# falcon-computing/bwa-flow

Hardware: AMD Instinct MI355X
Metric: million reads/sec (2×150 bp PE) end-to-end align; SW-extend GCUPS at 1/2/4/8 MI355X (higher is better)
Workload: dtype int32

## Files before the change

### bwa-flow_amd/csrc/capi.hip

```cpp
#include <hip/hip_runtime.h>
#include <string.h>

#include <algorithm>
#include <chrono>
#include <condition_variable>
#include <deque>
#include <functional>
#include <cstdio>
#include <mutex>
#include <new>
#include <string>
#include <thread>
#include <vector>

#include "regpost.h"
#include "seed.h"
#include "chain.h"
#include "ctx.h"
#include "engine.h"

using namespace bwagpu;

namespace {

// ... 65 lines not shown

struct InLayout {
  size_t seq_off, seq, rco, cso, rid, frac, seeds, total;
  void make(const bwagpu_batch_t& b) {
    size_t o = 0;
    auto take = [&](size_t n) {
      size_t at = o;
      o += (n + 255) & ~(size_t)255;
      return at;
    };
    seq_off = take(sizeof(int64_t) * (size_t)(b.n_reads + 1));
    rco = take(sizeof(int32_t) * (size_t)(b.n_reads + 1));
    cso = take(sizeof(int32_t) * (size_t)(b.n_chains + 1));
    rid = take(sizeof(int32_t) * (size_t)b.n_chains);
    frac = take(sizeof(float) * (size_t)b.n_chains);
    seeds = take(sizeof(bwagpu_seed_t) * (size_t)b.n_seeds);
    seq = take((size_t)b.seq_bytes);
    total = o;
  }
};

__global__ void side_probe_spin(uint64_t ticks) {
  const uint64_t t0 = __builtin_amdgcn_s_memrealtime();
  while (__builtin_amdgcn_s_memrealtime() - t0 < ticks) __builtin_amdgcn_s_sleep(8);
}
__global__ void side_probe_nop() {}

bool streams_concurrent(hipStream_t a, hipStream_t b) {
  hipEvent_t ea = nullptr, eb = nullptr;
  if (hipEventCreateWithFlags(&ea, hipEventDisableTiming) != hipSuccess) return false;
  if (hipEventCreateWithFlags(&eb, hipEventDisableTiming) != hipSuccess) {
    (void)hipEventDestroy(ea);
    return false;
  }
  hipLaunchKernelGGL(side_probe_spin, dim3(1), dim3(64), 0, a, (uint64_t)15000);
  bool conc = false;
  if (hipGetLastError() == hipSuccess && hipEventRecord(ea, a) == hipSuccess) {
    hipLaunchKernelGGL(side_probe_nop, dim3(1), dim3(64), 0, b);
    if (hipGetLastError() == hipSuccess && hipEventRecord(eb, b) == hipSuccess &&
        hipEventSynchronize(eb) == hipSuccess)
      conc = hipEventQuery(ea) == hipErrorNotReady;
  }
  (void)hipEventSynchronize(ea);
  (void)hipEventDestroy(ea);
  (void)hipEventDestroy(eb);
  return conc;
}

constexpr int kDenseScanBlock = 1024;
__global__ void __launch_bounds__(kDenseScanBlock) dense_scan_kernel(const int32_t* __restrict__ n, int nr,
                                                                     int32_t* __restrict__ off,
                                                                     int32_t* __restrict__ h_off) {
  __shared__ int32_t part[kDenseScanBlock];
  const int t = (int)threadIdx.x;
  const int per = (nr + kDenseScanBlock - 1) / kDenseScanBlock;
  const int r0 = min(t * per, nr), r1 = min(r0 + per, nr);
  int sum = 0;
  for (int r = r0; r < r1; ++r) sum += n[r];
  part[t] = sum;
  __syncthreads();
  for (int d = 1; d < kDenseScanBlock; d <<= 1) {
    const int v = t >= d ? part[t - d] : 0;
    __syncthreads();
    part[t] += v;
    __syncthreads();
  }
  int run = part[t] - sum;
  for (int r = r0; r < r1; ++r) {
    off[r] = run;
    h_off[r] = run;
    run += n[r];
  }
  if (t == kDenseScanBlock - 1) {
    off[nr] = part[t];
    h_off[nr] = part[t];
  }
}

__global__ void __launch_bounds__(256) dense_copy_kernel(const bwagpu_alnreg_t* __restrict__ out,
                                                         const int32_t* __restrict__ n,
                                                         const int32_t* __restrict__ off,
                                                         const int32_t* __restrict__ rco,
                                                         const int32_t* __restrict__ cso, int nr,
                                                         bwagpu_alnreg_t* __restrict__ dense) {
  constexpr int kW = (int)(sizeof(bwagpu_alnreg_t) / 8);
  const int r = (int)((blockIdx.x * 256u + threadIdx.x) >> 4), l = (int)(threadIdx.x & 15);
  if (r >= nr) return;
  const int words = n[r] * kW;
  const uint2* src = reinterpret_cast<const uint2*>(out + cso[rco[r]]);
  uint2* dst = reinterpret_cast<uint2*>(dense + off[r]);
  for (int w = l; w < words; w += 16) dst[w] = src[w];
}

}

namespace {

bool make_opt(const bwagpu_opt_t* o, DevOpt* d, std::string* why) {
  if (!o) { *why = "opt is NULL"; return false; }
  if (o->e_del <= 0 || o->e_ins <= 0) { *why = "gap extension penalties must be > 0"; return false; }
  if (o->w < 0 || o->a < 0) { *why = "negative band width or match score"; return false; }
  if (o->a > 127 || o->e_del > 65535 || o->e_ins > 65535 || o->o_del < 0 || o->o_del > 65535 || o->o_ins < 0 ||
      o->o_ins > 65535 || o->pen_clip5 < 0 || o->pen_clip5 >= (1 << 20) || o->pen_clip3 < 0 ||
      o->pen_clip3 >= (1 << 20) || o->w > (1 << 20)) {
    *why = "scoring option out of range";
    return false;
  }
  memset(d, 0, sizeof(*d));
  d->a = o->a;
  d->o_del = o->o_del;
  d->e_del = o->e_del;
  d->o_ins = o->o_ins;
  d->e_ins = o->e_ins;
  d->oe_del = o->o_del + o->e_del;
  d->oe_ins = o->o_ins + o->e_ins;
  d->pen_clip5 = o->pen_clip5;
  d->pen_clip3 = o->pen_clip3;
  d->w = o->w;
  d->zdrop = o->zdrop;
  int mx = 0;
  for (int i = 0; i < 25; ++i) mx = std::max<int>(mx, o->mat[i]);
  d->max_mat = mx;
  d->row_bound = 1;
  memcpy(d->mat, o->mat, 25);
  for (int q = 0; q < 5; ++q) {
    uint32_t w = 0;
    for (int t = 0; t < 4; ++t) w |= (uint32_t)(uint8_t)o->mat[t * 5 + q] << (8 * t);
    d->qprof[q] = w;
    d->qprof4[q] = o->mat[20 + q];
  }
  return true;
}

int create_common(int device, const bwagpu_opt_t* opt, const bwagpu_bns_t* bns, bwagpu_ctx_t** out,
                  bwagpu_ctx_t** made) {
  if (!out || !bns || bns->l_pac <= 0 || bns->n_seqs <= 0 || !bns->ann_offset || !bns->ann_len)
    return BWAGPU_E_INVAL;
  int n = 0;
  if (hipGetDeviceCount(&n) != hipSuccess || n <= 0) return BWAGPU_E_NODEVICE;
  if (device < 0 || device >= n) return BWAGPU_E_NODEVICE;
  bwagpu_ctx_t* ctx = new (std::nothrow) bwagpu_ctx_t();
  if (!ctx) return BWAGPU_E_NOMEM;
  std::string why;
  if (!make_opt(opt, &ctx->opt, &why)) {
    delete ctx;
    return BWAGPU_E_INVAL;
  }
  ctx->device = device;
  ctx->opt_b = opt->b;
  ctx->ext_form = set_ext_form(-1);
  ctx->ext_short = ext_short_default();
  ctx->ext_short_fill = ext_short_fill_default();
  ctx->light_pack = light_pack_default();
  *made = ctx;
  HIPC(hipSetDevice(device), "hipSetDevice");
  HIPC(hipMalloc(&ctx->d_ann_off, sizeof(int64_t) * bns->n_seqs), "hipMalloc(ann_offset)");
  HIPC(hipMalloc(&ctx->d_ann_len, sizeof(int32_t) * bns->n_seqs), "hipMalloc(ann_len)");
  HIPC(hipMemcpy(ctx->d_ann_off, bns->ann_offset, sizeof(int64_t) * bns->n_seqs, hipMemcpyHostToDevice),
       "upload ann_offset");
  HIPC(hipMemcpy(ctx->d_ann_len, bns->ann_len, sizeof(int32_t) * bns->n_seqs, hipMemcpyHostToDevice),
       "upload ann_len");
  for (auto& s : ctx->slot) {
    HIPC(hipEventCreate(&s.ev0), "hipEventCreate");
    HIPC(hipEventCreate(&s.ev1), "hipEventCreate");
    HIPC(hipEventCreate(&s.ev2), "hipEventCreate");
    HIPC(hipEventCreate(&s.ev3), "hipEventCreate");
  }
  ctx->ref.l_pac = bns->l_pac;
  ctx->ref.n_seqs = bns->n_seqs;
  ctx->ref.ann_offset = ctx->d_ann_off;
  ctx->ref.ann_len = ctx->d_ann_len;
  return BWAGPU_OK;
}

std::vector<Slot*> all_slots(bwagpu_ctx_t* ctx) {
  std::vector<Slot*> v;
  for (auto& x : ctx->slot) v.push_back(&x);
  for (auto& x : ctx->dev_scratch) v.push_back(&x);
  v.push_back(&ctx->ch_slot);
  return v;
}

void destroy_ctx(bwagpu_ctx_t* ctx) {
  if (!ctx) return;
  (void)hipSetDevice(ctx->device);
  for (auto& s : ctx->slot) {
    if (s.stream) (void)hipStreamSynchronize(s.stream);
    s.d_in.release(); s.release_scratch();
    s.d_out.release(); s.d_n.release(); s.d_stats.release();
    s.h_in.release(); s.h_out.release(); s.h_n.release(); s.h_stats.release();
    s.h_dense.release(); s.h_off.release(); s.d_off.release();
    if (s.ev0) (void)hipEventDestroy(s.ev0);
    if (s.ev1) (void)hipEventDestroy(s.ev1);
    if (s.ev2) (void)hipEventDestroy(s.ev2);
    if (s.ev3) (void)hipEventDestroy(s.ev3);
    if (s.stream) (void)hipStreamDestroy(s.stream);
  }
  for (int k = 0; k < BWAGPU_NUM_SLOTS; ++k) {
    if (ctx->dev_stream[k]) (void)hipStreamSynchronize(ctx->dev_stream[k]);
    Slot& s = ctx->dev_scratch[k];
    s.release_scratch();
    s.d_stats.release();
  }
  if (ctx->sdh_done) {
    (void)hipEventSynchronize(ctx->sdh_done);
    (void)hipEventDestroy(ctx->sdh_done);
  }
  for (hipStream_t x : ctx->side_graveyard) {
    (void)hipStreamSynchronize(x);
    (void)hipStreamDestroy(x);
  }
  ctx->side_graveyard.clear();
  for (hipEvent_t e : ctx->prof_ev) (void)hipEventDestroy(e);
  ctx->prof_ev.clear();
  for (int i = 0; i < bwagpu_ctx::kA2Streams; ++i) {
    if (ctx->a2_st[i]) (void)hipStreamSynchronize(ctx->a2_st[i]);
    if (ctx->a2_st[i]) (void)hipStreamDestroy(ctx->a2_st[i]);
    if (ctx->a2_join[i]) (void)hipEventDestroy(ctx->a2_join[i]);
  }
  if (ctx->a2_fork) (void)hipEventDestroy(ctx->a2_fork);
  ctx->ch_slot.release_scratch();
  for (int k = 0; k < 2; ++k) {
    if (ctx->ch_cs.side[k]) (void)hipStreamSynchronize(ctx->ch_cs.side[k]);
    if (ctx->ch_cs.side[k]) (void)hipStreamDestroy(ctx->ch_cs.side[k]);
    if (ctx->ch_cs.join[k]) (void)hipEventDestroy(ctx->ch_cs.join[k]);
  }
  if (ctx->ch_cs.fork) (void)hipEventDestroy(ctx->ch_cs.fork);
  ctx->ch_slot.d_out.release(); ctx->ch_slot.d_n.release(); ctx->ch_slot.d_stats.release();
  if (ctx->r2d_done && ctx->r2d_pending) (void)hipEventSynchronize(ctx->r2d_done);
  for (DevBuf* b : {&ctx->ex_tasks, &ctx->ex_list, &ctx->ex_q, &ctx->ex_t, &ctx->ex_res, &ctx->ex_stats, &ctx->a2_tasks,
                    &ctx->a2_q, &ctx->a2_t, &ctx->a2_out, &ctx->a2_scratch, &ctx->a2_lists, &ctx->a2_counts, &ctx->a2_boff,
                    &ctx->r2_tasks, &ctx->r2_q, &ctx->r2_out, &ctx->r2_cig, &ctx->r2_md, &ctx->r2_lists, &ctx->r2_z,
                    &ctx->r2_stats, &ctx->bwt_words, &ctx->sa_d, &ctx->sa_in, &ctx->sa_out, &ctx->occ_d, &ctx->sup_d, &ctx->sa_full, &ctx->sd_off,
                    &ctx->sd_seq, &ctx->sd_out, &ctx->sd_n, &ctx->sd_scratch, &ctx->sd_poff, &ctx->sd_pack,
                    &ctx->sd_heavy, &ctx->sd_dbg, &ctx->st_buf, &ctx->st_start, &ctx->st_q, &ctx->st_tasks, &ctx->st_lists,
                    &ctx->st_seen, &ctx->st_ctr, &ctx->st_out, &ctx->ch_npos, &ctx->ch_posoff, &ctx->ch_frac,
                    &ctx->ch_nout, &ctx->ch_noseed, &ctx->ch_nsw, &ctx->ch_need, &ctx->ch_swtab, &ctx->ch_alt,
                    &ctx->ch_kpos, &ctx->ch_rbeg, &ctx->ch_qinfo, &ctx->ch_label, &ctx->ch_score, &ctx->ch_slist,
                    &ctx->ch_ord, &ctx->ch_chains, &ctx->ch_nodes, &ctx->ch_ochains, &ctx->ch_oslist, &ctx->ch_bins, &ctx->ch_dbg, &ctx->ch_swoff, &ctx->ch_swtasks, &ctx->ch_swt,
                    &ctx->ch_swskip, &ctx->ch_swres, &ctx->ch_swscr, &ctx->ch_ocoff, &ctx->ch_osoff, &ctx->ch_rco,
                    &ctx->ch_cso, &ctx->ch_rid, &ctx->ch_cfrac, &ctx->ch_out, &ctx->ch_seeds, &ctx->ch_regoff,
                    &ctx->ch_regc, &ctx->rp_stats, &ctx->pe_isize, &ctx->pe_cnt, &ctx->rs_pair, &ctx->rs_soff,
                    &ctx->rs_tab, &ctx->rs_toff, &ctx->rs_boff, &ctx->rs_qpool, &ctx->rs_ctr, &ctx->rs_scr,
                    &ctx->ps_scratch, &ctx->ps_log, &ctx->ps_erfc, &ctx->r2d_keys, &ctx->r2d_lists, &ctx->r2d_tab,
                    &ctx->r2d_z, &ctx->r2d_sums})
    b->release();
  ctx->r2d_htab.release();
  for (hipEvent_t e : {ctx->r2d_done, ctx->r2d_ev[0], ctx->r2d_ev[1]})
    if (e) (void)hipEventDestroy(e);
  ctx->stg.release();
  for (hipEvent_t e : ctx->rs_ev)
    if (e) (void)hipEventDestroy(e);
  for (int k = 0; k < kRescueMaxRounds; ++k)
    for (DevBuf* b : {&ctx->rs_tasks[k], &ctx->rs_tpool[k], &ctx->rs_res[k]}) b->release();
  for (HostBuf* b : {&ctx->sdh_in, &ctx->chh_tot, &ctx->chh_rco, &ctx->chh_cso, &ctx->chh_chains, &ctx->chh_seeds, &ctx->chh_regs,
                     &ctx->chh_n})
    b->release();
  if (ctx->own_pac && ctx->d_pac) (void)hipFree(ctx->d_pac);
  if (ctx->d_ann_off) (void)hipFree(ctx->d_ann_off);
  if (ctx->d_ann_len) (void)hipFree(ctx->d_ann_len);
  delete ctx;
}

int check_batch_header(bwagpu_ctx_t* ctx, const bwagpu_batch_t* b) {
  if (!b) return fail(ctx, BWAGPU_E_INVAL, "batch is NULL");
  if (b->n_reads < 0 || b->n_chains < 0 || b->n_seeds < 0 || b->seq_bytes < 0)
    return fail(ctx, BWAGPU_E_INVAL, "negative batch dimension");
  if (b->n_reads == 0) return BWAGPU_OK;
  if (!b->seq_off || !b->read_chain_off || !b->chain_seed_off)
    return fail(ctx, BWAGPU_E_INVAL, "NULL offset array");
  if (b->seq_off[0] != 0 || b->seq_off[b->n_reads] != b->seq_bytes)
    return fail(ctx, BWAGPU_E_INVAL, "seq_off does not span seq_bytes");
  if (b->read_chain_off[0] != 0 || b->read_chain_off[b->n_reads] != b->n_chains)
    return fail(ctx, BWAGPU_E_INVAL, "read_chain_off does not span n_chains");
  if (b->chain_seed_off[0] != 0 || b->chain_seed_off[b->n_chains] != b->n_seeds)
    return fail(ctx, BWAGPU_E_INVAL, "chain_seed_off does not span n_seeds");
  if (b->n_chains && (!b->chain_rid || !b->chain_frac_rep)) return fail(ctx, BWAGPU_E_INVAL, "NULL chain array");
  if (b->n_seeds && !b->seeds) return fail(ctx, BWAGPU_E_INVAL, "NULL seeds");
  if (b->seq_bytes && !b->seq) return fail(ctx, BWAGPU_E_INVAL, "NULL seq");
  return BWAGPU_OK;
}

int check_reads(const bwagpu_batch_t* b, int64_t l_pac, int r0, int r1, int64_t* lmax, int* bad_read) {
  const int64_t two = l_pac << 1;
  const int64_t* so = b->seq_off;
  const int32_t* rco = b->read_chain_off;
  const int32_t* cso = b->chain_seed_off;
  const bwagpu_seed_t* sd = b->seeds;
  int64_t lm = 0;
  for (int r = r0; r < r1; ++r) {
    const int64_t l = so[r + 1] - so[r];
    if (l < 0) return 1;
    if (l > BWAGPU_MAX_READ_LEN) {
      *bad_read = r;
      return 2;
    }
    lm = std::max(lm, l);
    const int c0 = rco[r], c1 = rco[r + 1];
    if (c0 < 0 || c1 < c0 || c1 > b->n_chains) return 3;
    bool bad_seed = false;
    for (int c = c0; c < c1; ++c) {
      const int k0 = cso[c], k1 = cso[c + 1];
      if (k0 < 0 || k1 < k0 || k1 > b->n_seeds) return 4;
      for (int k = k0; k < k1; ++k) {
        const bwagpu_seed_t& s = sd[k];
        bad_seed |= (s.qbeg < 0) | (s.len <= 0) | ((int64_t)s.qbeg + s.len > l) | (s.rbeg < 0) | (s.rbeg + s.len > two);
// ... 31 lines not shown
  int code[4] = {0, 0, 0, 0}, bad_read[4] = {0, 0, 0, 0};
  int64_t lmaxs[4] = {0, 0, 0, 0};
  host_parallel(nt, [&](int t) {
    code[t] = check_reads(b, ctx->ref.l_pac, (int)((int64_t)b->n_reads * t / nt),
                          (int)((int64_t)b->n_reads * (t + 1) / nt), &lmaxs[t], &bad_read[t]);
  });
  if (int rc = check_report(ctx, b, code, bad_read, nt)) return rc;
  *lq_max_out = (int)std::max(std::max(lmaxs[0], lmaxs[1]), std::max(lmaxs[2], lmaxs[3]));
  return BWAGPU_OK;
}

int stage_and_check(bwagpu_ctx_t* ctx, const bwagpu_batch_t* b, char* h, const InLayout& L, int* lq_max_out) {
  *lq_max_out = 0;
  const int nr = b->n_reads;
  if (nr == 0) return BWAGPU_OK;
  constexpr int kBlk = 1024, kMaxT = 8;
  const int nt = b->n_seeds >= (1 << 16) ? kMaxT : 1;
  const int nblk = (nr + kBlk - 1) / kBlk;
  int code[kMaxT] = {}, bad_read[kMaxT] = {};
  int64_t lmaxs[kMaxT] = {};
  auto work = [&](int t) {
    for (int k = (int)((int64_t)nblk * t / nt), ke = (int)((int64_t)nblk * (t + 1) / nt); k < ke; ++k) {
      const int r0 = k * kBlk, r1 = std::min(nr, r0 + kBlk);
      const int64_t b0 = b->seq_off[r0], b1 = b->seq_off[r1];
      const int c0 = b->read_chain_off[r0], c1 = b->read_chain_off[r1];
      if (b0 < 0 || b1 < b0 || b1 > b->seq_bytes) {
        code[t] = 1;
        return;
      }
      if (c0 < 0 || c1 < c0 || c1 > b->n_chains) {
        code[t] = 3;
        return;
      }
      const int k0 = b->chain_seed_off[c0], k1 = b->chain_seed_off[c1];
      if (k0 < 0 || k1 < k0 || k1 > b->n_seeds) {
        code[t] = 4;
        return;
      }
      const int re = r1 == nr ? r1 + 1 : r1, ce = c1 == b->n_chains ? c1 + 1 : c1;
      memcpy(h + L.seq_off + sizeof(int64_t) * r0, b->seq_off + r0, sizeof(int64_t) * (size_t)(re - r0));
      memcpy(h + L.rco + sizeof(int32_t) * r0, b->read_chain_off + r0, sizeof(int32_t) * (size_t)(re - r0));
      memcpy(h + L.cso + sizeof(int32_t) * c0, b->chain_seed_off + c0, sizeof(int32_t) * (size_t)(ce - c0));
      if (c1 > c0) {
        memcpy(h + L.rid + sizeof(int32_t) * c0, b->chain_rid + c0, sizeof(int32_t) * (size_t)(c1 - c0));
        memcpy(h + L.frac + sizeof(float) * c0, b->chain_frac_rep + c0, sizeof(float) * (size_t)(c1 - c0));
      }
      if (k1 > k0) memcpy(h + L.seeds + sizeof(bwagpu_seed_t) * k0, b->seeds + k0, sizeof(bwagpu_seed_t) * (size_t)(k1 - k0));
      if (b1 > b0) memcpy(h + L.seq + b0, b->seq + b0, (size_t)(b1 - b0));
      int64_t lm = 0;
      if ((code[t] = check_reads(b, ctx->ref.l_pac, r0, r1, &lm, &bad_read[t]))) return;
      lmaxs[t] = std::max(lmaxs[t], lm);
    }
  };
  host_parallel(nt, work);
  if (int rc = check_report(ctx, b, code, bad_read, nt)) return rc;
  int64_t lm = 0;
  for (int t = 0; t < nt; ++t) lm = std::max(lm, lmaxs[t]);
  *lq_max_out = (int)lm;
  return BWAGPU_OK;
}

bool use_read_kernels() {
  const char* e = getenv("BWAGPU_C2A_PATH");
  return e && (strcmp(e, "fast") == 0 || strcmp(e, "read") == 0);
}

size_t variant_lds(const DevOpt& o, int v, int lq_max) {
  const Variant& vk = kVariants[v];
  const int lqv = std::min(lq_max, vk.max_len());
  const int tb = tb_bytes_for(o, std::max(lqv, 1));
  return vk.kind == VK_FAST ? (size_t)(kBlock / 64) * fast_wave_lds(tb) : (size_t)tb * (kBlock / vk.G);
}

int check_lds(bwagpu_ctx_t* ctx, int lq_max) {
  if (!use_read_kernels()) {
    if (spec_redo_cap(tb_bytes_for(ctx->opt, std::max(lq_max, 1))) < 64)
      return fail(ctx, BWAGPU_E_UNSUPPORTED, "LDS row buffer too large for these options (w, pen_clip, read length)");
    return BWAGPU_OK;
  }
  for (int v = 0; v < kNumVariants; ++v) {
    if (variant_lds(ctx->opt, v, lq_max) > 64 * 1024)
      return fail(ctx, BWAGPU_E_UNSUPPORTED, "LDS row buffer too large for these options (w, pen_clip, read length)");
  }
  return BWAGPU_OK;
}

void register_caller_locked(bwagpu_ctx_t* ctx, hipStream_t st) {
  for (hipStream_t c : ctx->callers)
    if (c == st) return;
  for (Slot* x : all_slots(ctx))
    if (x->side_chosen && x->spec.side && hipStreamSynchronize(x->spec.side) == hipSuccess &&
        !streams_concurrent(x->spec.side, st)) {
      ctx->side_graveyard.push_back(x->spec.side);
      x->spec.side = nullptr;
      x->side_chosen = false;
    }
  ctx->callers.push_back(st);
}

hipError_t choose_side(bwagpu_ctx_t* ctx, Slot& s, hipStream_t st, SpecStreams* snap) {
  std::lock_guard<std::mutex> g(ctx->side_mu);
  register_caller_locked(ctx, st);
  if (s.side_chosen) {
    *snap = s.spec;
    return hipSuccess;
  }
  if (!s.spec.fork) {
    hipError_t e = hipEventCreateWithFlags(&s.spec.fork, hipEventDisableTiming);
    if (e == hipSuccess) e = hipEventCreateWithFlags(&s.spec.join, hipEventDisableTiming);
    if (e != hipSuccess) return e;
  }
  std::vector<hipStream_t> avoid = ctx->callers;
  for (Slot* x : all_slots(ctx))
    if (x != &s && x->side_chosen && x->spec.side) avoid.push_back(x->spec.side);
  std::vector<hipStream_t> tried;
  hipStream_t pick = nullptr;
  hipError_t e = hipSuccess;
  for (int t = 0; t < 6 && !pick; ++t) {
    hipStream_t c = nullptr;
    if ((e = hipStreamCreateWithFlags(&c, hipStreamNonBlocking)) != hipSuccess) break;
    bool ok = true;
    for (hipStream_t a : avoid)
      if (!streams_concurrent(c, a)) {
        ok = false;
        break;
      }
    if (ok) pick = c;
    else tried.push_back(c);
  }
  for (hipStream_t c : tried) (void)hipStreamDestroy(c);
  if (e != hipSuccess) return e;
  s.spec.side = pick;
  s.side_chosen = true;
  *snap = s.spec;
  return hipSuccess;
}

int enqueue_spec(bwagpu_ctx_t* ctx, Slot& s, const DevBatch& db, int lq_max, bwagpu_alnreg_t* d_out, int32_t* d_n,
                 int64_t* d_stats, hipStream_t st) {
  const size_t nc = (size_t)std::max(db.n_chains, 1), ns = (size_t)std::max(db.n_seeds, 1),
               nr = (size_t)std::max(db.n_reads, 1);
  HIPC(s.d_win.ensure(sizeof(ChainWin) * nc), "hipMalloc(win)");
  HIPC(s.d_cread.ensure(sizeof(int32_t) * nc), "hipMalloc(chain_read)");
  HIPC(s.d_prog.ensure(sizeof(bwagpu_seed_t) * ns), "hipMalloc(prog)");
  HIPC(s.d_ext.ensure(sizeof(SeedExt) * ns), "hipMalloc(ext)");
  HIPC(s.d_tasks.ensure(sizeof(int2) * kSpecBins * (nc + (kSpecRounds - 1) * ns)), "hipMalloc(tasks)");
  HIPC(s.d_ctr.ensure(sizeof(int32_t) * SPC_WORDS), "hipMalloc(ctr)");
  HIPC(s.d_regpos.ensure(sizeof(int32_t) * ns), "hipMalloc(regpos)");
  HIPC(s.d_skipf.ensure(sizeof(int32_t) * ns), "hipMalloc(skipf)");
  HIPC(s.d_heavy.ensure(sizeof(int32_t) * nr), "hipMalloc(heavy)");
  HIPC(s.d_redo.ensure(sizeof(int32_t) * nr), "hipMalloc(redo)");
  HIPC(s.d_rbits.ensure(sizeof(uint32_t) * (nr / 32 + 1)), "hipMalloc(rbits)");
  HIPC(s.d_desc.ensure(sizeof(ReadDesc) * nr), "hipMalloc(desc)");
  HIPC(s.d_schain.ensure(sizeof(int32_t) * ns), "hipMalloc(seedchain)");
  HIPC(s.d_hinfo.ensure(sizeof(int4) * nr), "hipMalloc(hinfo)");
  HIPC(s.d_cov.ensure(sizeof(int32_t) * ns), "hipMalloc(cov)");
  HIPC(s.d_hflag.ensure(sizeof(int32_t) * ns), "hipMalloc(hflag)");
  HIPC(s.d_colent.ensure(sizeof(int32_t) * ns), "hipMalloc(colent)");
  HIPC(s.d_longc.ensure(sizeof(int32_t) * nc), "hipMalloc(longc)");
  HIPC(s.d_qh.ensure(sizeof(int32_t) * kQHWords), "hipMalloc(qh)");
  HIPC(s.d_sorth.ensure(sizeof(int32_t) * kSortWords), "hipMalloc(sorth)");
  HIPC(s.d_stasks.ensure(sizeof(int2) * kSpecBins * (nc + (kSpecRounds - 1) * ns)), "hipMalloc(stasks)");
  HIPC(s.d_ftask.ensure(sizeof(FatTask) * kSpecBins * (nc + (kSpecRounds - 1) * ns)), "hipMalloc(ftask)");
  HIPC(s.d_ftaskR.ensure(sizeof(FatTask) * kSpecBins * (nc + (kSpecRounds - 1) * ns)), "hipMalloc(ftaskR)");
  const int64_t mat_words = std::max<int64_t>(1 << 20, 16 * (int64_t)ns);
  HIPC(s.d_mat.ensure(sizeof(uint64_t) * (size_t)mat_words), "hipMalloc(mat)");
  SpecArgs a;
  a.win = s.d_win.as<ChainWin>();
  a.chain_read = s.d_cread.as<int32_t>();
  a.prog = s.d_prog.as<bwagpu_seed_t>();
  a.ext = s.d_ext.as<SeedExt>();
  a.tasks = s.d_tasks.as<int2>();
  a.ctr = s.d_ctr.as<int32_t>();
  a.regpos = s.d_regpos.as<int32_t>();
  a.skipf = s.d_skipf.as<int32_t>();
  a.heavy = s.d_heavy.as<int32_t>();
  a.redo = s.d_redo.as<int32_t>();
  a.rbits = s.d_rbits.as<uint32_t>();
  a.rdesc = s.d_desc.as<ReadDesc>();
  a.seedchain = s.d_schain.as<int32_t>();
  a.hinfo = s.d_hinfo.as<int4>();
  a.mat = s.d_mat.as<uint64_t>();
  a.mat_words = (int64_t)(s.d_mat.cap / sizeof(uint64_t));
  a.cov = s.d_cov.as<int32_t>();
  a.hflag = s.d_hflag.as<int32_t>();
  a.colent = s.d_colent.as<int32_t>();
  a.longc = s.d_longc.as<int32_t>();
  a.qh = s.d_qh.as<int32_t>();
  a.sorth = s.d_sorth.as<int32_t>();
  a.stasks = s.d_stasks.as<int2>();
  a.ftask = s.d_ftask.as<FatTask>();
  a.ftaskR = s.d_ftaskR.as<FatTask>();
  static const int ext_prefetch = [] {
    const char* e = getenv("BWAGPU_EXT_PREFETCH");
    return e ? std::max(0, atoi(e)) : 0;
  }();
  a.ext_prefetch = ext_prefetch;
  static const int risky_first = [] {
    const char* e = getenv("BWAGPU_LIGHT_RISKY_FIRST");
    return e && e[0] == '1';
  }();
  a.risky_first = risky_first;
  static const int emu_strict = [] {
    const char* e = getenv("BWAGPU_EMU_STRICT");
    return !(e && e[0] == '0');
  }();
  a.emu_strict = emu_strict;
  a.light_pack = ctx->light_pack;
  a.out = d_out;
  a.out_n = d_n;
  a.stats = d_stats;
  SpecStreams ss;
  HIPC(choose_side(ctx, s, st, &ss), "side stream");
  a.lq_bound = lq_max;
  const int tb = tb_bytes_for(ctx->opt, std::max(lq_max, 1));
  ss.form = ctx->ext_form;
  ss.short_q = ctx->ext_short;
  ss.short_fill = ctx->ext_short_fill;
  ss.pool = ctx->prof_ev.empty() ? nullptr : ctx->prof_ev.data();
  ss.pool_n = (int)ctx->prof_ev.size();
  ss.pool_used = &ctx->prof_used;
  HIPC(launch_spec_clear(a, db.n_reads, db.n_seeds, st), "spec clear");
  HIPC(launch_spec_chain2aln(ctx->opt, ctx->ref, db, a, tb, lq_max, st, ss), "spec chain2aln launch");
  return BWAGPU_OK;
}

int enqueue_chain2aln(bwagpu_ctx_t* ctx, Slot& s, const DevBatch& db, int lq_max, bwagpu_alnreg_t* d_out,
                      int32_t* d_n, int64_t* d_stats, hipStream_t st) {
  if (!use_read_kernels()) return enqueue_spec(ctx, s, db, lq_max, d_out, d_n, d_stats, st);
  HIPC(s.d_win.ensure(sizeof(ChainWin) * (size_t)std::max(db.n_chains, 1)), "hipMalloc(win)");
  HIPC(s.d_srt.ensure(sizeof(uint64_t) * (size_t)std::max(db.n_seeds, 1)), "hipMalloc(srt)");
  HIPC(s.d_prog.ensure(sizeof(bwagpu_seed_t) * (size_t)std::max(db.n_seeds, 1)), "hipMalloc(prog)");
  const size_t nr = (size_t)std::max(db.n_reads, 1);
  HIPC(s.d_desc.ensure(sizeof(ReadDesc) * nr), "hipMalloc(desc)");
  HIPC(s.d_lists.ensure(2 * sizeof(int32_t) * nr), "hipMalloc(lists)");
  int32_t* bins = s.d_lists.as<int32_t>();
  int32_t* read_list = bins + nr;
  HIPC(s.d_counts.ensure(sizeof(int32_t) * kCountWords), "hipMalloc(counts)");
  HIPC(hipMemsetAsync(s.d_counts.p, 0, sizeof(int32_t) * kCountWords, st), "memset counts");
  if (db.n_reads) HIPC(hipMemsetAsync(d_n, 0, sizeof(int32_t) * db.n_reads, st), "memset out_n");
  HIPC(launch_chain_prep(ctx->opt, ctx->ref, db, s.d_win.as<ChainWin>(), s.d_srt.as<uint64_t>(),
                         s.d_prog.as<bwagpu_seed_t>(), d_stats, st),
       "chain_prep launch");
  HIPC(launch_read_order(db, bins, s.d_counts.as<int32_t>() + kHistOff, s.d_counts.as<int32_t>(),
                         s.d_desc.as<ReadDesc>(), read_list, d_stats, st),
       "read order launch");
  C2AArgs a;
  a.read_list = read_list;
  a.desc = s.d_desc.as<ReadDesc>();
  a.counts = s.d_counts.as<int32_t>();
  a.win = s.d_win.as<ChainWin>();
  a.srt = s.d_srt.as<uint64_t>();
  a.prog = s.d_prog.as<bwagpu_seed_t>();
  a.out = d_out;
  a.out_n = d_n;
  a.stats = d_stats;
  for (int v = 0; v < kNumVariants; ++v) {
    const int lqv = std::min(lq_max, kVariants[v].max_len());
    const int tb = tb_bytes_for(ctx->opt, std::max(lqv, 1));
    HIPC(launch_chain2aln(v, ctx->opt, ctx->ref, db, db.n_reads, tb, a, st), "chain2aln launch");
  }
  return BWAGPU_OK;
}

}

extern "C" {

int bwagpu_abi_version(void) { return BWAGPU_ABI_VERSION; }

int bwagpu_device_count(int* n) {
  if (!n) return BWAGPU_E_INVAL;
  int k = 0;
  if (hipGetDeviceCount(&k) != hipSuccess) k = 0;
  *n = k;
  return k > 0 ? BWAGPU_OK : BWAGPU_E_NODEVICE;
}

int bwagpu_create(int device, const bwagpu_opt_t* opt, const bwagpu_bns_t* bns, const uint8_t* pac_host,
                  bwagpu_ctx_t** out) {
  if (!pac_host) return BWAGPU_E_INVAL;
  bwagpu_ctx_t* ctx = nullptr;
  int rc = create_common(device, opt, bns, out, &ctx);
  if (rc == BWAGPU_OK) {
    const size_t pac_bytes = (size_t)(bns->l_pac / 4 + 1);
    hipError_t e = hipMalloc(&ctx->d_pac, pac_bytes);
    if (e == hipSuccess) {
      ctx->own_pac = true;
      e = hipMemcpy(ctx->d_pac, pac_host, pac_bytes, hipMemcpyHostToDevice);
    }
    if (e != hipSuccess) rc = hip_fail(ctx, e, "pac upload");
    ctx->ref.pac = (const uint8_t*)ctx->d_pac;
  }
  if (rc != BWAGPU_OK) {
    destroy_ctx(ctx);
    return rc;
  }
  *out = ctx;
  return BWAGPU_OK;
}

int bwagpu_create_resident(int device, const bwagpu_opt_t* opt, const bwagpu_bns_t* bns, const void* pac_device,
                           bwagpu_ctx_t** out) {
  if (!pac_device) return BWAGPU_E_INVAL;
  bwagpu_ctx_t* ctx = nullptr;
  int rc = create_common(device, opt, bns, out, &ctx);
  if (rc != BWAGPU_OK) {
    destroy_ctx(ctx);
    return rc;
  }
  ctx->d_pac = (void*)pac_device;
  ctx->own_pac = false;
  ctx->ref.pac = (const uint8_t*)pac_device;
  *out = ctx;
  return BWAGPU_OK;
}

int bwagpu_destroy(bwagpu_ctx_t* ctx) {
  if (!ctx) return BWAGPU_E_INVAL;
  destroy_ctx(ctx);
  return BWAGPU_OK;
}

const char* bwagpu_last_error(const bwagpu_ctx_t* ctx) { return ctx ? ctx->err.c_str() : "NULL context"; }

int bwagpu_set_watchdog_ms(bwagpu_ctx_t* ctx, int ms) {
  if (!ctx || ms < 0) return BWAGPU_E_INVAL;
  ctx->watchdog_ms = ms;
  return BWAGPU_OK;
}

namespace {
void expand_slots(const Slot& s, bwagpu_alnreg_t* dst) {
  const char* h = s.h_in.as<const char>();
  const int32_t* rco = s.kept ? s.keep_rco.data() : (const int32_t*)(h + s.in_rco);
  const int32_t* cso = s.kept ? s.keep_cso.data() : (const int32_t*)(h + s.in_cso);
  const int32_t* n = s.h_n.as<const int32_t>();
  const int32_t* off = s.h_off.as<const int32_t>();
  const bwagpu_alnreg_t* src = s.h_dense.as<const bwagpu_alnreg_t>();
  for (int32_t r = 0; r < s.n_reads; ++r)
    if (n[r]) memcpy(dst + cso[rco[r]], src + off[r], sizeof(bwagpu_alnreg_t) * (size_t)n[r]);
}
}

int bwagpu_chain2aln_submit(bwagpu_ctx_t* ctx, int slot, const bwagpu_batch_t* b) {
  if (!ctx || slot < 0 || slot >= BWAGPU_NUM_SLOTS) return BWAGPU_E_INVAL;
  Slot& s = ctx->slot[slot];
  if (s.busy) return fail(ctx, BWAGPU_E_INVAL, "slot already has a batch in flight");
  s.has_results = false;
  s.kept = false;
  s.slot_view = false;
  int lq_max = 0;
  int rc = check_batch_header(ctx, b);
  if (rc) return rc;
  HIPC(hipSetDevice(ctx->device), "hipSetDevice");
  s.t_submit = std::chrono::steady_clock::now();
  InLayout L;
  L.make(*b);
  HIPC(s.h_in.ensure(L.total), "hipHostMalloc(in)");
  HIPC(s.d_in.ensure(L.total), "hipMalloc(in)");
  HIPC(s.d_out.ensure(sizeof(bwagpu_alnreg_t) * (size_t)std::max(b->n_seeds, 1)), "hipMalloc(out)");
// ... 187 lines not shown
  if (!ctx || slot < 0 || slot >= BWAGPU_NUM_SLOTS || !regs || !n || !off) return BWAGPU_E_INVAL;
  Slot& s = ctx->slot[slot];
  if (s.busy) return fail(ctx, BWAGPU_E_INVAL, "slot's batch still in flight (wait first)");
  if (!s.has_results || !s.h_dense.p || !s.h_off.p) return fail(ctx, BWAGPU_E_INVAL, "slot has no results");
  *regs = s.h_dense.as<const bwagpu_alnreg_t>();
  *n = s.h_n.as<const int32_t>();
  *off = s.h_off.as<const int32_t>();
  return BWAGPU_OK;
}

int bwagpu_chain2aln(bwagpu_ctx_t* ctx, const bwagpu_batch_t* b, bwagpu_alnreg_t* out_regs, int32_t* out_n) {
  int rc = bwagpu_chain2aln_submit(ctx, 0, b);
  if (rc) return rc;
  return bwagpu_chain2aln_wait(ctx, 0, out_regs, out_n);
}

int bwagpu_chain2aln_device(bwagpu_ctx_t* ctx, const bwagpu_batch_t* db_in, bwagpu_alnreg_t* dev_out,
                            int32_t* dev_n, int64_t* dev_stats, void* stream) {
  if (!ctx || !db_in || !dev_out || !dev_n) return BWAGPU_E_INVAL;
  HIPC(hipSetDevice(ctx->device), "hipSetDevice");
  const int lq_bound = use_read_kernels() ? BWAGPU_MAX_READ_LEN : ctx->dev_read_len;
  int rc = check_lds(ctx, lq_bound);
  if (rc) return rc;
  hipStream_t st = (hipStream_t)stream;
  if (!st) HIPC(lazy_stream(ctx->slot[0], &st), "hipStreamCreate");
  int k = 0;
  while (k < BWAGPU_NUM_SLOTS && ctx->dev_stream[k] && ctx->dev_stream[k] != st) ++k;
  if (k == BWAGPU_NUM_SLOTS) return fail(ctx, BWAGPU_E_INVAL, "more than BWAGPU_NUM_SLOTS streams on one context");
  ctx->dev_stream[k] = st;
  Slot& s = ctx->dev_scratch[k];
  DevBatch db;
  db.n_reads = db_in->n_reads;
  db.n_chains = db_in->n_chains;
  db.n_seeds = db_in->n_seeds;
  db.seq_off = db_in->seq_off;
  db.seq = db_in->seq;
  db.read_chain_off = db_in->read_chain_off;
  db.chain_seed_off = db_in->chain_seed_off;
  db.chain_rid = db_in->chain_rid;
  db.chain_frac_rep = db_in->chain_frac_rep;
  db.seeds = db_in->seeds;
  int64_t* stats = dev_stats;
  if (!stats) {
    HIPC(s.d_stats.ensure(sizeof(int64_t) * ST_N), "hipMalloc(stats)");
    stats = s.d_stats.as<int64_t>();
    HIPC(hipMemsetAsync(stats, 0, sizeof(int64_t) * ST_N, st), "memset stats");
  }
  return enqueue_chain2aln(ctx, s, db, lq_bound, dev_out, dev_n, stats, st);
}

int bwagpu_debug_set_trace(bwagpu_ctx_t* ctx, void* dev_ptr) {
  if (!ctx) return BWAGPU_E_INVAL;
  HIPC(hipSetDevice(ctx->device), "hipSetDevice");
  HIPC(set_trace(dev_ptr), "set trace");
  HIPC(set_trace_spec(dev_ptr), "set trace");
  return BWAGPU_OK;
}

int bwagpu_debug_fail_wait(bwagpu_ctx_t* ctx, int after_n_waits, int code) {
  if (!ctx || code <= 0) return BWAGPU_E_INVAL;
  ctx->fail_after = after_n_waits;
  ctx->fail_code = code;
  return BWAGPU_OK;
}

int bwagpu_debug_occupancy(bwagpu_ctx_t* ctx, void* stream, int64_t* out) {
  if (!ctx || !out) return BWAGPU_E_INVAL;
  hipStream_t st = nullptr;
  if (int rc = entry_stream(ctx, stream, &st)) return rc;
  int k = 0;
  while (k < BWAGPU_NUM_SLOTS && ctx->dev_stream[k] != st) ++k;
  if (k == BWAGPU_NUM_SLOTS || !ctx->dev_scratch[k].d_ctr.p) return fail(ctx, BWAGPU_E_INVAL, "no device-entry batch on this stream");
  HIPC(hipStreamSynchronize(st), "hipStreamSynchronize");
  int32_t c[SPC_WORDS];
  HIPC(hipMemcpy(c, ctx->dev_scratch[k].d_ctr.p, sizeof c, hipMemcpyDeviceToHost), "hipMemcpy(ctr)");
  memcpy(out, c + 32, 14 * sizeof(int64_t));
#ifdef BWAGPU_OCC_DIAG
  return BWAGPU_OK;
#else
  return fail(ctx, BWAGPU_E_UNSUPPORTED, "built without BWAGPU_OCC_DIAG");
#endif
}

int bwagpu_debug_spec_counters(bwagpu_ctx_t* ctx, void* stream, int64_t* out) {
  if (!ctx || !out) return BWAGPU_E_INVAL;
  hipStream_t st = nullptr;
  if (int rc = entry_stream(ctx, stream, &st)) return rc;
  int k = 0;
  while (k < BWAGPU_NUM_SLOTS && ctx->dev_stream[k] != st) ++k;
  if (k == BWAGPU_NUM_SLOTS || !ctx->dev_scratch[k].d_ctr.p) return fail(ctx, BWAGPU_E_INVAL, "no device-entry batch on this stream");
  HIPC(hipStreamSynchronize(st), "hipStreamSynchronize");
  int32_t c[SPC_WORDS];
  HIPC(hipMemcpy(c, ctx->dev_scratch[k].d_ctr.p, sizeof c, hipMemcpyDeviceToHost), "hipMemcpy(ctr)");
  for (int r = 0; r < kSpecRounds; ++r) {
    out[r] = 0;
    for (int b = 0; b < kSpecBins; ++b) out[r] += c[SPC_CNT + r * kSpecBins + b];
  }
  int64_t spec = 0;
  memcpy(&spec, c + SPC_SPEC64, 8);
  out[3] = spec;
  out[4] = c[SPC_MISS];
  out[5] = c[SPC_HEAVY_N];
  out[6] = c[SPC_REDO_N];
  out[7] = c[SPC_HCOLS];
  return BWAGPU_OK;
}

int bwagpu_debug_spec_ext(bwagpu_ctx_t* ctx, void* stream, void* host_out, int32_t n) {
  if (!ctx || !host_out || n < 0) return BWAGPU_E_INVAL;
  hipStream_t st = nullptr;
  if (int rc = entry_stream(ctx, stream, &st)) return rc;
  int k = 0;
  while (k < BWAGPU_NUM_SLOTS && ctx->dev_stream[k] != st) ++k;
  if (k == BWAGPU_NUM_SLOTS || !ctx->dev_scratch[k].d_ext.p || ctx->dev_scratch[k].d_ext.cap < sizeof(SeedExt) * (size_t)n)
    return fail(ctx, BWAGPU_E_INVAL, "no device-entry batch of that size on this stream");
  HIPC(hipStreamSynchronize(st), "hipStreamSynchronize");
  HIPC(hipMemcpy(host_out, ctx->dev_scratch[k].d_ext.p, sizeof(SeedExt) * (size_t)n, hipMemcpyDeviceToHost),
       "hipMemcpy(ext)");
  return BWAGPU_OK;
}

int bwagpu_debug_ext_form(int form) { return set_ext_form(form); }

int bwagpu_streams_concurrent(void* a, void* b) {
  if (!a || !b || a == b) return BWAGPU_E_INVAL;
  return streams_concurrent((hipStream_t)a, (hipStream_t)b) ? 1 : 0;
}

int bwagpu_ctx_ext_form(bwagpu_ctx_t* ctx, int form) {
  if (!ctx) return BWAGPU_E_INVAL;
  const int prev = ctx->ext_form;
  if (form >= 0) ctx->ext_form = form > 2 ? 1 : form;
  return prev;
}

int bwagpu_ctx_ext_short(bwagpu_ctx_t* ctx, int q) {
  if (!ctx) return BWAGPU_E_INVAL;
  const int prev = ctx->ext_short;
  if (q >= 0) ctx->ext_short = q > 63 ? 63 : q;
  return prev;
}

int bwagpu_ctx_ext_short_fill(bwagpu_ctx_t* ctx, int percent) {
  if (!ctx) return BWAGPU_E_INVAL;
  const int prev = ctx->ext_short_fill;
  if (percent >= 0) ctx->ext_short_fill = percent > 100000 ? 100000 : percent;
  return prev;
}

int bwagpu_ctx_light_pack(bwagpu_ctx_t* ctx, int on) {
  if (!ctx) return BWAGPU_E_INVAL;
  const int prev = ctx->light_pack;
  if (on >= 0) ctx->light_pack = on != 0;
  return prev;
}

int bwagpu_debug_spec_short(bwagpu_ctx_t* ctx, void* stream, int64_t* out) {
  if (!ctx || !out) return BWAGPU_E_INVAL;
  hipStream_t st = nullptr;
  if (int rc = entry_stream(ctx, stream, &st)) return rc;
  int k = 0;
  while (k < BWAGPU_NUM_SLOTS && ctx->dev_stream[k] != st) ++k;
  if (k == BWAGPU_NUM_SLOTS || !ctx->dev_scratch[k].d_ctr.p) return fail(ctx, BWAGPU_E_INVAL, "no device-entry batch on this stream");
  HIPC(hipStreamSynchronize(st), "hipStreamSynchronize");
  int32_t c[SPC_WORDS];
  HIPC(hipMemcpy(c, ctx->dev_scratch[k].d_ctr.p, sizeof c, hipMemcpyDeviceToHost), "hipMemcpy(ctr)");
  out[0] = c[SPC_SHORT_N];
  for (int r = 0; r < 2; ++r) {
    const int l = r * kSpecBins;
    out[1 + 4 * r] = c[SPC_LCNT + l];
    out[2 + 4 * r] = c[SPC_LLONG + l];
    out[3 + 4 * r] = c[SPC_RCNT + l];
    out[4 + 4 * r] = c[SPC_RLONG + l];
  }
  return BWAGPU_OK;
}

int bwagpu_ctx_row_bound(bwagpu_ctx_t* ctx, int on) {
  if (!ctx) return BWAGPU_E_INVAL;
  const int prev = ctx->opt.row_bound;
  if (on >= 0) ctx->opt.row_bound = on ? 1 : 0;
  return prev;
}

int bwagpu_debug_ext_kernel(bwagpu_ctx_t* ctx, int32_t lq_max) {
  if (!ctx || lq_max < 1 || lq_max > BWAGPU_MAX_READ_LEN) return BWAGPU_E_INVAL;
  return ext_kernel_for(ctx->opt, ctx->ext_form, tb_bytes_for(ctx->opt, lq_max));
}

int bwagpu_prof_start(bwagpu_ctx_t* ctx, int max_launches) {
  if (!ctx || max_launches < 0) return BWAGPU_E_INVAL;
  HIPC(hipSetDevice(ctx->device), "hipSetDevice");
  for (hipEvent_t e : ctx->prof_ev) HIPC(hipEventSynchronize(e), "hipEventSynchronize");
  for (hipEvent_t e : ctx->prof_ev) (void)hipEventDestroy(e);
  ctx->prof_ev.clear();
  ctx->prof_used = 0;
  for (int i = 0; i < 2 * max_launches; ++i) {
    hipEvent_t e = nullptr;
    HIPC(hipEventCreate(&e), "hipEventCreate");
    ctx->prof_ev.push_back(e);
  }
  return BWAGPU_OK;
}

int bwagpu_prof_read(bwagpu_ctx_t* ctx, double* total_ms, int32_t* launches) {
  if (!ctx || !total_ms || !launches) return BWAGPU_E_INVAL;
  HIPC(hipSetDevice(ctx->device), "hipSetDevice");
  double t = 0;
  for (int i = 0; i + 1 < ctx->prof_used; i += 2) {
    HIPC(hipEventSynchronize(ctx->prof_ev[i + 1]), "hipEventSynchronize");
    float ms = 0;
    HIPC(hipEventElapsedTime(&ms, ctx->prof_ev[i], ctx->prof_ev[i + 1]), "hipEventElapsedTime");
    t += ms;
  }
  *total_ms = t;
  *launches = ctx->prof_used / 2;
  return BWAGPU_OK;
}

int bwagpu_prof_intervals(bwagpu_ctx_t* ctx, double* start_ms, double* end_ms, int32_t max, int32_t* n) {
  if (!ctx || !n || max < 0 || (max && (!start_ms || !end_ms))) return BWAGPU_E_INVAL;
  HIPC(hipSetDevice(ctx->device), "hipSetDevice");
  int k = 0;
  for (int i = 0; i + 1 < ctx->prof_used && k < max; i += 2, ++k) {
    HIPC(hipEventSynchronize(ctx->prof_ev[i + 1]), "hipEventSynchronize");
    float a = 0, b = 0;
    HIPC(hipEventElapsedTime(&a, ctx->prof_ev[0], ctx->prof_ev[i]), "hipEventElapsedTime");
    HIPC(hipEventElapsedTime(&b, ctx->prof_ev[0], ctx->prof_ev[i + 1]), "hipEventElapsedTime");
    start_ms[k] = a;
    end_ms[k] = b;
  }
  *n = k;
  return BWAGPU_OK;
}

int bwagpu_last_stats(const bwagpu_ctx_t* ctx, int slot, bwagpu_stats_t* out) {
  if (!ctx || !out || slot < 0 || slot >= BWAGPU_NUM_SLOTS) return BWAGPU_E_INVAL;
  *out = ctx->slot[slot].last;
  return BWAGPU_OK;
}

}

extern "C" int bwagpu_set_bwt(bwagpu_ctx_t* ctx, const bwagpu_bwt_t* bwt) {
  if (!ctx || !bwt || !bwt->bwt || bwt->bwt_size == 0) return BWAGPU_E_INVAL;
  if (bwt->bwt_size < ((bwt->seq_len + 127) >> 7) * 16 || bwt->L2[4] != bwt->seq_len || bwt->primary > bwt->seq_len)
    return fail(ctx, BWAGPU_E_INVAL, "bwt header inconsistent with its occurrence array");
  HIPC(hipSetDevice(ctx->device), "hipSetDevice");
  HIPC(ctx->bwt_words.ensure(sizeof(uint32_t) * bwt->bwt_size + 64), "hipMalloc");
  HIPC(hipMemcpy(ctx->bwt_words.p, bwt->bwt, sizeof(uint32_t) * bwt->bwt_size, hipMemcpyHostToDevice), "H2D");
  ctx->bwt.primary = bwt->primary;
  for (int i = 0; i < 5; ++i) ctx->bwt.L2[i] = bwt->L2[i];
  ctx->bwt.seq_len = bwt->seq_len;
  ctx->bwt.bwt = ctx->bwt_words.as<uint32_t>();
  {
    HIPC(ctx->occ_d.ensure(2 * sizeof(uint4) * (size_t)occ64_blocks(bwt->seq_len)), "hipMalloc");
    ctx->bwt.sup_shift = ctx->sup_shift;
    HIPC(ctx->sup_d.ensure(4 * sizeof(uint64_t) * (size_t)occ64_supers(bwt->seq_len, ctx->sup_shift)), "hipMalloc");
    HIPC(hipMemset(ctx->occ_d.p, 0, 2 * sizeof(uint4) * (size_t)occ64_blocks(bwt->seq_len)), "memset");
    hipStream_t st = nullptr;
  HIPC(lazy_stream(ctx->slot[0], &st), "hipStreamCreate");
    HIPC(launch_build_occ64(ctx->bwt, ctx->occ_d.as<uint4>(), ctx->sup_d.as<uint64_t>(), st), "build_occ64 launch");
    HIPC(hipStreamSynchronize(st), "sync");
    ctx->bwt.occ = ctx->occ_d.as<uint4>();
    ctx->bwt.sup = ctx->sup_d.as<uint64_t>();
  }
  ctx->bwt.sa = nullptr;
  ctx->bwt.sa_mask = 0;
  ctx->bwt.sa_shift = 0;
  ctx->bwt.sa_full32 = nullptr;
  ctx->bwt.sa_full64 = nullptr;
  if (bwt->sa) {
    const int iv = bwt->sa_intv;
    if (iv < 1 || (iv & (iv - 1)) || bwt->n_sa < bwt->seq_len / (uint64_t)iv + 1)
      return fail(ctx, BWAGPU_E_INVAL, "suffix array sample interval / size inconsistent");
    HIPC(ctx->sa_d.ensure(sizeof(uint64_t) * bwt->n_sa), "hipMalloc");
    HIPC(hipMemcpy(ctx->sa_d.p, bwt->sa, sizeof(uint64_t) * bwt->n_sa, hipMemcpyHostToDevice), "H2D");
    ctx->bwt.sa = ctx->sa_d.as<uint64_t>();
    ctx->bwt.sa_mask = (uint64_t)iv - 1;
    while ((1 << ctx->bwt.sa_shift) < iv) ++ctx->bwt.sa_shift;
    const char* fe = getenv("BWAGPU_SA_FULL");
    const bool narrow = bwt->seq_len < 0xffffffffull && !(fe && strcmp(fe, "64") == 0);
    const uint64_t bytes = (bwt->seq_len + 1) * (narrow ? 4 : 8);
    size_t free_b = 0, total_b = 0;
    if (!(fe && strcmp(fe, "0") == 0) && iv > 1 && hipMemGetInfo(&free_b, &total_b) == hipSuccess &&
        bytes <= ((uint64_t)64 << 30) && bytes <= free_b / 4) {
      HIPC(ctx->sa_full.ensure((size_t)bytes), "hipMalloc");
      hipStream_t st = nullptr;
      HIPC(lazy_stream(ctx->slot[0], &st), "hipStreamCreate");
      HIPC(launch_sa_expand(ctx->bwt, narrow ? ctx->sa_full.as<uint32_t>() : nullptr,
                            narrow ? nullptr : ctx->sa_full.as<uint64_t>(), st),
           "sa_expand launch");
      HIPC(hipStreamSynchronize(st), "sync");
      if (narrow) ctx->bwt.sa_full32 = ctx->sa_full.as<uint32_t>();
      else ctx->bwt.sa_full64 = ctx->sa_full.as<uint64_t>();
    }
  }
  ctx->has_bwt = true;
  return BWAGPU_OK;
}

extern "C" int bwagpu_bwt_sa(bwagpu_ctx_t* ctx, int64_t n, const uint64_t* k, uint64_t* out) {
  if (!ctx || n < 0 || (n && (!k || !out))) return BWAGPU_E_INVAL;
  if (!ctx->has_bwt || !ctx->bwt.sa) return fail(ctx, BWAGPU_E_INVAL, "no suffix array: pass it to bwagpu_set_bwt");
  for (int64_t i = 0; i < n; ++i)
    if (k[i] > ctx->bwt.seq_len) return fail(ctx, BWAGPU_E_INVAL, "BWT position past seq_len");
// ... 533 lines not shown
```

### bwa-flow_amd/csrc/ctx.h

```cpp
#pragma once
#include <hip/hip_runtime.h>
#include <stdint.h>

#include <algorithm>
#include <chrono>
#include <mutex>
#include <string>
#include <vector>

#include "bwagpu.h"
#include "chain.h"
#include "engine.h"
#include "rescue.h"
#include "seed.h"
#include "stage_host.h"
#include "task_host.h"

namespace bwagpu {

template <bool kPinned>
struct GrowBuf {
  void* p = nullptr;
  size_t cap = 0;
  hipError_t ensure(size_t n) {
    if (n <= cap) return hipSuccess;
    release();
    const size_t want = std::max<size_t>(n + n / 4, 4096);
    const hipError_t e = kPinned ? hipHostMalloc(&p, want, hipHostMallocDefault) : hipMalloc(&p, want);
    if (e == hipSuccess) cap = want;
    else p = nullptr;
    return e;
  }
  void release() {
    if (p) (void)(kPinned ? hipHostFree(p) : hipFree(p));
    p = nullptr;
    cap = 0;
  }
  template <class T>
  T* as() const { return (T*)p; }
};
using DevBuf = GrowBuf<false>;
using HostBuf = GrowBuf<true>;

struct Slot {
  hipStream_t stream = nullptr;
  std::once_flag stream_once;
  hipError_t stream_err = hipSuccess;
  hipEvent_t ev0 = nullptr, ev1 = nullptr, ev2 = nullptr, ev3 = nullptr;
  DevBuf d_in, d_win, d_srt, d_prog, d_desc, d_out, d_n, d_stats, d_lists, d_counts;
  DevBuf d_cread, d_ext, d_tasks, d_ctr, d_regpos, d_skipf, d_heavy, d_redo, d_rbits;
  DevBuf d_schain, d_hinfo, d_mat, d_cov, d_hflag, d_colent, d_qh, d_longc, d_sorth, d_stasks, d_ftask, d_ftaskR;
  SpecStreams spec;
  bool side_chosen = false;
  void release_scratch() {
    d_win.release(); d_srt.release(); d_prog.release(); d_desc.release(); d_lists.release(); d_counts.release();
    d_cread.release(); d_ext.release(); d_tasks.release(); d_ctr.release(); d_regpos.release(); d_skipf.release();
    d_heavy.release(); d_redo.release(); d_rbits.release(); d_schain.release(); d_hinfo.release(); d_mat.release(); d_cov.release(); d_hflag.release(); d_colent.release(); d_longc.release();
    d_qh.release();
    d_sorth.release();
    d_stasks.release();
    d_ftask.release();
    d_ftaskR.release();
    if (spec.side) (void)hipStreamSynchronize(spec.side);
    if (spec.side) (void)hipStreamDestroy(spec.side);
    if (spec.fork) (void)hipEventDestroy(spec.fork);
    if (spec.join) (void)hipEventDestroy(spec.join);
    spec = SpecStreams{};
    side_chosen = false;
  }
  HostBuf h_in, h_out, h_n, h_stats;
  HostBuf h_dense, h_off;
  DevBuf d_off;
  size_t in_rco = 0, in_cso = 0;
  bool slot_view = false;
  bool busy = false;
  bool has_results = false;
  bool kept = false;
  std::vector<int32_t> keep_rco, keep_cso;
  int32_t n_reads = 0, n_chains = 0, n_seeds = 0;
  std::chrono::steady_clock::time_point t_submit;
  bwagpu_stats_t last{};
  int64_t h2d = 0, d2h = 0;
};

inline hipError_t lazy_stream(Slot& s, hipStream_t* st) {
  std::call_once(s.stream_once, [&s] { s.stream_err = hipStreamCreateWithFlags(&s.stream, hipStreamNonBlocking); });
  *st = s.stream;
  return s.stream_err;
}

struct Staging {
  DevBuf regs, out_regs;
  DevBuf seq;
  DevBuf seq_off, reg_off, out_off;
  DevBuf n, out_n, n_pri, status, n_sw, mapq, sel;
  DevBuf pes;
  void release() {
    for (DevBuf* b : {&regs, &out_regs, &seq, &seq_off, &reg_off, &out_off, &n, &out_n, &n_pri, &status, &n_sw, &mapq,
                      &sel, &pes})
      b->release();
  }
};

}

struct bwagpu_ctx {
  using DevBuf = bwagpu::DevBuf;
  using HostBuf = bwagpu::HostBuf;
  using Slot = bwagpu::Slot;
  int device = 0;
  std::mutex side_mu;
  std::vector<hipStream_t> callers, side_graveyard;
  bwagpu::DevOpt opt{};
  bwagpu::DevRef ref{};
  bool own_pac = false;
  void* d_pac = nullptr;
  int64_t* d_ann_off = nullptr;
  int32_t* d_ann_len = nullptr;
  int watchdog_ms = 10000;
  int ext_form = 0;
  int ext_short = 0;
  int light_pack = 0;
  int ext_short_fill = 0;
  Slot slot[BWAGPU_NUM_SLOTS];
  hipStream_t dev_stream[BWAGPU_NUM_SLOTS] = {};
  Slot dev_scratch[BWAGPU_NUM_SLOTS];
  DevBuf ex_tasks, ex_list, ex_q, ex_t, ex_res, ex_stats;
  DevBuf a2_tasks, a2_q, a2_t, a2_out, a2_scratch, a2_lists, a2_counts, a2_boff;
  DevBuf r2_tasks, r2_q, r2_out, r2_cig, r2_md, r2_lists, r2_z, r2_stats;
  DevBuf r2d_keys, r2d_lists, r2d_tab, r2d_z, r2d_sums;
  HostBuf r2d_htab;
  hipEvent_t r2d_done = nullptr, r2d_ev[2] = {};
  bool r2d_pending = false, r2d_timing = false, r2d_timed = false;
  double r2d_wait_ms = 0, r2d_call_ms = 0;
  int32_t r2d_jobs = 0;
  static constexpr int kA2Streams = 4;
  hipStream_t a2_st[kA2Streams] = {};
  hipEvent_t a2_fork = nullptr, a2_join[kA2Streams] = {};
  DevBuf bwt_words, sa_d, sa_in, sa_out, occ_d, sup_d, sa_full;
  bwagpu::DevBwt bwt{};
  bool has_bwt = false;
  DevBuf sd_off, sd_seq, sd_out, sd_n, sd_scratch, sd_poff, sd_pack, sd_heavy, sd_dbg;
  DevBuf ch_npos, ch_posoff, ch_frac, ch_nout, ch_noseed, ch_nsw, ch_need, ch_swtab, ch_alt;
  DevBuf ch_kpos, ch_rbeg, ch_qinfo, ch_label, ch_score, ch_slist, ch_ord, ch_chains, ch_nodes;
  DevBuf ch_ochains, ch_oslist, ch_bins, ch_dbg;
  DevBuf ch_swoff, ch_swtasks, ch_swt, ch_swskip, ch_swres, ch_swscr;
  DevBuf ch_ocoff, ch_osoff, ch_rco, ch_cso, ch_rid, ch_cfrac, ch_out, ch_seeds;
  DevBuf ch_regoff, ch_regc;
  HostBuf chh_tot, chh_rco, chh_cso, chh_chains, chh_seeds, chh_regs, chh_n;
  HostBuf sdh_in;
  hipEvent_t sdh_done = nullptr;
  Slot ch_slot;
  bwagpu::ChainStreams ch_cs{};
  bool has_alt = false;
  bwagpu::Staging stg;
  int opt_b = 0;
  bwagpu_postopt_t post_opt{};
  int32_t post_flags = 0;
  int64_t post_id0 = 0;
  DevBuf rp_stats;
  DevBuf pe_isize, pe_cnt;
  DevBuf rs_pair, rs_soff, rs_tab, rs_toff, rs_boff, rs_qpool, rs_ctr, rs_scr;
  DevBuf rs_tasks[bwagpu::kRescueMaxRounds], rs_tpool[bwagpu::kRescueMaxRounds], rs_res[bwagpu::kRescueMaxRounds];
  int32_t rescue_drop = 0;
  hipEvent_t rs_ev[4 * bwagpu::kRescueMaxRounds] = {};
  int rs_ev_rounds = 0;
  hipStream_t rs_ev_stream = nullptr;
  DevBuf ps_scratch, ps_log, ps_erfc;
  bool ps_log_ready = false;
  DevBuf st_buf, st_start, st_q, st_tasks, st_lists, st_seen, st_ctr, st_out;
  int seed_budget = 1024;
  int sup_shift = 32;
  int dev_read_len = BWAGPU_MAX_READ_LEN;
  int fail_after = -1, fail_code = 0;
  std::vector<hipEvent_t> prof_ev;
  int prof_used = 0;
  std::string err;
};

namespace bwagpu {

inline int fail(bwagpu_ctx_t* c, int code, const std::string& msg) {
  if (c) c->err = msg;
  return code;
}

inline int hip_fail(bwagpu_ctx_t* c, hipError_t e, const char* what) {
  std::string m = std::string(what) + ": " + hipGetErrorString(e);
  if (e == hipErrorOutOfMemory || e == hipErrorMemoryAllocation) return fail(c, BWAGPU_E_NOMEM, m);
  return fail(c, BWAGPU_E_DEVICE, m);
}

#define HIPC(call, what)                             \
  do {                                               \
    hipError_t e_ = (call);                          \
    if (e_ != hipSuccess) return hip_fail(ctx, e_, what); \
  } while (0)
#define TRY(call)                     \
  do {                                \
    if (int rc_ = (call)) return rc_; \
  } while (0)

inline int refuse(bwagpu_ctx_t* c, int code, const char* why) { return why && *why ? fail(c, code, why) : code; }

inline int entry_stream(bwagpu_ctx_t* ctx, void* stream, hipStream_t* st) {
  HIPC(hipSetDevice(ctx->device), "hipSetDevice");
  *st = (hipStream_t)stream;
  if (!*st) HIPC(lazy_stream(ctx->slot[0], st), "hipStreamCreate");
  return BWAGPU_OK;
}

inline int side_fork(bwagpu_ctx_t* ctx, hipStream_t st, size_t n_launches, int* used) {
  for (int i = 0; i < bwagpu_ctx::kA2Streams; ++i) {
    if (!ctx->a2_st[i]) HIPC(hipStreamCreateWithFlags(&ctx->a2_st[i], hipStreamNonBlocking), "stream");
    if (!ctx->a2_join[i]) HIPC(hipEventCreateWithFlags(&ctx->a2_join[i], hipEventDisableTiming), "event");
  }
  if (!ctx->a2_fork) HIPC(hipEventCreateWithFlags(&ctx->a2_fork, hipEventDisableTiming), "event");
  *used = (int)std::min<size_t>(bwagpu_ctx::kA2Streams, n_launches);
  HIPC(hipEventRecord(ctx->a2_fork, st), "event");
  for (int i = 0; i < *used; ++i) HIPC(hipStreamWaitEvent(ctx->a2_st[i], ctx->a2_fork, 0), "stream wait");
  return BWAGPU_OK;
}
inline int side_join(bwagpu_ctx_t* ctx, hipStream_t st, int used) {
  for (int i = 0; i < used; ++i) {
    HIPC(hipEventRecord(ctx->a2_join[i], ctx->a2_st[i]), "event");
    HIPC(hipStreamWaitEvent(st, ctx->a2_join[i], 0), "stream wait");
  }
  return BWAGPU_OK;
}

struct EventPair {
  hipEvent_t e0 = nullptr, e1 = nullptr;
  EventPair() = default;
  EventPair(const EventPair&) = delete;
  EventPair& operator=(const EventPair&) = delete;
  ~EventPair() {
    if (e0) (void)hipEventDestroy(e0);
    if (e1) (void)hipEventDestroy(e1);
  }
  hipError_t start(hipStream_t st) {
    hipError_t e = hipEventCreate(&e0);
    if (e == hipSuccess) e = hipEventCreate(&e1);
    return e == hipSuccess ? hipEventRecord(e0, st) : e;
  }
  hipError_t stop(hipStream_t st) { return hipEventRecord(e1, st); }
  float ms() const {
    float t = 0;
    (void)hipEventElapsedTime(&t, e0, e1);
    return t;
  }
};

int enqueue_regpost(bwagpu_ctx_t* ctx, const bwagpu_postopt_t& po, int32_t flags, int64_t id0, int32_t n_reads,
                    const int64_t* seq_off, const uint8_t* seq, const int64_t* reg_off, const int32_t* rco,
                    const int32_t* cso, bwagpu_alnreg_t* regs, int32_t* n, int64_t* stats, hipStream_t st);

struct HostCall {
  bwagpu_ctx_t* ctx;
  Staging& g;
  hipStream_t st = nullptr;
  EventPair ev;
  int64_t h2d = 0, d2h = 0, hs[ST_N] = {};
  std::vector<int64_t> roff, soff, ooff;
  bool open = false;

  explicit HostCall(bwagpu_ctx_t* c) : ctx(c), g(c->stg) {}
  HostCall(const HostCall&) = delete;
  HostCall& operator=(const HostCall&) = delete;
  ~HostCall() {
    if (open) (void)hipStreamSynchronize(st);
  }
  int begin() {
    if (int rc = entry_stream(ctx, nullptr, &st)) return rc;
    open = true;
    return BWAGPU_OK;
// ... 55 lines not shown
```

### bwa-flow_amd/csrc/engine.h

```cpp
#pragma once
#include <hip/hip_runtime.h>
#include <stdint.h>

#include "bwagpu.h"
#include "bwagpu_debug.h"
#include "pure.h"
#include "spec_plan.h"

namespace bwagpu {

struct ReadDesc {
  int64_t qoff;
  int32_t rd;
  int32_t lq;
  int32_t c0;
  int32_t nch;
  int32_t s0;
  int32_t ns;
};

struct ChainWin {
  int64_t lo, hi;
};

struct DevBatch {
  int32_t n_reads, n_chains, n_seeds;
  const int64_t* seq_off;
  const uint8_t* seq;
  const int32_t* read_chain_off;
  const int32_t* chain_seed_off;
  const int32_t* chain_rid;
  const float* chain_frac_rep;
  const bwagpu_seed_t* seeds;
};

struct DevRef {
  int64_t l_pac;
  int32_t n_seqs;
  const uint8_t* pac;
  const int64_t* ann_offset;
  const int32_t* ann_len;
};

enum { ST_CELLS = 0, ST_ROWS = 1, ST_CALLS = 2, ST_ERR = 3, ST_N = 4 };
enum { ERR_RID = 1, ERR_LEN = 2 };

constexpr int kFastMaxSeeds = 32;
constexpr int kFastMaxChains = 32;
constexpr int kSeqLds = 256;
constexpr int kNumVariants = 3;
extern const Variant kVariants[kNumVariants];
constexpr int kHistOff = 128;
constexpr int kCountWords = kHistOff + kNumVariants * 256;

hipError_t launch_chain_prep(const DevOpt& o, const DevRef& ref, const DevBatch& b, ChainWin* win, uint64_t* srt,
                             bwagpu_seed_t* prog, int64_t* stats, hipStream_t st);
hipError_t launch_read_order(const DevBatch& b, int32_t* bins, int32_t* hist, int32_t* counts, ReadDesc* desc,
                             int32_t* list, int64_t* stats, hipStream_t st);
struct C2AArgs {
  const int32_t* read_list;
  const ReadDesc* desc;
  int32_t* counts;
  const ChainWin* win;
  uint64_t* srt;
  const bwagpu_seed_t* prog;
  bwagpu_alnreg_t* out;
  int32_t* out_n;
  int64_t* stats;
};
hipError_t launch_chain2aln(int variant, const DevOpt& o, const DevRef& ref, const DevBatch& b, int32_t max_list,
                            int tb_bytes, const C2AArgs& a, hipStream_t st);
size_t fast_wave_lds(int tb);

hipError_t launch_extend(int variant, bool t5, const DevOpt& o, int32_t n_tasks,
                         const bwagpu_ext_task_t* tasks, const int32_t* task_list, int32_t n_list,
                         const uint8_t* qpool, const uint8_t* tpool, int tb_bytes,
                         bwagpu_ext_result_t* res, int64_t* stats, hipStream_t st);
hipError_t launch_extend4(const DevOpt& o, const bwagpu_ext_task_t* tasks, const int32_t* task_list, int32_t n_list,
                          const uint8_t* qpool, const uint8_t* tpool, int tb_bytes, bwagpu_ext_result_t* res,
                          int64_t* stats, hipStream_t st);

struct SeedExt {
  int64_t rb, re;
  int32_t qb, qe, score, truesc, w;
  int32_t cells, rows, calls;
};

constexpr int kSpecRounds = 3;
constexpr int kOrderLane = 8;
constexpr int kSelLight = 64;
constexpr int kSelRegLds = 256;
constexpr int kSelMatMaxSeeds = 4096;
enum {
  SPC_CNT = 0,
  SPC_HEAVY_N = 16,
  SPC_SEL_CUR = 17,
  SPC_REDO_N = 20,
  SPC_SPEC64 = 24,
  SPC_MISS = 26,
  SPC_MATW64 = 28,
  SPC_HCOLS = 30,
  SPC_LONG_N = 31,
  SPC_LCNT = 64,
  SPC_RCNT = 73,
  SPC_LIGHT_CUR = 82,
  SPC_LLONG = 84,
  SPC_RLONG = 93,
  SPC_SHORT_N = 102,
  SPC_WORDS = 128
};
constexpr int kQHStride = 32;
constexpr int kQHShort = 2 * kSpecRounds * kSpecBins * 8 * kQHStride;
constexpr int kQHWords = 2 * kQHShort;
constexpr int kSortKeys = 1024;
constexpr int kSortWordsR = kSpecRounds * 2 * kSortKeys;
constexpr int kSortWords = 2 * kSortWordsR;
__host__ __device__ inline size_t spec_list_off(int list, int n_chains, int n_seeds) {
  const int round = list / kSpecBins, bin = list % kSpecBins;
  return round == 0 ? (size_t)bin * n_chains
                    : (size_t)kSpecBins * n_chains + ((size_t)(round - 1) * kSpecBins + bin) * n_seeds;
}
struct FatTask {
  int64_t rbeg, qoff;
  int32_t pos;
  int32_t dlo, dhi;
  uint32_t qls;
};
static_assert(sizeof(FatTask) == 32, "FatTask layout");
static_assert(BWAGPU_MAX_READ_LEN < 1024, "FatTask packs qbeg / len / lq in 10 bits each");
struct SpecArgs {
  int lq_bound;
  ChainWin* win;
  int32_t* chain_read;
  bwagpu_seed_t* prog;
  SeedExt* ext;
  int2* tasks;
  int32_t* ctr;
  int32_t* regpos;
  int32_t* skipf;
  int32_t* heavy;
  int32_t* redo;
  uint32_t* rbits;
  ReadDesc* rdesc;
  int32_t* seedchain;
  int4* hinfo;
  int32_t* colent;
  int32_t* longc;
  uint64_t* mat;
  int64_t mat_words;
  int32_t* cov;
  int32_t* hflag;
  int32_t* qh;
  int32_t* sorth;
  int2* stasks;
  FatTask* ftask;
  FatTask* ftaskR;
  int risky_first;
  int emu_strict;
  int light_pack;
  int ext_prefetch;
  bwagpu_alnreg_t* out;
  int32_t* out_n;
  int64_t* stats;
};
struct SpecStreams {
  hipStream_t side = nullptr;
  hipEvent_t fork = nullptr, join = nullptr;
  hipEvent_t* pool = nullptr;
  int pool_n = 0;
  int* pool_used = nullptr;
  int form = 0;
  int short_q = 0;
  int short_fill = 0;
};
int set_ext_form(int form);
int ext_short_default();
int ext_short_fill_default();
int light_pack_default();
int ext_kernel_for(const DevOpt& o, int form, int tb_bytes);
hipError_t launch_spec_clear(const SpecArgs& a, int n_reads, int n_seeds, hipStream_t st);
hipError_t launch_spec_chain2aln(const DevOpt& o, const DevRef& ref, const DevBatch& b, const SpecArgs& a,
                                 int tb_bytes, int lq_max, hipStream_t st, const SpecStreams& ss);
size_t spec_select_lds(int tb_bytes);
int spec_redo_cap(int tb_bytes);

struct StreamTask {
  bwagpu_seed_t s;
  int64_t lo, hi;
  int64_t qoff;
  int32_t lq, pad_;
};
enum { STR_ERR_RECORD = 1, STR_ERR_TASK = 2, STR_ERR_DUP = 4, STR_ERR_SEED = 8, STR_ERR_BASE = 16 };
enum { kStrDecoded = 4, kStrMax = 5, kStrErr = 6, kStrHeads = 64 };
constexpr int kStrCtrWords = kStrHeads + kSpecBins * 8 * kQHStride;
struct StreamArgs {
  const int32_t* buf;
  const int64_t* rstart;
  int32_t n_reads, cap;
  int64_t l_pac;
  uint8_t* qpool;
  StreamTask* tasks;
  int32_t* lists;
  int32_t* seen;
  int32_t* ctr;
  int32_t* out;
};
hipError_t launch_sw_stream(const DevOpt& o, const DevRef& ref, const StreamArgs& a, int tb_bytes, hipStream_t st);

hipError_t set_trace(void* dev_ptr);
hipError_t set_trace_spec(void* dev_ptr);

}
```

### bwa-flow_amd/csrc/spec.hip

```cpp
#include "spec_dev.h"

namespace bwagpu {

__device__ uint32_t* g_trace = nullptr;
hipError_t set_trace_spec(void* p) { return hipMemcpyToSymbol(HIP_SYMBOL(g_trace), &p, sizeof(p)); }


__global__ void __launch_bounds__(256) spec_chain_kernel(DevOpt o, DevRef ref, DevBatch b, SpecArgs a) {
  sel_prio();
  const int c = blockIdx.x * blockDim.x + threadIdx.x;
  bool task = false, longc = false;
  int bin = 0, s0 = 0;
  if (c < b.n_chains) {
    const int rd = a.chain_read[c];
    s0 = b.chain_seed_off[c];
    const int ns = b.chain_seed_off[c + 1] - s0;
    const int lq = (int)(b.seq_off[rd + 1] - b.seq_off[rd]);
    if (ns <= 0) {
      a.win[c] = ChainWin{0, 0};
    } else {
      int64_t wlo = ref.l_pac << 1, whi = 0;
      longc = ns > kOrderLane;
      if (!longc) {
        uint64_t key[kOrderLane];
#pragma unroll
        for (int t = 0; t < kOrderLane; ++t) {
          key[t] = ~0ull;
          if (t < ns) {
            const bwagpu_seed_t v = b.seeds[s0 + t];
            key[t] = (uint64_t)(uint32_t)v.score << 32 | (uint32_t)t;
            seed_reach(o, v, lq, wlo, whi);
          }
        }
#pragma unroll
        for (int t = 0; t < kOrderLane; ++t) {
          if (t < ns) {
            int rank = 0;
#pragma unroll
            for (int u = 0; u < kOrderLane; ++u) rank += key[u] < key[t];
            bwagpu_seed_t v = b.seeds[s0 + t];
            v.pad_ = key[t] == 0 ? 1 : 0;
            a.prog[s0 + ns - 1 - rank] = v;
            a.seedchain[s0 + ns - 1 - rank] = c;
          }
        }
      }
      const bool ok = finish_window(ref, b.chain_rid[c], b.seeds[s0].rbeg, wlo, whi);
      if (!ok) {
        atomicOr((unsigned long long*)&a.stats[ST_ERR], (unsigned long long)ERR_RID);
        a.win[c] = ChainWin{0, -1};
      } else {
        if (!longc) a.win[c] = ChainWin{wlo, whi};
        task = lq <= a.lq_bound;
        bin = spec_bin(lq);
      }
    }
  }
#pragma unroll
  for (int k = 0; k < kSpecBins; ++k) {
    const int p = wave_append(&a.ctr[SPC_CNT + k], task && bin == k);
    if (p >= 0) a.tasks[(size_t)k * b.n_chains + p] = make_int2(s0, c);
  }
  const int p = wave_append(&a.ctr[SPC_LONG_N], longc);
  if (p >= 0) a.longc[p] = c;
}

__global__ void __launch_bounds__(256) spec_reads_kernel(DevBatch b, SpecArgs a) {
  sel_prio();
  const int rd = blockIdx.x * blockDim.x + threadIdx.x;
  bool heavy = false;
  int ns = 0;
  if (rd < b.n_reads) {
    const int lq = (int)(b.seq_off[rd + 1] - b.seq_off[rd]);
    if (lq > a.lq_bound) atomicOr((unsigned long long*)&a.stats[ST_ERR], (unsigned long long)ERR_LEN);
    ReadDesc d;
    d.qoff = b.seq_off[rd];
    d.rd = rd;
    d.lq = lq;
    d.c0 = b.read_chain_off[rd];
    d.nch = b.read_chain_off[rd + 1] - d.c0;
    d.s0 = b.chain_seed_off[d.c0];
    d.ns = b.chain_seed_off[d.c0 + d.nch] - d.s0;
    a.rdesc[rd] = d;
    for (int c = d.c0; c < d.c0 + d.nch; ++c) a.chain_read[c] = rd;
    heavy = d.ns > kSelLight || d.nch > kSelLight;
    ns = d.ns;
  }
  const int p = wave_append(&a.ctr[SPC_HEAVY_N], heavy);
  if (p >= 0) {
    a.heavy[p] = rd;
    const long long words = 2 * tri_off(ns);
    int woff = -1, col = 0;
    if (ns <= kSelMatMaxSeeds) {
      const long long o = (long long)atomicAdd(reinterpret_cast<unsigned long long*>(&a.ctr[SPC_MATW64]),
                                               (unsigned long long)words);
      if (o + words <= a.mat_words) {
        woff = (int)o;
        col = atomicAdd(&a.ctr[SPC_HCOLS], ns);
        for (int i = 0; i < ns; ++i) a.colent[col + i] = p;
      }
    }
    a.hinfo[p] = make_int4(rd, woff, col, ns);
  }
}

constexpr int kOrderBlocks = 1024;
constexpr int kOrderLds = 4096;
__device__ __forceinline__ uint64_t order_key(const bwagpu_seed_t* sd, int i) {
  return (uint64_t)(uint32_t)sd[i].score << 32 | (uint32_t)i;
}
__global__ void __launch_bounds__(256) spec_order_kernel(DevOpt o, DevRef ref, DevBatch b, SpecArgs a) {
  sel_prio();
  __shared__ uint64_t keys[kOrderLds];
  __shared__ int64_t wred[2][4];
  const int tid = (int)threadIdx.x;
  const int n_long = __hip_atomic_load(&a.ctr[SPC_LONG_N], __ATOMIC_RELAXED, __HIP_MEMORY_SCOPE_AGENT);
  for (int gi = (int)blockIdx.x; gi < n_long; gi += (int)gridDim.x) {
    const int g = a.longc[gi];
    const int s0 = b.chain_seed_off[g], ns = b.chain_seed_off[g + 1] - s0;
    const bwagpu_seed_t* sd = b.seeds + s0;
    const bool in_lds = ns <= kOrderLds;
    const int rd = a.chain_read[g];
    const int lq = (int)(b.seq_off[rd + 1] - b.seq_off[rd]);
    int64_t wlo = ref.l_pac << 1, whi = 0;
    for (int i = tid; i < ns; i += 256) {
      const bwagpu_seed_t v = sd[i];
      if (in_lds) keys[i] = (uint64_t)(uint32_t)v.score << 32 | (uint32_t)i;
      seed_reach(o, v, lq, wlo, whi);
    }
#pragma unroll
    for (int m = 32; m >= 1; m >>= 1) {
      wlo = min(wlo, (int64_t)__shfl_xor((long long)wlo, m, 64));
      whi = max(whi, (int64_t)__shfl_xor((long long)whi, m, 64));
    }
    if ((tid & 63) == 0) {
      wred[0][tid >> 6] = wlo;
      wred[1][tid >> 6] = whi;
    }
    __syncthreads();
    if (tid == 0) {
      wlo = min(min(wred[0][0], wred[0][1]), min(wred[0][2], wred[0][3]));
      whi = max(max(wred[1][0], wred[1][1]), max(wred[1][2], wred[1][3]));
      if (finish_window(ref, b.chain_rid[g], sd[0].rbeg, wlo, whi)) a.win[g] = ChainWin{wlo, whi};
    }
    for (int i = tid; i < ns; i += 256) {
      bwagpu_seed_t v = sd[i];
      const uint64_t ki = (uint64_t)(uint32_t)v.score << 32 | (uint32_t)i;
      int rank = 0;
      if (in_lds)
        for (int j = 0; j < ns; ++j) rank += keys[j] < ki;
      else
        for (int j = 0; j < ns; ++j) rank += order_key(sd, j) < ki;
      v.pad_ = ki == 0 ? 1 : 0;
      a.prog[s0 + ns - 1 - rank] = v;
      a.seedchain[s0 + ns - 1 - rank] = g;
    }
    __syncthreads();
  }
}


template <int C>
__global__ void __launch_bounds__(kBlock) spec_ext_kernel(DevOpt o, DevRef ref, DevBatch b, SpecArgs a, int list,
                                                          int tb_bytes) {
  extern __shared__ __attribute__((aligned(16))) uint8_t lds[];
  const int wib = uni((int)(threadIdx.x >> 6));
  uint8_t* const tbl = lds + wib * 2 * tb_bytes;
  uint8_t* const tbr = tbl + tb_bytes;
  const int n = uni(__hip_atomic_load(&a.ctr[SPC_CNT + list], __ATOMIC_RELAXED, __HIP_MEMORY_SCOPE_AGENT));
  const int2* tl = a.tasks + spec_list_off(list, b.n_chains, b.n_seeds);
  ShardQ qq;
  qq.init(a.qh + 8 * kQHStride * list, n);
  long long spec_cells = 0;
  int m0, cap;
  while (qq.claim(1, m0, cap)) {
    for (int m = m0; m < m0 + 1 && m < cap; ++m) {
      const int2 tk = tl[qq.shard + 8 * m];
      const int pos = uni(tk.x), c = uni(tk.y);
      const int rd = uni(a.chain_read[c]);
      const int64_t qoff = uni64(b.seq_off[rd]);
      const int lq = uni((int)(b.seq_off[rd + 1] - qoff));
      const bwagpu_seed_t s = uni_seed(a.prog[pos]);
      ChainWin cw = a.win[c];
      cw.lo = uni64(cw.lo);
      cw.hi = uni64(cw.hi);
      const SeedExt e = extend_seed<C>(o, ref, s, lq, b.seq + qoff, cw, tbl, tbr);
      store_ext(a.ext + pos, e);
      spec_cells += e.cells;
    }
  }
  if ((threadIdx.x & 63) == 0 && spec_cells)
    atomicAdd(reinterpret_cast<unsigned long long*>(a.ctr + SPC_SPEC64), (unsigned long long)spec_cells);
}


struct PairCtx {
  int64_t rbeg, lo, hi, qoff;
  int32_t qbeg, len, lq, phase;
  int64_t rb, re;
  int32_t score, truesc, qb, qe, sc0, aw0, aw1, cells, rows, calls, pad_[2];
};
static_assert(sizeof(PairCtx) == 112, "PairCtx layout");
typedef volatile __attribute__((address_space(3))) PairCtx LdsCtx;

template <int PMAX>
__device__ __forceinline__ SeedExt extend_seed2(const DevOpt& o, const DevRef& ref, LdsCtx* cx, const uint8_t* seq,
                                                uint8_t* tbl, uint8_t* tbr) {
  {
    const int64_t rbeg = cx->rbeg, lo = cx->lo, hi = cx->hi;
    const int qbeg = cx->qbeg, len = cx->len, lq = cx->lq;
    const int qlenL = qbeg, qlenR = lq - (qbeg + len);
    const int64_t x0R = rbeg + len;
    fill_two_half(tbl, rbeg - 1, qlenL ? rows_needed(o, qlenL, (int)(rbeg - lo), o.w << 1, o.pen_clip5) : 0, tbr, x0R,
                  qlenR ? rows_needed(o, qlenR, (int)(hi - x0R), o.w << 1, o.pen_clip3) : 0, ref);
    cx->phase = qbeg != 0 ? 0 : (qlenR != 0 ? 2 : 4);
    const int sc = qbeg != 0 ? -1 : len * o.a;
    cx->score = sc;
    cx->truesc = sc;
    cx->qb = 0;
    cx->qe = lq;
    cx->sc0 = 0;
    cx->aw0 = o.w;
    cx->aw1 = o.w;
    cx->rb = rbeg;
    cx->re = rbeg + len;
    cx->cells = 0;
    cx->rows = 0;
    cx->calls = 0;
  }
  for (;;) {
    const int phase = cx->phase;
    if (phase >= 4) break;
    const int64_t rbeg = cx->rbeg;
    const int qbeg = cx->qbeg, len = cx->len, lq = cx->lq;
    const bool left = phase < 2;
    const int t = phase & 1;
    const int qlenR = lq - (qbeg + len);
    const int qlen = left ? qbeg : qlenR;
    const int64_t x0 = left ? rbeg - 1 : rbeg + len;
    const int tlen = left ? (int)(rbeg - cx->lo) : (int)(cx->hi - x0);
    const int qa = left ? qbeg - 1 : qbeg + len;
    const int eb = left ? o.pen_clip5 : o.pen_clip3;
    if (t == 0) cx->sc0 = cx->score;
    const int h0 = left ? len * o.a : cx->sc0;
    const int aw = o.w << t;
    if (left) cx->aw0 = aw;
    else cx->aw1 = aw;
    Tally32 tl{0, 0, 0};
    const ExtOut x = extend_pair_dispatch<PMAX>(o, qlen, seq + cx->qoff, qa, left ? -1 : 1, tlen, left ? tbl : tbr, aw,
                                             eb, o.zdrop, h0, tl);
    cx->cells = cx->cells + tl.cells;
    cx->rows = cx->rows + tl.rows;
    cx->calls = cx->calls + tl.calls;
    const int prev = cx->score;
    const int score = x.score;
    cx->score = score;
// ... 885 lines not shown
    }
    const bool present = r < d.ns && vchain;
    const bool computed = present && x.calls != 0;
    const uint64_t present_m = __builtin_amdgcn_ballot_w64(present);
    const uint64_t computed_m = __builtin_amdgcn_ballot_w64(computed);
    const uint64_t pad_m = __builtin_amdgcn_ballot_w64(r < d.ns && sd.pad_ != 0);
    const int rep_lim = (int)floor(.1 * d.lq) + 1;
    const int S = d.ns <= 8 ? 8 : d.ns <= 16 ? 16 : d.ns <= 32 ? 32 : 64;
    const int lgS = S == 8 ? 3 : S == 16 ? 4 : S == 32 ? 5 : 6;
    const int npass = (S * S) >> 6;
    uint32_t c_lo = 0, c_hi = 0, o_lo = 0, o_hi = 0;
    int cov = 0;
    const int j = r & (S - 1);
    const int jl = min(j, d.ns - 1) << 2;
    const int64_t j_rbeg = (int64_t)((uint64_t)(uint32_t)__builtin_amdgcn_ds_bpermute(jl, (int)(sd.rbeg >> 32)) << 32 |
                                     (uint32_t)__builtin_amdgcn_ds_bpermute(jl, (int)sd.rbeg));
    const int j_qbeg = __builtin_amdgcn_ds_bpermute(jl, sd.qbeg), j_len = __builtin_amdgcn_ds_bpermute(jl, sd.len);
    const int j_cid = __builtin_amdgcn_ds_bpermute(jl, cid);
    const bool j_pad = __builtin_amdgcn_ds_bpermute(jl, sd.pad_) != 0;
    const bool j_done = __builtin_amdgcn_ds_bpermute(jl, computed ? 1 : 0) != 0;
    RegRec pj;
    pj.rb = (int64_t)((uint64_t)(uint32_t)__builtin_amdgcn_ds_bpermute(jl, (int)(x.rb >> 32)) << 32 |
                      (uint32_t)__builtin_amdgcn_ds_bpermute(jl, (int)x.rb));
    pj.re = (int64_t)((uint64_t)(uint32_t)__builtin_amdgcn_ds_bpermute(jl, (int)(x.re >> 32)) << 32 |
                      (uint32_t)__builtin_amdgcn_ds_bpermute(jl, (int)x.re));
    pj.qb = __builtin_amdgcn_ds_bpermute(jl, x.qb);
    pj.qe = __builtin_amdgcn_ds_bpermute(jl, x.qe);
    pj.w = __builtin_amdgcn_ds_bpermute(jl, x.w);
    pj.seedlen0 = j_len;
    for (int it = 0; it < npass; ++it) {
      const int k = (it << (6 - lgS)) + (r >> lgS);
      const int kl = min(k, d.ns - 1) << 2;
      bwagpu_seed_t sk;
      sk.rbeg = (int64_t)((uint64_t)(uint32_t)__builtin_amdgcn_ds_bpermute(kl, (int)(sd.rbeg >> 32)) << 32 |
                          (uint32_t)__builtin_amdgcn_ds_bpermute(kl, (int)sd.rbeg));
      sk.qbeg = __builtin_amdgcn_ds_bpermute(kl, sd.qbeg);
      sk.len = __builtin_amdgcn_ds_bpermute(kl, sd.len);
      const int k_cid = __builtin_amdgcn_ds_bpermute(kl, cid);
      const bool valid = k < d.ns && j < d.ns;
      const bool inside = valid && j < k && j_done &&
                          !(sk.rbeg < pj.rb || sk.rbeg + sk.len > pj.re || sk.qbeg < pj.qb || sk.qbeg + sk.len > pj.qe) &&
                          !(sk.len - j_len >= rep_lim);
      uint64_t cm = __builtin_amdgcn_ballot_w64(inside);
      if (cm) cm = __builtin_amdgcn_ballot_w64(inside && seed_near(MG, sk, pj));
      const int len95 = (int)ceil(sk.len * .95);
      const bool a1 = sk.qbeg <= j_qbeg && sk.qbeg + sk.len - j_qbeg >= sk.len >> 2 &&
                      (int64_t)(j_qbeg - sk.qbeg) != j_rbeg - sk.rbeg;
      const bool b1 = j_qbeg <= sk.qbeg && j_qbeg + j_len - sk.qbeg >= sk.len >> 2 &&
                      (int64_t)(sk.qbeg - j_qbeg) != sk.rbeg - j_rbeg;
      const uint64_t om = __builtin_amdgcn_ballot_w64(valid && j < k && j_cid == k_cid && !j_pad && j_len >= len95 && (a1 || b1));
      c_lo = r == it ? (uint32_t)cm : c_lo;
      c_hi = r == it ? (uint32_t)(cm >> 32) : c_hi;
      o_lo = r == it ? (uint32_t)om : o_lo;
      o_hi = r == it ? (uint32_t)(om >> 32) : o_hi;
      if (WRITE) {
        const int64_t krb = (int64_t)((uint64_t)(uint32_t)__builtin_amdgcn_ds_bpermute(kl, (int)(x.rb >> 32)) << 32 |
                                      (uint32_t)__builtin_amdgcn_ds_bpermute(kl, (int)x.rb));
        const int64_t kre = (int64_t)((uint64_t)(uint32_t)__builtin_amdgcn_ds_bpermute(kl, (int)(x.re >> 32)) << 32 |
                                      (uint32_t)__builtin_amdgcn_ds_bpermute(kl, (int)x.re));
        const int kqb = __builtin_amdgcn_ds_bpermute(kl, x.qb), kqe = __builtin_amdgcn_ds_bpermute(kl, x.qe);
        int v = valid && j_cid == k_cid && j_qbeg >= kqb && j_qbeg + j_len <= kqe && j_rbeg >= krb &&
                        j_rbeg + j_len <= kre ? j_len : 0;
        for (int m = 1; m < S; m <<= 1) v += __shfl_xor(v, m, 64);
        const int src = (r - (it << (6 - lgS))) << lgS;
        const int got = __builtin_amdgcn_ds_bpermute(min(max(src, 0), 63) << 2, v);
        cov = (r >= (it << (6 - lgS)) && r < ((it + 1) << (6 - lgS))) ? got : cov;
      }
    }
    uint64_t ext = 0, skip = pad_m, pend = 0, spend = 0, unc = 0;
    int miss = -1;
    for (int k = 0; k < d.ns; ++k) {
      const uint64_t bit = 1ull << k;
      if (!(present_m & bit)) continue;
      const int it = (k << lgS) >> 6, sh = (k << lgS) & 63;
      const uint64_t fld = S == 64 ? ~0ull : ((1ull << S) - 1);
      const uint64_t cm = ((uint64_t)__builtin_amdgcn_readlane(c_hi, it) << 32 | (uint32_t)__builtin_amdgcn_readlane(c_lo, it)) >> sh & fld;
      if (cm & ext) {
        const uint64_t om = ((uint64_t)__builtin_amdgcn_readlane(o_hi, it) << 32 | (uint32_t)__builtin_amdgcn_readlane(o_lo, it)) >> sh & fld;
        if (!(om & ~skip)) {
          skip |= bit;
          if (MODE == SEL_EMULATE && a.emu_strict && (!(cm & ext & ~unc) || (om & unc))) {
            unc |= bit;
            if (!(computed_m & bit)) spend |= bit;
          }
          continue;
        }
      }
      if (!(computed_m & bit)) {
        if (MODE == SEL_EMULATE) {
          pend |= bit;
          unc |= bit;
          continue;
        }
        miss = k;
        break;
      }
      ext |= bit;
      if (MODE == SEL_EMULATE && pend) unc |= bit;
    }
    if constexpr (MODE == SEL_EMULATE) {
      const int list = kSpecBins + spec_bin(d.lq);
      const bool pnd = ((pend | spend) >> r) & 1;
      const int p = wave_append(&a.ctr[SPC_CNT + list], pnd);
      if (p >= 0) a.tasks[spec_list_off(list, b.n_chains, b.n_seeds) + p] = make_int2(d.s0 + r, d.c0 + cid);
      if (pend && r == 0) atomicOr(&a.rbits[rd >> 5], 1u << (rd & 31));
    } else {
      if (BWAGPU_LIGHT_INLINE && miss >= 0 && d.lq <= kSpecBinLen[0]) {
        const bwagpu_seed_t sm = uni_seed(a.prog[d.s0 + miss]);
        const int cm_id = uni(__shfl(cid, miss, 64));
        ChainWin cw = a.win[d.c0 + cm_id];
        cw.lo = uni64(cw.lo);
        cw.hi = uni64(cw.hi);
        const SeedExt e = extend_seed<3>(o, ref, sm, d.lq, b.seq + d.qoff, cw, tbl, tbr);
        store_ext(a.ext + d.s0 + miss, e);
        if (r == 0) atomicAdd(&a.ctr[SPC_MISS], 1);
        mem_fence_group();
        __builtin_amdgcn_wave_barrier();
        continue;
      }
      if (miss >= 0) {
        const int list = 2 * kSpecBins + spec_bin(d.lq);
        const int p = wave_append(&a.ctr[SPC_CNT + list], r >= miss && present && !computed);
        if (p >= 0) a.tasks[spec_list_off(list, b.n_chains, b.n_seeds) + p] = make_int2(d.s0 + r, d.c0 + cid);
        if (r == miss) a.redo[atomicAdd(&a.ctr[SPC_REDO_N], 1)] = rd;
        break;
      }
      const bool mine = (ext >> r) & 1;
      if (mine) {
        const int slot = (int)__popcll(ext & lt_mask);
        uint2* dst = reinterpret_cast<uint2*>(a.out + d.s0 + slot);
        dst[0] = make_uint2((uint32_t)x.rb, (uint32_t)((uint64_t)x.rb >> 32));
        dst[1] = make_uint2((uint32_t)x.re, (uint32_t)((uint64_t)x.re >> 32));
        dst[2] = make_uint2((uint32_t)x.qb, (uint32_t)x.qe);
        dst[3] = make_uint2((uint32_t)rid, (uint32_t)x.score);
        dst[4] = make_uint2((uint32_t)x.truesc, 0u);
        dst[5] = make_uint2(0u, 0u);
        dst[6] = make_uint2(0u, (uint32_t)x.w);
        dst[7] = make_uint2((uint32_t)cov, 0u);
        dst[8] = make_uint2(0u, (uint32_t)sd.len);
        dst[9] = make_uint2(0u, __float_as_uint(frac));
        dst[10] = make_uint2(0u, 0u);
        tl.cells += x.cells;
        tl.rows += x.rows;
        tl.calls += x.calls - 1;
      }
      if (r == 0) a.out_n[rd] = (int)__popcll(ext);
    }
    trace_read(MODE, b.n_reads, rd, t_start, d.ns, (int)__popcll(ext), 1);
    break;
    }
}

constexpr int kPackW = 8;
template <int MODE>
__device__ __forceinline__ uint64_t light_packed(const DevBatch& b, const SpecArgs& a, const int32_t* MG, int rd,
                                                 const ReadDesc& d, bool nar, Tally& tl) {
  constexpr bool WRITE = MODE != SEL_EMULATE;
  const uint64_t t_start = g_trace ? __builtin_amdgcn_s_memrealtime() : 0;
  int r = (int)(threadIdx.x & 63);
  asm volatile("" : "+v"(r));
  const int i = r & 7, g0 = r & ~7;
  const auto grp = [&](int v, int l) { return __builtin_amdgcn_ds_bpermute((g0 + l) << 2, v); };
  const auto grp64 = [&](int64_t v, int l) {
    return (int64_t)((uint64_t)(uint32_t)grp((int)(v >> 32), l) << 32 | (uint32_t)grp((int)v, l));
  };
  const auto byte_of = [&](uint64_t m) { return (uint32_t)(m >> g0) & 0xFFu; };
  const bool has_c = nar && i < d.nch, has_s = nar && i < d.ns;
  int ce_l = 15, rid_l = 0;
  float fr_l = 0.f;
  bool ok_l = false;
  if (has_c) {
    ce_l = b.chain_seed_off[d.c0 + i + 1] - d.s0;
    const ChainWin cw = a.win[d.c0 + i];
    ok_l = cw.hi >= cw.lo;
    rid_l = b.chain_rid[d.c0 + i];
    fr_l = b.chain_frac_rep[d.c0 + i];
  }
  bwagpu_seed_t sd{};
  SeedExt x{};
  if (has_s) {
    sd = a.prog[d.s0 + i];
    x = a.ext[d.s0 + i];
  }
  uint32_t ends = (uint32_t)ce_l << (4 * i);
  ends |= (uint32_t)dpp<0xB1>(0, (int)ends);
  ends |= (uint32_t)dpp<0x4E>(0, (int)ends);
  ends |= (uint32_t)dpp<0x141>(0, (int)ends);
  int cid = 0;
#pragma unroll
  for (int c = 0; c < kPackW - 1; ++c) cid += (int)((ends >> (4 * c)) & 15u) <= i;
  const bool vchain = grp(ok_l ? 1 : 0, cid) != 0;
  const int rid = grp(rid_l, cid);
  const float frac = __int_as_float(grp(__float_as_int(fr_l), cid));
  const bool present = has_s && vchain;
  const bool computed = present && x.calls != 0;
  const bool j_pad = has_s && sd.pad_ != 0;
  const uint32_t present_m = byte_of(__builtin_amdgcn_ballot_w64(present));
  const uint32_t computed_m = byte_of(__builtin_amdgcn_ballot_w64(computed));
  const uint32_t pad_m = byte_of(__builtin_amdgcn_ballot_w64(j_pad));
  const int rep_lim = (int)floor(.1 * d.lq) + 1;
  RegRec pj;
  pj.rb = x.rb;
  pj.re = x.re;
  pj.qb = x.qb;
  pj.qe = x.qe;
  pj.w = x.w;
  pj.seedlen0 = sd.len;
  uint64_t C = 0, O = 0;
  int cov = 0;
#pragma unroll 1
  for (int k = 0; k < kPackW && __builtin_amdgcn_ballot_w64(nar && k < d.ns) != 0; ++k) {
    bwagpu_seed_t sk;
    sk.rbeg = grp64(sd.rbeg, k);
    sk.qbeg = grp(sd.qbeg, k);
    sk.len = grp(sd.len, k);
    const int k_cid = grp(cid, k);
    const bool valid = has_s && k < d.ns;
    const bool inside = valid && i < k && computed &&
                        !(sk.rbeg < pj.rb || sk.rbeg + sk.len > pj.re || sk.qbeg < pj.qb || sk.qbeg + sk.len > pj.qe) &&
                        !(sk.len - sd.len >= rep_lim);
    uint64_t cm = __builtin_amdgcn_ballot_w64(inside);
    if (cm) cm = __builtin_amdgcn_ballot_w64(inside && seed_near(MG, sk, pj));
    const int len95 = (int)ceil(sk.len * .95);
    const bool a1 = sk.qbeg <= sd.qbeg && sk.qbeg + sk.len - sd.qbeg >= sk.len >> 2 &&
                    (int64_t)(sd.qbeg - sk.qbeg) != sd.rbeg - sk.rbeg;
    const bool b1 = sd.qbeg <= sk.qbeg && sd.qbeg + sd.len - sk.qbeg >= sk.len >> 2 &&
                    (int64_t)(sk.qbeg - sd.qbeg) != sk.rbeg - sd.rbeg;
    const uint64_t om = __builtin_amdgcn_ballot_w64(valid && i < k && cid == k_cid && !j_pad && sd.len >= len95 && (a1 || b1));
    C |= (uint64_t)byte_of(cm) << (8 * k);
    O |= (uint64_t)byte_of(om) << (8 * k);
    if (WRITE) {
      const int64_t krb = grp64(x.rb, k), kre = grp64(x.re, k);
      const int kqb = grp(x.qb, k), kqe = grp(x.qe, k);
      int v = valid && cid == k_cid && sd.qbeg >= kqb && sd.qbeg + sd.len <= kqe && sd.rbeg >= krb &&
                      sd.rbeg + sd.len <= kre ? sd.len : 0;
      v += dpp<0xB1>(0, v);
      v += dpp<0x4E>(0, v);
      v += dpp<0x141>(0, v);
      cov = i == k ? v : cov;
    }
  }
  uint32_t ext = 0, skip = pad_m, pend = 0, spend = 0, unc = 0;
  bool missed = false;
#pragma unroll
  for (int k = 0; k < kPackW; ++k) {
    const uint32_t bit = 1u << k;
    const uint32_t cm = (uint32_t)(C >> (8 * k)) & 0xFFu, om = (uint32_t)(O >> (8 * k)) & 0xFFu;
    const bool act = (present_m & bit) != 0 && !missed;
    const bool done = (computed_m & bit) != 0;
    const bool skp = act && (cm & ext) != 0 && !(om & ~skip);
    const bool sunc = skp && MODE == SEL_EMULATE && a.emu_strict && (!(cm & ext & ~unc) || (om & unc));
    const bool nores = act && !skp && !done;
    const bool go = act && !skp && done;
    skip |= skp ? bit : 0u;
    spend |= sunc && !done ? bit : 0u;
    if (MODE == SEL_EMULATE) {
      unc |= sunc || nores || (go && pend) ? bit : 0u;
      pend |= nores ? bit : 0u;
    } else {
      missed = missed || nores;
    }
    ext |= go ? bit : 0u;
  }
  if constexpr (MODE == SEL_EMULATE) {
    const bool pnd = nar && (((pend | spend) >> i) & 1u) != 0;
    const int bin = spec_bin(d.lq);
    for (int k = 0; k < kSpecBins; ++k) {
      const int list = kSpecBins + k;
      const int p = wave_append(&a.ctr[SPC_CNT + list], pnd && bin == k);
      if (p >= 0) a.tasks[spec_list_off(list, b.n_chains, b.n_seeds) + p] = make_int2(d.s0 + i, d.c0 + cid);
    }
    if (nar && pend && i == 0) atomicOr(&a.rbits[rd >> 5], 1u << (rd & 31));
  } else {
    const bool wr = nar && !missed;
    if (wr && ((ext >> i) & 1u)) {
      const int slot = (int)__popc(ext & ((1u << i) - 1u));
      uint2* dst = reinterpret_cast<uint2*>(a.out + d.s0 + slot);
      dst[0] = make_uint2((uint32_t)x.rb, (uint32_t)((uint64_t)x.rb >> 32));
      dst[1] = make_uint2((uint32_t)x.re, (uint32_t)((uint64_t)x.re >> 32));
      dst[2] = make_uint2((uint32_t)x.qb, (uint32_t)x.qe);
      dst[3] = make_uint2((uint32_t)rid, (uint32_t)x.score);
      dst[4] = make_uint2((uint32_t)x.truesc, 0u);
      dst[5] = make_uint2(0u, 0u);
      dst[6] = make_uint2(0u, (uint32_t)x.w);
      dst[7] = make_uint2((uint32_t)cov, 0u);
      dst[8] = make_uint2(0u, (uint32_t)sd.len);
      dst[9] = make_uint2(0u, __float_as_uint(frac));
      dst[10] = make_uint2(0u, 0u);
      tl.cells += x.cells;
      tl.rows += x.rows;
      tl.calls += x.calls - 1;
    }
    if (wr && i == 0) a.out_n[rd] = (int)__popc(ext);
  }
  if (uint32_t* const tr = g_trace) {
    const uint64_t t_end = __builtin_amdgcn_s_memrealtime();
    uint32_t v = 1u;
    v = i == 0 ? (uint32_t)t_start : v;
    v = i == 1 ? (uint32_t)(t_start >> 32) : v;
    v = i == 2 ? (uint32_t)t_end : v;
    v = i == 3 ? (uint32_t)(t_end >> 32) : v;
    v = i == 4 ? (uint32_t)d.ns : v;
    v = i == 5 ? (uint32_t)__popc(ext) : v;
    v = i == 6 ? __builtin_amdgcn_s_getreg((31 << 11) | 20) : v;
    if (nar && !missed) tr[((size_t)MODE * b.n_reads + rd) * 8 + i] = v;
  }
  return __builtin_amdgcn_ballot_w64(nar && missed);
}

template <int MODE>
__global__ void __launch_bounds__(kBlock) spec_select_light(DevOpt o, DevRef ref, DevBatch b, SpecArgs a,
                                                            int tb_bytes) {
  sel_prio();
  constexpr bool WRITE = MODE != SEL_EMULATE;
  __shared__ int32_t MG[kMglN];
  extern __shared__ __attribute__((aligned(16))) uint8_t lrows[];
  uint8_t* const tbl = lrows + (threadIdx.x >> 6) * 2 * tb_bytes;
  uint8_t* const tbr = tbl + tb_bytes;
  constexpr int kLightList = 64;
  __shared__ int32_t WL[kBlock / 64][kLightList];
  int32_t* const wl = WL[threadIdx.x >> 6];
  for (int x = threadIdx.x; x < kMglN; x += kBlock) MG[x] = max_gap_len(o, x);
  __syncthreads();
  const int r = (int)(threadIdx.x & 63);
  Tally tl{0, 0, 0};
  const int NW = (int)gridDim.x * (kBlock / 64);
  const int w0 = (int)blockIdx.x * (kBlock / 64) + uni((int)(threadIdx.x >> 6));
  constexpr int kLightChunk = 16;
  int ph = 0, cb = 0, ce = 0, pbase = w0 - 64 * NW;
  uint64_t pm = 0;
  const auto risky = [&](int x) { return ((a.rbits[x >> 5] >> (x & 31)) & 1u) != 0; };
  const auto next_read = [&]() -> int {
    if (ph == 0) {
      for (;;) {
        if (pm) {
          const int i = __builtin_ctzll(pm);
          pm &= pm - 1;
          return pbase + i * NW;
        }
        pbase += 64 * NW;
        if (pbase >= b.n_reads) break;
        const int x = pbase + r * NW;
        pm = __builtin_amdgcn_ballot_w64(x < b.n_reads && risky(x));
      }
      ph = 1;
    }
    for (;;) {
      if (cb >= ce) {
        int c = 0;
        if (r == 0) c = atomicAdd(&a.ctr[SPC_LIGHT_CUR], kLightChunk);
        c = __builtin_amdgcn_readfirstlane(__shfl(c, 0, 64));
        if (c >= b.n_reads) return b.n_reads;
        cb = c;
        ce = min(c + kLightChunk, b.n_reads);
      }
      const int y = cb++;
      if (!risky(y)) return y;
    }
  };
  const bool dyn = MODE == SEL_FINAL && a.risky_first;
  const bool pack = a.light_pack && !dyn;
  const int n_units = pack ? (b.n_reads + kPackW - 1) / kPackW : b.n_reads;
  const int unit_reads = pack ? kPackW : dyn ? 1 : 64;
  const uint64_t first_lanes = pack ? 0x0101010101010101ull : dyn ? 1ull : ~0ull;
  const auto lane_read = [&](int u) { return pack ? kPackW * u + (r >> 3) : dyn ? u : u + r * NW; };
  const uint64_t lt_mask = r ? (~0ull >> (64 - r)) : 0ull;
  int un = dyn ? next_read() : w0;
  while (un < n_units) {
    int nw = 0;
    ReadDesc dn{};
    if (lane_read(un) < b.n_reads) dn = a.rdesc[lane_read(un)];
    while (un < n_units && nw + unit_reads <= kLightList) {
      const ReadDesc d = dn;
      const int rd = lane_read(un);
      un = dyn ? next_read() : pack ? un + NW : un + 64 * NW;
      if (un < n_units && lane_read(un) < b.n_reads) dn = a.rdesc[lane_read(un)];
      const bool mine = rd < b.n_reads && !(d.ns > kSelLight || d.nch > kSelLight) && !(d.lq > a.lq_bound);
      const bool nar = pack && mine && d.ns <= kPackW && d.nch <= kPackW;
      if (WRITE && mine && !nar && d.ns == 0) a.out_n[rd] = 0;
      uint64_t wide = __builtin_amdgcn_ballot_w64(mine && !nar && d.ns != 0);
      if (pack) wide |= light_packed<MODE>(b, a, MG, rd, d, nar, tl);
      wide &= first_lanes;
      if ((wide >> r) & 1) wl[nw + (int)__popcll(wide & lt_mask)] = rd;
      nw += (int)__popcll(wide);
    }
    __builtin_amdgcn_fence(__ATOMIC_RELEASE, "wavefront");
    __builtin_amdgcn_wave_barrier();
    __builtin_amdgcn_fence(__ATOMIC_ACQUIRE, "wavefront");
    ReadDesc wn{};
    if (nw) wn = a.rdesc[uni(wl[0])];
    for (int k = 0; k < nw; ++k) {
      const ReadDesc u = uniform_desc(wn);
      const int rd = uni(wl[k]);
      if (k + 1 < nw) wn = a.rdesc[uni(wl[k + 1])];
      light_read<MODE>(o, ref, b, a, MG, tbl, tbr, rd, u, tl);
    }
    __builtin_amdgcn_fence(__ATOMIC_RELEASE, "wavefront");
    __builtin_amdgcn_wave_barrier();
    __builtin_amdgcn_fence(__ATOMIC_ACQUIRE, "wavefront");
  }
  if constexpr (WRITE) block_stats<64>(tl, a.stats);
}

template <int MODE>
__global__ void __launch_bounds__(kBlock) spec_pairs_kernel(DevOpt o, DevBatch b, SpecArgs a) {
  sel_prio();
  __shared__ int32_t MG[kMglN];
  for (int x = threadIdx.x; x < kMglN; x += kBlock) MG[x] = max_gap_len(o, x);
  __syncthreads();
  const int r = (int)(threadIdx.x & 63);
  const int ncol = uni(__hip_atomic_load(&a.ctr[SPC_HCOLS], __ATOMIC_RELAXED, __HIP_MEMORY_SCOPE_AGENT));
  const int nwv = (int)gridDim.x * (kBlock / 64);
  int x = (int)blockIdx.x * (kBlock / 64) + uni((int)(threadIdx.x >> 6));
  if (x >= ncol) return;
  int4 hi = a.hinfo[uni(a.colent[x])];
  for (; x < ncol; x += nwv) {
    const int tn = uni(a.colent[min(x + nwv, ncol - 1)]);
    const int rd = uni(hi.x), woff = uni(hi.y), col = uni(hi.z), ns = uni(hi.w);
    const int k = x - col, nw = (ns + 63) >> 6;
    const int nlow = (k + 63) >> 6;
    const ReadDesc d = uniform_desc(a.rdesc[rd]);
    const int rep_lim = (int)floor(.1 * d.lq) + 1;
    const bwagpu_seed_t s = uni_seed(a.prog[d.s0 + k]);
    const int ck = uni(a.seedchain[d.s0 + k]);
    const int len95 = uni((int)ceil(s.len * .95));
    const SeedExt ek = a.ext[d.s0 + k];
    const bool k_cov = uni(ek.calls) != 0 && (MODE == SEL_EMULATE || uni(a.cov[d.s0 + k]) < 0);
    const int64_t krb = uni64(ek.rb), kre = uni64(ek.re);
    const int kqb = uni(ek.qb), kqe = uni(ek.qe);
    const int4 hin = a.hinfo[tn];
    const ChainWin wk = a.win[ck];
    if (r == 0)
      a.hflag[d.s0 + k] = (uni64(wk.hi) >= uni64(wk.lo) ? 1 : 0) | (uni(ek.calls) != 0 ? 2 : 0) | (s.pad_ != 0 ? 4 : 0);
    int cov = 0;
    bwagpu_seed_t sj{};
    int cj = 0;
    SeedExt ej{};
    if (nlow > 0) {
      const int jj = min(r, ns - 1);
      sj = a.prog[d.s0 + jj];
      cj = a.seedchain[d.s0 + jj];
      ej = a.ext[d.s0 + jj];
    }
    for (int w = 0; w < nlow; ++w) {
      const bwagpu_seed_t sc = sj;
      const int cc = cj;
      const SeedExt ec = ej;
      if (w + 1 < nlow) {
        const int jj = min(64 * (w + 1) + r, ns - 1);
        sj = a.prog[d.s0 + jj];
        cj = a.seedchain[d.s0 + jj];
        ej = a.ext[d.s0 + jj];
      }
      const int j = 64 * w + r;
      RegRec p;
      p.rb = ec.rb;
      p.re = ec.re;
      p.qb = ec.qb;
      p.qe = ec.qe;
      p.w = ec.w;
      p.seedlen0 = sc.len;
      const bool inside = j < k && ec.calls != 0 &&
                          !(s.rbeg < p.rb || s.rbeg + s.len > p.re || s.qbeg < p.qb || s.qbeg + s.len > p.qe) &&
                          !(s.len - sc.len >= rep_lim);
      uint64_t cm = __builtin_amdgcn_ballot_w64(inside);
      if (cm) cm = __builtin_amdgcn_ballot_w64(inside && seed_near(MG, s, p));
      if (r == 0) a.mat[woff + tri_off(k) + w] = cm;
      if (MODE == SEL_EMULATE) {
        const bool a1 = s.qbeg <= sc.qbeg && s.qbeg + s.len - sc.qbeg >= s.len >> 2 &&
                        (int64_t)(sc.qbeg - s.qbeg) != sc.rbeg - s.rbeg;
        const bool b1 = sc.qbeg <= s.qbeg && sc.qbeg + sc.len - s.qbeg >= s.len >> 2 &&
                        (int64_t)(s.qbeg - sc.qbeg) != s.rbeg - sc.rbeg;
        const uint64_t om =
            __builtin_amdgcn_ballot_w64(j < k && cc == ck && sc.pad_ == 0 && sc.len >= len95 && (a1 || b1));
        if (r == 0) a.mat[woff + tri_off(ns) + tri_off(k) + w] = om;
      }
      if (k_cov)
        cov += (j < ns && cc == ck && sc.qbeg >= kqb && sc.qbeg + sc.len <= kqe && sc.rbeg >= krb &&
                sc.rbeg + sc.len <= kre) ? sc.len : 0;
    }
    if (k_cov) {
      for (int w = nlow; w < nw; ++w) {
        const int j = 64 * w + r, jj = min(j, ns - 1);
        const bwagpu_seed_t sc = a.prog[d.s0 + jj];
        const int cc = a.seedchain[d.s0 + jj];
        cov += (j < ns && cc == ck && sc.qbeg >= kqb && sc.qbeg + sc.len <= kqe && sc.rbeg >= krb &&
                sc.rbeg + sc.len <= kre) ? sc.len : 0;
      }
      cov = (int)grp_sum64(cov, 64);
      if (r == 0) a.cov[d.s0 + k] = cov;
    } else if (MODE == SEL_EMULATE) {
      if (r == 0) a.cov[d.s0 + k] = -1;
    }
    hi = hin;
  }
}

__device__ __forceinline__ uint64_t lane64(uint64_t v, int l) { return (uint64_t)readlane64((int64_t)v, l); }

constexpr int kScanLds = 64 * 1024;

__device__ __forceinline__ void heavy_fill_missing(const DevOpt& o, const DevRef& ref, const DevBatch& b,
                                                   const SpecArgs& a, const ReadDesc& d, int k, int ns,
                                                   uint64_t* C, uint8_t* tbl, uint8_t* tbr) {
  const int r = (int)(threadIdx.x & 63);
  const bwagpu_seed_t sk = uni_seed(a.prog[d.s0 + k]);
  const int ck = uni(a.seedchain[d.s0 + k]);
  ChainWin cw = a.win[ck];
  cw.lo = uni64(cw.lo);
  cw.hi = uni64(cw.hi);
  const SeedExt e = d.lq <= 192 ? extend_seed<3>(o, ref, sk, d.lq, b.seq + d.qoff, cw, tbl, tbr)
                                 : extend_seed<4>(o, ref, sk, d.lq, b.seq + d.qoff, cw, tbl, tbr);
  store_ext(a.ext + d.s0 + k, e);
  if (r == 0) atomicAdd(&a.ctr[SPC_MISS], 1);
  RegRec p;
  p.rb = e.rb;
  p.re = e.re;
  p.qb = e.qb;
  p.qe = e.qe;
  p.w = e.w;
  p.seedlen0 = sk.len;
  const int rep_lim = (int)floor(.1 * d.lq) + 1;
  int cov = 0;
  for (int base = 0; base < ns; base += 64) {
    const int j = base + r, jj = min(j, ns - 1);
    const bwagpu_seed_t sj = a.prog[d.s0 + jj];
    bool in = j > k && j < ns && !(sj.rbeg < p.rb || sj.rbeg + sj.len > p.re || sj.qbeg < p.qb || sj.qbeg + sj.len > p.qe) &&
              !(sj.len - sk.len >= rep_lim);
    if (in) {
      const int qd1 = sj.qbeg - p.qb;
      const int64_t rd1 = sj.rbeg - p.rb;
      const int g1 = max_gap_len(o, max(qd1 < rd1 ? qd1 : (int)rd1, 0));
      const int bw1 = g1 < p.w ? g1 : p.w;
      const int qd2 = p.qe - (sj.qbeg + sj.len);
      const int64_t rd2 = p.re - (sj.rbeg + sj.len);
// ... 103 lines not shown
              if (MODE == SEL_EMULATE) is_pend = is_unc = true;
              else is_lack = true;
            } else {
              is_ext = true;
              is_unc = strict && (fp < k || (pn & lt_mask));
            }
          }
          const uint64_t e1 = __builtin_amdgcn_ballot_w64(is_ext), sk1 = skp0 | __builtin_amdgcn_ballot_w64(is_skip);
          uint64_t pn1 = 0, sp1 = 0, un1 = 0, lack1 = 0;
          if (MODE == SEL_EMULATE) {
            pn1 = __builtin_amdgcn_ballot_w64(is_pend);
            if (strict) {
              sp1 = __builtin_amdgcn_ballot_w64(is_spend);
              un1 = __builtin_amdgcn_ballot_w64(is_unc);
            }
          } else {
            lack1 = __builtin_amdgcn_ballot_w64(is_lack);
          }
          const bool same = e1 == e && sk1 == sk && pn1 == pn && sp1 == sp && un1 == un && lack1 == lack;
          e = e1, sk = sk1, pn = pn1, sp = sp1, un = un1, lack = lack1;
          if (same) {
            resolved = lack == 0;
            break;
          }
        }
        if (resolved) {
          ext = e, skp = sk, pend = pn, spend = sp;
          uncb = strict ? un : pn;
          if (pn) fp = min(fp, kb + (int)__builtin_ctzll(pn));
        }
      }
      const uint64_t cbm = resolved ? 0 : __builtin_amdgcn_ballot_w64(valid && cb);
      uint64_t obm = resolved ? 0 : __builtin_amdgcn_ballot_w64(valid && ob);
      const uint64_t cbcm = resolved ? 0 : __builtin_amdgcn_ballot_w64(valid && cbc);
      const uint64_t oum = resolved ? 0 : __builtin_amdgcn_ballot_w64(valid && ou);
      for (int i = 0; i < (resolved ? 0 : nb); ++i) {
        const uint64_t bit = 1ull << i;
        if (!(pres & bit)) continue;
        if ((cbm & bit) || (lane64(cin, i) & ext)) {
          if (!(obm & bit) && !(lane64(oin, i) & ~skp)) {
            skp |= bit;
            if (strict && (!((cbcm & bit) || (lane64(cin, i) & ext & ~uncb)) || (oum & bit) || (lane64(oin, i) & uncb))) {
              uncb |= bit;
              if (!(comp & bit)) spend |= bit;
            }
            continue;
          }
        }
        if (!(comp & bit)) {
          if (MODE == SEL_EMULATE) {
            pend |= bit;
            uncb |= bit;
            fp = min(fp, kb + i);
            continue;
          }
          if (d.lq > kSpecBinLen[1]) {
            miss = kb + i;
            break;
          }
          heavy_fill_missing(o, ref, b, a, d, kb + i, ns, C, tbl, tbr);
          comp |= bit;
          cin = valid && r > 0 ? C[row + bw] : 0;
          const bool fresh = valid && !need && cin != 0;
          if (__builtin_amdgcn_ballot_w64(fresh)) {
            if (fresh) {
              for (int w = 0; w < bw; ++w) ob |= (O[row + w] & ~lane64(skip_w, w)) != 0;
              oin = O[row + bw];
            }
            need = need || fresh;
            obm = __builtin_amdgcn_ballot_w64(valid && ob);
          }
        }
        ext |= bit;
        if (strict && fp < kb + i) uncb |= bit;
      }
      ext_w = r == bw ? ext : ext_w;
      skip_w = r == bw ? skp : skip_w;
      pend_w = r == bw ? pend | spend : pend_w;
      unc_w = r == bw ? uncb : unc_w;
      computed_w = r == bw ? comp : computed_w;
    }
    int nreg = 0;
    if constexpr (MODE == SEL_EMULATE) {
      const int list = kSpecBins + spec_bin(d.lq);
      const int tot = (int)grp_sum64(r < nw ? (int)__popcll(pend_w) : 0, 64);
      if (tot) {
        int off = 0;
        if (r == 0) off = atomicAdd(&a.ctr[SPC_CNT + list], tot);
        off = __builtin_amdgcn_readfirstlane(off);
        for (int w = 0; w < nw; ++w) {
          const uint64_t pw = lane64(pend_w, w);
          const int j = 64 * w + r;
          if ((pw >> r) & 1)
            a.tasks[spec_list_off(list, b.n_chains, b.n_seeds) + off + (int)__popcll(pw & lt_mask)] =
                make_int2(d.s0 + j, a.seedchain[d.s0 + j]);
          off += (int)__popcll(pw);
        }
      }
    } else {
      if (miss >= 0) {
        if (r == 0) {
          const int list = 2 * kSpecBins + spec_bin(d.lq);
          const int p = atomicAdd(&a.ctr[SPC_CNT + list], 1);
          a.tasks[spec_list_off(list, b.n_chains, b.n_seeds) + p] = make_int2(d.s0 + miss, a.seedchain[d.s0 + miss]);
          a.redo[atomicAdd(&a.ctr[SPC_REDO_N], 1)] = rd;
        }
        continue;
      }
      for (int w = 0; w < nw; ++w) {
        const uint64_t ew = (uint64_t)__builtin_amdgcn_readlane((uint32_t)(ext_w >> 32), w) << 32 |
                            (uint32_t)__builtin_amdgcn_readlane((uint32_t)ext_w, w);
        const int j = 64 * w + r;
        if ((ew >> r) & 1) {
          const int slot = nreg + (int)__popcll(ew & lt_mask);
          const SeedExt x = a.ext[d.s0 + j];
          const int c = a.seedchain[d.s0 + j];
          uint2* dst = reinterpret_cast<uint2*>(a.out + d.s0 + slot);
          dst[0] = make_uint2((uint32_t)x.rb, (uint32_t)((uint64_t)x.rb >> 32));
          dst[1] = make_uint2((uint32_t)x.re, (uint32_t)((uint64_t)x.re >> 32));
          dst[2] = make_uint2((uint32_t)x.qb, (uint32_t)x.qe);
          dst[3] = make_uint2((uint32_t)b.chain_rid[c], (uint32_t)x.score);
          dst[4] = make_uint2((uint32_t)x.truesc, 0u);
          dst[5] = make_uint2(0u, 0u);
          dst[6] = make_uint2(0u, (uint32_t)x.w);
          dst[7] = make_uint2((uint32_t)a.cov[d.s0 + j], 0u);
          dst[8] = make_uint2(0u, (uint32_t)a.prog[d.s0 + j].len);
          dst[9] = make_uint2(0u, __float_as_uint(b.chain_frac_rep[c]));
          dst[10] = make_uint2(0u, 0u);
          tl.cells += x.cells;
          tl.rows += x.rows;
          tl.calls += x.calls - 1;
        }
        nreg += (int)__popcll(ew);
      }
      if (r == 0) a.out_n[rd] = nreg;
    }
    trace_read(MODE, b.n_reads, rd, t_start, ns, nreg, 3);
  }
  if constexpr (WRITE) block_stats<64>(tl, a.stats);
}

constexpr int kScanGrid = 1024;

#ifndef BWAGPU_LIGHT_PACK_DEFAULT
#define BWAGPU_LIGHT_PACK_DEFAULT 1
#endif
int light_pack_default() {
  static const int v = [] {
    const char* e = getenv("BWAGPU_LIGHT_PACK");
    return e && e[0] ? (atoi(e) != 0 ? 1 : 0) : BWAGPU_LIGHT_PACK_DEFAULT;
  }();
  return v;
}
#ifndef BWAGPU_LIGHT_PACK_WGS_DEFAULT
#define BWAGPU_LIGHT_PACK_WGS_DEFAULT 2
#endif
static int light_pack_wgs() {
  static const int v = [] {
    const char* e = getenv("BWAGPU_LIGHT_PACK_WGS");
    return std::min(std::max(e && e[0] ? atoi(e) : BWAGPU_LIGHT_PACK_WGS_DEFAULT, 1), 64);
  }();
  return v;
}
static int device_cus() {
  int dev = 0, ncu = 0;
  if (hipGetDevice(&dev) != hipSuccess ||
      hipDeviceGetAttribute(&ncu, hipDeviceAttributeMultiprocessorCount, dev) != hipSuccess || ncu < 1)
    return 256;
  return ncu;
}

template <int MODE>
static void launch_select(const DevOpt& o, const DevRef& ref, const DevBatch& b, const SpecArgs& a, int tb_bytes,
                          hipStream_t st, const SpecStreams& ss) {
  hipStream_t hs = st;
  if (MODE != SEL_REDO && ss.side) {
    (void)hipEventRecord(ss.fork, st);
    (void)hipStreamWaitEvent(ss.side, ss.fork, 0);
    hs = ss.side;
  }
  if (MODE != SEL_REDO) {
    const size_t lds = BWAGPU_LIGHT_INLINE && MODE == SEL_FINAL ? (size_t)(kBlock / 64) * 2 * tb_bytes : 0;
    int nb = resident_blocks(spec_select_light<MODE>, lds);
    if (a.light_pack && !(MODE == SEL_FINAL && a.risky_first)) {
      const int octets = (b.n_reads + kPackW - 1) / kPackW, per_wg = kBlock / 64;
      nb = std::min(nb, std::max(1, std::min((octets + per_wg - 1) / per_wg, light_pack_wgs() * device_cus())));
    }
    hipLaunchKernelGGL((spec_select_light<MODE>), dim3(nb), dim3(kBlock), lds, st, o, ref, b, a, tb_bytes);
  }
  if (MODE != SEL_REDO) {
    const int nb = resident_blocks(spec_pairs_kernel<MODE>, 0);
    hipLaunchKernelGGL((spec_pairs_kernel<MODE>), dim3(nb), dim3(kBlock), 0, hs, o, b, a);
    hipLaunchKernelGGL((spec_scan_kernel<MODE>), dim3(kScanGrid), dim3(64), (size_t)kScanLds + 2 * (size_t)tb_bytes, hs, o,
                       ref, b, a, tb_bytes);
  }
  hipLaunchKernelGGL((spec_select_kernel<MODE, true>), dim3(MODE == SEL_REDO ? 256 : 1024), dim3(64),
                     (size_t)kSelHeavyLds, hs, o, ref, b, a, tb_bytes);
  if (hs != st) {
    (void)hipEventRecord(ss.join, hs);
    (void)hipStreamWaitEvent(st, ss.join, 0);
  }
}

static std::atomic<int> g_ext_form{0};
int ext_kernel_for(const DevOpt& o, int form, int tb_bytes) { return ext_plan(o, form, tb_bytes, 0).bin[0].code; }
int set_ext_form(int form) {
  const int prev = g_ext_form.load(std::memory_order_relaxed);
  if (form >= 0) g_ext_form.store(form > 2 ? 1 : form, std::memory_order_relaxed);
  return prev;
}

#ifndef BWAGPU_EXT_SHORT_Q_DEFAULT
#define BWAGPU_EXT_SHORT_Q_DEFAULT 63
#endif
int ext_short_default() {
  static const int q = [] {
    const char* e = getenv("BWAGPU_EXT_SHORT_Q");
    const int v = e && e[0] ? atoi(e) : BWAGPU_EXT_SHORT_Q_DEFAULT;
    return std::min(std::max(v, 0), kShortQMax);
  }();
  return q;
}
#ifndef BWAGPU_EXT_SHORT_FILL_DEFAULT
#define BWAGPU_EXT_SHORT_FILL_DEFAULT 150
#endif
int ext_short_fill_default() {
  static const int f = [] {
    const char* e = getenv("BWAGPU_EXT_SHORT_FILL");
    return std::min(std::max(e && e[0] ? atoi(e) : BWAGPU_EXT_SHORT_FILL_DEFAULT, 0), 100000);
  }();
  return f;
}


static void launch_sort(const ExtBin& k, const ExtRound& r, int bin0, int nbins, int short_q) {
  if (k.phased) launch_side_sort(r, bin0, nbins, short_q);
  else launch_task_sort(r, bin0, nbins);
}
static void launch_ext_bin(const ExtBin& k, const ExtRound& r, int list, const ExtPlan& p, int short_fill) {
  if (k.family == SIDE4) launch_side_bin(k, r, list, p, short_fill);
  else launch_task_bin(k, r, list, p.quad);
}

static void launch_ext_round(const DevOpt& o, const DevRef& ref, const DevBatch& b, const SpecArgs& a, int round,
                             int tb_bytes, int lq_max, hipStream_t st, const SpecStreams& ss) {
  const int l = round * kSpecBins;
  const bool bin1 = lq_max > kSpecBinLen[0], bin2 = lq_max > kSpecBinLen[1];
  const ExtPlan plan = ext_plan(o, ss.form, tb_bytes, ss.short_q);
  const ExtRound r{o, ref, b, a, round, tb_bytes, st};
  if (!bin1 || plan.bin[0].phased == plan.bin[1].phased) {
    launch_sort(plan.bin[0], r, 0, bin1 ? 2 : 1, plan.short_q);
  } else {
    launch_sort(plan.bin[0], r, 0, 1, plan.short_q);
    launch_sort(plan.bin[1], r, 1, 1, 0);
  }
  const bool prof = ss.pool && *ss.pool_used + 2 <= ss.pool_n;
  if (prof) (void)hipEventRecord(ss.pool[*ss.pool_used], st);
  launch_ext_bin(plan.bin[0], r, l + 0, plan, ss.short_fill);
  if (prof) {
    (void)hipEventRecord(ss.pool[*ss.pool_used + 1], st);
    *ss.pool_used += 2;
  }
  if (!bin1) return;
  launch_ext_bin(plan.bin[1], r, l + 1, plan, ss.short_fill);
  if (bin2) launch_task_long(r, l + 2);
}

hipError_t launch_spec_chain2aln(const DevOpt& o, const DevRef& ref, const DevBatch& b, const SpecArgs& a,
                                 int tb_bytes, int lq_max, hipStream_t st, const SpecStreams& ss) {
  if (b.n_reads == 0) return hipSuccess;
  hipLaunchKernelGGL(spec_reads_kernel, dim3((b.n_reads + 255) / 256), dim3(256), 0, st, b, a);
  if (b.n_chains) {
    hipLaunchKernelGGL(spec_chain_kernel, dim3((b.n_chains + 255) / 256), dim3(256), 0, st, o, ref, b, a);
    hipLaunchKernelGGL(spec_order_kernel, dim3(kOrderBlocks), dim3(256), 0, st, o, ref, b, a);
  }
  if (b.n_chains) {
    launch_ext_round(o, ref, b, a, 0, tb_bytes, lq_max, st, ss);
    launch_select<SEL_EMULATE>(o, ref, b, a, tb_bytes, st, ss);
    launch_ext_round(o, ref, b, a, 1, tb_bytes, lq_max, st, ss);
  }
  launch_select<SEL_FINAL>(o, ref, b, a, tb_bytes, st, ss);
  if (b.n_chains && lq_max > kSpecBinLen[0] && !a.emu_strict) launch_ext_round(o, ref, b, a, 2, tb_bytes, lq_max, st, ss);
  if (b.n_chains) launch_select<SEL_REDO>(o, ref, b, a, tb_bytes, st, ss);
  return hipGetLastError();
}

__global__ void __launch_bounds__(256) spec_clear_kernel(SpecArgs a, int nr, int ns) {
  const int t0 = (int)(blockIdx.x * 256 + threadIdx.x), nt = (int)(gridDim.x * 256);
  switch (blockIdx.y) {
    case 0:
      for (int i = t0; i < 3 * ns; i += nt) reinterpret_cast<uint4*>(a.ext)[i] = make_uint4(0, 0, 0, 0);
      break;
    case 1:
      for (int i = t0; i < nr; i += nt) a.out_n[i] = 0;
      break;
    case 2:
      for (int i = t0; i < nr / 32 + 1; i += nt) a.rbits[i] = 0;
      break;
    case 3:
      for (int i = t0; i < kQHWords; i += nt) a.qh[i] = 0;
      break;
    case 4:
      for (int i = t0; i < kSortWords; i += nt) a.sorth[i] = 0;
      break;
    default:
      for (int i = t0; i < SPC_WORDS; i += nt) a.ctr[i] = 0;
  }
}
static_assert(sizeof(SeedExt) == 48, "spec_clear_kernel clears SeedExt as three uint4");

hipError_t launch_spec_clear(const SpecArgs& a, int n_reads, int n_seeds, hipStream_t st) {
  hipLaunchKernelGGL(spec_clear_kernel, dim3(256, 6), dim3(256), 0, st, a, n_reads, n_seeds);
  return hipGetLastError();
}

size_t spec_select_lds(int tb_bytes) { return (size_t)kSelHeavyLds + 0 * tb_bytes; }
int spec_redo_cap(int tb_bytes) { return sel_heavy_cap(SEL_REDO, tb_bytes); }

}
```

### bwa-flow_amd/python/bwagpu/abi.py

```python
from __future__ import annotations

import ctypes as C
import os

import numpy as np

HERE = os.path.dirname(os.path.abspath(__file__))
PKG_ROOT = os.path.normpath(os.path.join(HERE, "..", ".."))
REPO_ROOT = os.path.normpath(os.path.join(PKG_ROOT, ".."))
LIB_DIR = os.path.join(PKG_ROOT, "lib")

ABI_VERSION = 1
OK, E_INVAL, E_NOMEM, E_DEVICE, E_HANG, E_RESULTS, E_UNSUPPORTED, E_NODEVICE = range(8)
ERR_NAMES = {
    OK: "OK", E_INVAL: "E_INVAL", E_NOMEM: "E_NOMEM", E_DEVICE: "E_DEVICE", E_HANG: "E_HANG",
    E_RESULTS: "E_RESULTS", E_UNSUPPORTED: "E_UNSUPPORTED", E_NODEVICE: "E_NODEVICE",
}
MAX_READ_LEN = 1023
NUM_SLOTS = 4

SEED_DTYPE = np.dtype([("rbeg", "<i8"), ("qbeg", "<i4"), ("len", "<i4"), ("score", "<i4"),
                       ("pad", "<i4")])
ALNREG_DTYPE = np.dtype([
    ("rb", "<i8"), ("re", "<i8"), ("qb", "<i4"), ("qe", "<i4"), ("rid", "<i4"), ("score", "<i4"),
# ... 20 lines not shown
assert EXT_TASK_DTYPE.itemsize == 40 and EXT_RES_DTYPE.itemsize == 24


class Opt(C.Structure):
    _fields_ = [("a", C.c_int32), ("b", C.c_int32), ("o_del", C.c_int32), ("e_del", C.c_int32),
                ("o_ins", C.c_int32), ("e_ins", C.c_int32), ("pen_clip5", C.c_int32),
                ("pen_clip3", C.c_int32), ("w", C.c_int32), ("zdrop", C.c_int32),
                ("mat", C.c_int8 * 25), ("pad_", C.c_int8 * 3)]


class Bns(C.Structure):
    _fields_ = [("l_pac", C.c_int64), ("n_seqs", C.c_int32), ("pad_", C.c_int32),
                ("ann_offset", C.c_void_p), ("ann_len", C.c_void_p)]


class BatchC(C.Structure):
    _fields_ = [("n_reads", C.c_int32), ("n_chains", C.c_int32), ("n_seeds", C.c_int32),
                ("pad_", C.c_int32), ("seq_bytes", C.c_int64), ("seq_off", C.c_void_p),
                ("seq", C.c_void_p), ("read_chain_off", C.c_void_p), ("chain_seed_off", C.c_void_p),
                ("chain_rid", C.c_void_p), ("chain_frac_rep", C.c_void_p), ("seeds", C.c_void_p)]


class Stats(C.Structure):
    _fields_ = [("kernel_ms", C.c_double), ("total_ms", C.c_double), ("cells", C.c_int64),
                ("rows", C.c_int64), ("ext_calls", C.c_int64), ("h2d_bytes", C.c_int64),
                ("d2h_bytes", C.c_int64)]


class BwtC(C.Structure):
    _fields_ = [("primary", C.c_uint64), ("L2", C.c_uint64 * 5), ("seq_len", C.c_uint64),
                ("bwt_size", C.c_uint64), ("bwt", C.c_void_p), ("sa_intv", C.c_int32), ("pad_", C.c_int32),
                ("n_sa", C.c_uint64), ("sa", C.c_void_p)]


class SeedOpt(C.Structure):
    _fields_ = [("min_seed_len", C.c_int32), ("split_width", C.c_int32), ("max_mem_intv", C.c_int32),
                ("split_factor", C.c_float)]


INTV_DTYPE = np.dtype([("x", "<u8", (3,)), ("info", "<u8")])
assert INTV_DTYPE.itemsize == 32

CHAIN_DTYPE = np.dtype([("pos", "<i8"), ("rid", "<i4"), ("n", "<i4"), ("w", "<i4"), ("kept", "<i4"),
                        ("first", "<i4"), ("is_alt", "<i4"), ("frac_rep", "<f4"), ("pad_", "<i4")])
assert CHAIN_DTYPE.itemsize == 40


class ChainOpt(C.Structure):
    _fields_ = [("max_occ", C.c_int32), ("max_chain_gap", C.c_int32), ("min_chain_weight", C.c_int32),
                ("max_chain_extend", C.c_int32), ("mask_level", C.c_float), ("drop_ratio", C.c_float)]


class ChainsC(C.Structure):
    _fields_ = [("n_reads", C.c_int32), ("n_chains", C.c_int32), ("n_seeds", C.c_int64),
                ("read_chain_off", C.c_void_p), ("chain_seed_off", C.c_void_p), ("chains", C.c_void_p),
                ("seeds", C.c_void_p)]


class PostOpt(C.Structure):
    _fields_ = [("max_chain_gap", C.c_int32), ("mask_level_redun", C.c_float), ("mask_level", C.c_float),
                ("pad_", C.c_int32)]


POST_DEDUP_PATCH, POST_MARK_ALT, POST_PRIMARY = 1, 2, 4


def default_postopt() -> PostOpt:
    return PostOpt(10000, 0.95, 0.50, 0)


class PairOpt(C.Structure):
    _fields_ = [("max_ins", C.c_int32), ("max_matesw", C.c_int32), ("pen_unpaired", C.c_int32),
                ("min_seed_len", C.c_int32), ("max_chain_gap", C.c_int32), ("mask_level_redun", C.c_float),
                ("mask_level", C.c_float), ("max_rounds", C.c_int32)]


def default_pairopt() -> PairOpt:
    return PairOpt(10000, 50, 17, 19, 10000, 0.95, 0.50, 3)


PESTAT_DTYPE = np.dtype([("low", "<i4"), ("high", "<i4"), ("failed", "<i4"), ("pad", "<i4"), ("avg", "<f8"),
                         ("std", "<f8")])
assert PESTAT_DTYPE.itemsize == 32 and C.sizeof(PairOpt) == 32
RESCUE_DONE, RESCUE_UNFINISHED, RESCUE_OVERFLOW, RESCUE_UNSUPPORTED = 0, 1, 2, 3


class SelOpt(C.Structure):
    _fields_ = [("T", C.c_int32), ("pen_unpaired", C.c_int32), ("min_seed_len", C.c_int32),
                ("mapQ_coef_len", C.c_float), ("mapQ_coef_fac", C.c_int32), ("mask_level", C.c_float),
                ("drop_ratio", C.c_float), ("flags", C.c_int32)]


def default_selopt(flags: int = 0) -> SelOpt:
    return SelOpt(30, 17, 19, 50.0, 3, 0.50, 0.50, int(flags))


MEM_F_NOPAIRING, MEM_F_ALL, MEM_F_NO_MULTI, MEM_F_PRIMARY5, MEM_F_KEEP_SUPP_MAPQ = 0x4, 0x8, 0x10, 0x800, 0x1000
SEL_MAX_REGS = 512
SEL_DONE, SEL_TOO_MANY, SEL_SKIPPED = 0, 1, 2
SEL_NO_PAIRING, SEL_PAIRED = 0, 1
PAIRSEL_DTYPE = np.dtype([("status", "<i4"), ("branch", "<i4"), ("n_pri", "<i4", (2,)), ("z", "<i4", (2,)),
                          ("mapq", "<i4", (2,)), ("alt", "<i4", (2,)), ("extra_flag", "<i4"), ("o", "<i4"),
                          ("subo", "<i4"), ("n_sub", "<i4"), ("pad", "<i4", (2,))])
assert PAIRSEL_DTYPE.itemsize == 64 and C.sizeof(SelOpt) == 32


def default_chainopt() -> dict:
    return dict(max_occ=500, max_chain_gap=10000, min_chain_weight=0, max_chain_extend=1 << 30, mask_level=0.5,
                drop_ratio=0.5)

_VP = C.c_void_p
PROTOS = {
    "bwagpu_abi_version": (C.c_int, []),
    "bwagpu_device_count": (C.c_int, [C.POINTER(C.c_int)]),
    "bwagpu_create": (C.c_int, [C.c_int, C.POINTER(Opt), C.POINTER(Bns), _VP, C.POINTER(_VP)]),
    "bwagpu_create_resident": (C.c_int, [C.c_int, C.POINTER(Opt), C.POINTER(Bns), _VP, C.POINTER(_VP)]),
    "bwagpu_destroy": (C.c_int, [_VP]),
    "bwagpu_last_error": (C.c_char_p, [_VP]),
    "bwagpu_set_watchdog_ms": (C.c_int, [_VP, C.c_int]),
    "bwagpu_chain2aln_submit": (C.c_int, [_VP, C.c_int, C.POINTER(BatchC)]),
    "bwagpu_chain2aln_wait": (C.c_int, [_VP, C.c_int, _VP, _VP]),
    "bwagpu_chain2aln_stage": (C.c_int, [_VP, C.c_int, C.c_int32, C.c_int32, C.c_int32, C.c_int64,
                                         C.POINTER(BatchC)]),
    "bwagpu_chain2aln_results": (C.c_int, [_VP, C.c_int, C.POINTER(_VP), C.POINTER(_VP)]),
    "bwagpu_chain2aln_results_dense": (C.c_int, [_VP, C.c_int, C.POINTER(_VP), C.POINTER(_VP), C.POINTER(_VP)]),
    "bwagpu_chain2aln": (C.c_int, [_VP, C.POINTER(BatchC), _VP, _VP]),
    "bwagpu_chain2aln_device": (C.c_int, [_VP, C.POINTER(BatchC), _VP, _VP, _VP, _VP]),
    "bwagpu_extend_batch": (C.c_int, [_VP, C.c_int32, _VP, _VP, C.c_int64, _VP, C.c_int64, _VP]),
    "bwagpu_align2_batch": (C.c_int, [_VP, C.c_int32, _VP, _VP, C.c_int64, _VP, C.c_int64, _VP]),
    "bwagpu_align2_device": (C.c_int, [_VP, C.c_int32, _VP, _VP, _VP, _VP, _VP, _VP]),
    "bwagpu_reg2aln_batch": (C.c_int, [_VP, C.c_int32, _VP, _VP, C.c_int64, C.c_int32, C.c_int32, _VP, _VP, _VP]),
    "bwagpu_reg2aln_device": (C.c_int, [_VP, C.c_int32, _VP, _VP, _VP, C.c_int64, C.c_int32, C.c_int32, _VP, _VP,
                                        _VP, _VP]),
    "bwagpu_reg2aln_jobs_device": (C.c_int, [_VP, C.c_int32, _VP, _VP, _VP, _VP, _VP, C.c_int32, _VP, _VP, _VP, _VP]),
    "bwagpu_debug_reg2aln_times": (C.c_int, [_VP, _VP]),
    "bwagpu_last_stats": (C.c_int, [_VP, C.c_int, C.POINTER(Stats)]),
    "bwagpu_debug_set_trace": (C.c_int, [_VP, _VP]),
    "bwagpu_prof_start": (C.c_int, [_VP, C.c_int]),
    "bwagpu_debug_fail_wait": (C.c_int, [_VP, C.c_int, C.c_int]),
    "bwagpu_debug_spec_counters": (C.c_int, [_VP, _VP, _VP]),
    "bwagpu_debug_occupancy": (C.c_int, [_VP, _VP, _VP]),
    "bwagpu_debug_spec_ext": (C.c_int, [_VP, _VP, _VP, C.c_int32]),
    "bwagpu_prof_read": (C.c_int, [_VP, C.POINTER(C.c_double), C.POINTER(C.c_int32)]),
    "bwagpu_prof_intervals": (C.c_int, [_VP, _VP, _VP, C.c_int32, C.POINTER(C.c_int32)]),
    "bwagpu_set_bwt": (C.c_int, [_VP, C.POINTER(BwtC)]),
    "bwagpu_debug_seed_budget": (C.c_int, [_VP, C.c_int32]),
    "bwagpu_debug_sup_shift": (C.c_int, [_VP, C.c_int32]),
    "bwagpu_set_device_read_len": (C.c_int, [_VP, C.c_int32]),
    "bwagpu_debug_ext_form": (C.c_int, [C.c_int]),
    "bwagpu_ctx_ext_form": (C.c_int, [_VP, C.c_int]),
    "bwagpu_ctx_ext_short": (C.c_int, [_VP, C.c_int]),
    "bwagpu_ctx_ext_short_fill": (C.c_int, [_VP, C.c_int]),
    "bwagpu_ctx_light_pack": (C.c_int, [_VP, C.c_int]),
    "bwagpu_debug_spec_short": (C.c_int, [_VP, _VP, _VP]),
    "bwagpu_ctx_row_bound": (C.c_int, [_VP, C.c_int]),
    "bwagpu_debug_ext_kernel": (C.c_int, [_VP, C.c_int32]),
    "bwagpu_streams_concurrent": (C.c_int, [_VP, _VP]),
    "bwagpu_bwt_sa": (C.c_int, [_VP, C.c_int64, _VP, _VP]),
    "bwagpu_sw_stream": (C.c_int, [_VP, _VP, C.c_int64, _VP, C.c_int32, C.POINTER(C.c_int32)]),
    "bwagpu_collect_intv": (C.c_int, [_VP, C.POINTER(SeedOpt), C.c_int32, _VP, _VP, C.c_int32, _VP, C.c_int64,
                                       _VP]),
    "bwagpu_set_alt": (C.c_int, [_VP, _VP]),
    "bwagpu_seqs2chains": (C.c_int, [_VP, C.POINTER(SeedOpt), C.POINTER(ChainOpt), C.c_int32, _VP, _VP, C.c_int32,
                                      C.POINTER(ChainsC)]),
    "bwagpu_seqs2regions": (C.c_int, [_VP, C.POINTER(SeedOpt), C.POINTER(ChainOpt), C.c_int32, _VP, _VP, _VP,
                                       C.POINTER(_VP), C.POINTER(C.c_int64)]),
    "bwagpu_regs_post": (C.c_int, [_VP, C.POINTER(PostOpt), C.c_int32, C.c_int64, C.c_int32, _VP, _VP, _VP, _VP,
                                    _VP]),
    "bwagpu_regs_post_device": (C.c_int, [_VP, C.POINTER(PostOpt), C.c_int32, C.c_int64, C.POINTER(BatchC), _VP,
                                           _VP, _VP, _VP]),
    "bwagpu_set_regs_post": (C.c_int, [_VP, C.POINTER(PostOpt), C.c_int32, C.c_int64]),
    "bwagpu_pestat": (C.c_int, [_VP, C.POINTER(PairOpt), C.c_int32, _VP, _VP, _VP, _VP]),
    "bwagpu_pestat_device": (C.c_int, [_VP, C.POINTER(PairOpt), C.c_int32, _VP, _VP, _VP, _VP, _VP]),
    "bwagpu_mate_rescue": (C.c_int, [_VP, C.POINTER(PairOpt), _VP, C.c_int32, _VP, _VP, _VP, _VP, _VP, _VP, _VP, _VP,
                                      _VP, _VP]),
    "bwagpu_mate_rescue_device": (C.c_int, [_VP, C.POINTER(PairOpt), _VP, C.POINTER(BatchC), _VP, _VP, _VP, _VP, _VP,
                                             _VP, _VP, _VP, _VP]),
    "bwagpu_mark_primary": (C.c_int, [_VP, C.POINTER(SelOpt), C.c_int64, C.c_int32, _VP, _VP, _VP, _VP, _VP]),
    "bwagpu_mark_primary_device": (C.c_int, [_VP, C.POINTER(SelOpt), C.c_int64, C.c_int32, _VP, _VP, _VP, _VP, _VP,
                                              _VP]),
    "bwagpu_pair_select": (C.c_int, [_VP, C.POINTER(SelOpt), _VP, C.c_int64, C.c_int32, _VP, _VP, _VP, _VP, _VP, _VP,
                                      _VP]),
    "bwagpu_pair_select_device": (C.c_int, [_VP, C.POINTER(SelOpt), _VP, C.c_int64, C.c_int32, _VP, _VP, _VP, _VP,
                                             _VP, _VP, _VP, _VP]),
    "bwagpu_debug_rescue_drop": (C.c_int, [_VP, C.c_int32]),
    "bwagpu_debug_rescue_times": (C.c_int, [_VP, _VP]),
}

_lib = None


def lib_path() -> str:
    return os.environ.get("BWAGPU_LIB", os.path.join(LIB_DIR, "libbwagpu.so"))


def load() -> C.CDLL:
    global _lib
    if _lib is not None:
        return _lib
    p = lib_path()
    if os.environ.get("BWAGPU_NO_TORCH") != "1":
        try:
            import torch
        except Exception:
            pass
    if not os.path.exists(p):
        raise RuntimeError(f"bwagpu: HIP engine library missing at {p}; run __graft_entry__.build()")
    lib = C.CDLL(p)
    for name, (res, args) in PROTOS.items():
        if (name.startswith("bwagpu_debug_") or name == "bwagpu_ctx_light_pack") and not hasattr(lib, name):
            continue
        fn = getattr(lib, name)
        fn.restype = res
        fn.argtypes = args
    if lib.bwagpu_abi_version() != ABI_VERSION:
        raise RuntimeError("bwagpu: ABI version mismatch")
    _lib = lib
    return lib


def opt_from_dict(d: dict) -> Opt:
    o = Opt()
    for k in ("a", "b", "o_del", "e_del", "o_ins", "e_ins", "pen_clip5", "pen_clip3", "w", "zdrop"):
        setattr(o, k, int(d[k]))
    mat = d.get("mat")
    if mat is None:
        mat = fill_scmat(int(d["a"]), int(d["b"]))
    for i in range(25):
        o.mat[i] = int(mat[i])
    return o


def fill_scmat(a: int, b: int) -> np.ndarray:
    m = np.full((5, 5), -1, np.int8)
    for i in range(4):
        for j in range(4):
            m[i, j] = a if i == j else -b
    return m.reshape(-1)


def default_opt() -> dict:
    return dict(a=1, b=4, o_del=6, e_del=1, o_ins=6, e_ins=1, pen_clip5=5, pen_clip3=5, w=100,
                zdrop=100, mat=fill_scmat(1, 4))
```

### bwa-flow_amd/python/bwagpu/engine.py

```python
from __future__ import annotations

import ctypes as C
from dataclasses import dataclass

import numpy as np

from . import abi


class BwaGpuError(RuntimeError):
    def __init__(self, code: int, msg: str):
        super().__init__(f"{abi.ERR_NAMES.get(code, code)}: {msg}")
        self.code = code


def _ptr(a: np.ndarray | None):
    return None if a is None or a.size == 0 else a.ctypes.data_as(C.c_void_p)


@dataclass
class Batch:
    seq_off: np.ndarray
    seq: np.ndarray
    read_chain_off: np.ndarray
# ... 130 lines not shown
        self._check(self.lib.bwagpu_chain2aln_submit(self.ctx, slot, C.byref(bc)), "submit")

    def wait(self, slot: int, batch: Batch, out=None):
        if out is None:
            regs = np.zeros(max(batch.n_seeds, 1), abi.ALNREG_DTYPE)
            n = np.zeros(max(batch.n_reads, 1), np.int32)
        else:
            regs, n = out
            if (regs.dtype != abi.ALNREG_DTYPE or n.dtype != np.int32 or not regs.flags.c_contiguous
                    or not n.flags.c_contiguous or len(regs) < max(batch.n_seeds, 1) or len(n) < max(batch.n_reads, 1)):
                raise ValueError("wait: out arrays too small or of the wrong dtype/layout")
        self._check(self.lib.bwagpu_chain2aln_wait(self.ctx, slot, _ptr(regs), _ptr(n)), "wait")
        return regs[:batch.n_seeds], n[:batch.n_reads]

    def wait_dense(self, slot: int, batch: Batch, out=None):
        self._check(self.lib.bwagpu_chain2aln_wait(self.ctx, slot, None, None), "wait")
        rp, np_, op = C.c_void_p(), C.c_void_p(), C.c_void_p()
        self._check(self.lib.bwagpu_chain2aln_results_dense(self.ctx, slot, C.byref(rp), C.byref(np_), C.byref(op)),
                    "results_dense")
        nr = batch.n_reads
        if nr == 0:
            return np.zeros(0, abi.ALNREG_DTYPE), np.zeros(0, np.int32)
        cnt = np.ctypeslib.as_array(C.cast(np_, C.POINTER(C.c_int32)), (nr,))
        tot = int(np.ctypeslib.as_array(C.cast(op, C.POINTER(C.c_int32)), (nr + 1,))[nr])
        view = (np.ctypeslib.as_array(C.cast(rp, C.POINTER(C.c_uint8)), (tot * abi.ALNREG_DTYPE.itemsize,))
                .view(abi.ALNREG_DTYPE) if tot else np.zeros(0, abi.ALNREG_DTYPE))
        if out is None:
            return view, cnt
        regs, n = out
        if len(regs) < tot or len(n) < nr:
            raise ValueError("wait_dense: out arrays too small")
        n[:nr] = cnt
        regs[:tot] = view
        return regs[:tot], n[:nr]

    def chain2aln_device(self, dev_batch: abi.BatchC, dev_out: int, dev_n: int, dev_stats: int | None,
                         stream: int | None):
        self._check(self.lib.bwagpu_chain2aln_device(self.ctx, C.byref(dev_batch), C.c_void_p(dev_out),
                                                     C.c_void_p(dev_n),
                                                     C.c_void_p(dev_stats) if dev_stats else None,
                                                     C.c_void_p(stream) if stream else None),
                    "chain2aln_device")

    def extend_batch(self, tasks: np.ndarray, qpool: np.ndarray, tpool: np.ndarray) -> np.ndarray:
        tasks = np.ascontiguousarray(tasks, abi.EXT_TASK_DTYPE)
        qpool = np.ascontiguousarray(qpool, np.uint8)
        tpool = np.ascontiguousarray(tpool, np.uint8)
        res = np.zeros(max(len(tasks), 1), abi.EXT_RES_DTYPE)
        self._check(self.lib.bwagpu_extend_batch(self.ctx, len(tasks), _ptr(tasks), _ptr(qpool), len(qpool),
                                                 _ptr(tpool), len(tpool), _ptr(res)), "extend_batch")
        return res[:len(tasks)]

    def align2_batch(self, tasks: np.ndarray, qpool: np.ndarray, tpool: np.ndarray) -> np.ndarray:
        tasks = np.ascontiguousarray(tasks, abi.ALIGN2_TASK_DTYPE)
        qpool = np.ascontiguousarray(qpool, np.uint8)
        tpool = np.ascontiguousarray(tpool, np.uint8)
        res = np.zeros(max(len(tasks), 1), abi.KSWR_DTYPE)
        self._check(self.lib.bwagpu_align2_batch(self.ctx, len(tasks), _ptr(tasks), _ptr(qpool), len(qpool),
                                                 _ptr(tpool), len(tpool), _ptr(res)), "align2_batch")
        return res[:len(tasks)]

    def align2_device(self, n: int, dev_tasks: int, dev_q: int, dev_t: int, dev_out: int, dev_scratch: int,
                      stream: int | None = None):
        self._check(self.lib.bwagpu_align2_device(self.ctx, n, dev_tasks, dev_q, dev_t, dev_out, dev_scratch,
                                                  stream), "align2_device")

    def reg2aln_batch(self, tasks: np.ndarray, qpool: np.ndarray, max_ops: int = 64, max_md: int = 512):
        tasks = np.ascontiguousarray(tasks, abi.REG2ALN_TASK_DTYPE)
        qpool = np.ascontiguousarray(qpool, np.uint8)
        n = len(tasks)
        out = np.zeros(max(n, 1), abi.ALN_DTYPE)
        cig = np.zeros((max(n, 1), max_ops), np.uint32)
        md = np.zeros((max(n, 1), max_md), np.uint8)
        self._check(self.lib.bwagpu_reg2aln_batch(self.ctx, n, _ptr(tasks), _ptr(qpool), len(qpool), max_ops, max_md,
                                                  _ptr(out), _ptr(cig), _ptr(md)), "reg2aln_batch")
        return out[:n], cig[:n], md[:n]

    def reg2aln_device(self, n_cap: int, dev_tasks: int, dev_qpool: int, qpool_len: int, dev_out: int,
                       dev_cigar: int, dev_md: int, max_ops: int = 64, max_md: int = 512,
                       dev_n_tasks: int | None = None, stream: int | None = None):
        self._check(self.lib.bwagpu_reg2aln_device(
            self.ctx, int(n_cap), C.c_void_p(dev_n_tasks) if dev_n_tasks else None, C.c_void_p(dev_tasks),
            C.c_void_p(dev_qpool) if dev_qpool else None, int(qpool_len), int(max_ops), int(max_md),
            C.c_void_p(dev_out), C.c_void_p(dev_cigar), C.c_void_p(dev_md),
            C.c_void_p(stream) if stream else None), "reg2aln_device")

    def reg2aln_jobs_device(self, n_reads: int, dev_reg_off: int, dev_regs: int, dev_n: int, dev_select: int,
                            dev_seq_off: int, job_cap: int, dev_tasks: int, dev_job_of: int, dev_n_jobs: int,
                            stream: int | None = None):
        self._check(self.lib.bwagpu_reg2aln_jobs_device(
            self.ctx, int(n_reads), C.c_void_p(dev_reg_off), C.c_void_p(dev_regs), C.c_void_p(dev_n),
            C.c_void_p(dev_select), C.c_void_p(dev_seq_off), int(job_cap),
            C.c_void_p(dev_tasks) if dev_tasks else None, C.c_void_p(dev_job_of), C.c_void_p(dev_n_jobs),
            C.c_void_p(stream) if stream else None), "reg2aln_jobs_device")

    def debug_reg2aln_times(self) -> dict:
        out = np.zeros(4, np.float64)
        self._check(self.lib.bwagpu_debug_reg2aln_times(self.ctx, _ptr(out)), "debug_reg2aln_times")
        return dict(wait_ms=float(out[0]), bins_ms=float(out[1]), call_ms=float(out[2]), jobs=int(out[3]))

    def set_bwt(self, hdr, words, sa=None, sa_intv: int = 32):
        hdr = np.asarray(hdr, np.int64)
        self._bwt_words = np.ascontiguousarray(words, np.uint32)
        self._bwt_sa = None if sa is None else np.ascontiguousarray(sa, np.uint64)
        b = abi.BwtC()
        b.primary = int(hdr[0])
        for i in range(5):
            b.L2[i] = int(hdr[1 + i])
        b.seq_len = int(hdr[6])
        b.bwt_size = len(self._bwt_words)
        b.bwt = self._bwt_words.ctypes.data
        if self._bwt_sa is not None:
            b.sa_intv = sa_intv
            b.n_sa = len(self._bwt_sa)
            b.sa = self._bwt_sa.ctypes.data
        self._check(self.lib.bwagpu_set_bwt(self.ctx, C.byref(b)), "set_bwt")

    def bwt_sa(self, ks) -> np.ndarray:
        ks = np.ascontiguousarray(ks, np.uint64)
        out = np.zeros(max(len(ks), 1), np.uint64)
        self._check(self.lib.bwagpu_bwt_sa(self.ctx, len(ks), _ptr(ks), _ptr(out)), "bwt_sa")
        return out[:len(ks)]

    def sw_stream(self, words: np.ndarray, cap_tasks: int) -> np.ndarray:
        words = np.ascontiguousarray(words, np.int32)
        out = np.zeros((max(cap_tasks, 1), 10), np.int16)
        n = C.c_int32(0)
        self._check(self.lib.bwagpu_sw_stream(self.ctx, _ptr(words), len(words), _ptr(out), int(cap_tasks),
                                              C.byref(n)), "sw_stream")
        return out[:n.value]

    EXT_KERNELS = {2: "spec_ext2_kernel<5>",
                   18: "spec_side4_kernel<16, 10, true>", 14: "spec_side4_kernel<32, 5, true>",
                   15: "spec_side4_kernel<32, 8, false>"}

    def ext_kernel(self, lq_max: int = 256) -> str:
        k = self.lib.bwagpu_debug_ext_kernel(self.ctx, int(lq_max))
        if k not in self.EXT_KERNELS:
            raise BwaGpuError(k, "debug_ext_kernel")
        return self.EXT_KERNELS[k]

    def ext_form(self, form: int = -1) -> int:
        return self.lib.bwagpu_ctx_ext_form(self.ctx, int(form))

    def ext_short(self, q: int = -1) -> int:
        return self.lib.bwagpu_ctx_ext_short(self.ctx, int(q))

    def ext_short_fill(self, percent: int = -1) -> int:
        return self.lib.bwagpu_ctx_ext_short_fill(self.ctx, int(percent))

    def light_pack(self, on: int = -1) -> int:
        return self.lib.bwagpu_ctx_light_pack(self.ctx, int(on))

    def row_bound(self, on: int = -1) -> int:
        return self.lib.bwagpu_ctx_row_bound(self.ctx, int(on))

    def set_device_read_len(self, max_len: int):
        self._check(self.lib.bwagpu_set_device_read_len(self.ctx, int(max_len)), "set_device_read_len")

    def sup_shift(self, shift: int):
        self._check(self.lib.bwagpu_debug_sup_shift(self.ctx, shift), "sup_shift")

    def seed_budget(self, budget: int):
        self._check(self.lib.bwagpu_debug_seed_budget(self.ctx, budget), "seed_budget")

    def collect_intv(self, seq_off: np.ndarray, seq: np.ndarray, min_seed_len: int = 19, split_width: int = 10,
                     max_mem_intv: int = 20, split_factor: float = 1.5, max_per_read: int = 256,
                     out_cap: int | None = None, out: np.ndarray | None = None):
        seq_off = np.ascontiguousarray(seq_off, np.int64)
        seq = np.ascontiguousarray(seq, np.uint8)
        n = len(seq_off) - 1
        o = abi.SeedOpt(min_seed_len, split_width, max_mem_intv, split_factor)
        if out is not None:
            if out.dtype != abi.INTV_DTYPE or not out.flags.c_contiguous:
                raise ValueError("out must be a contiguous INTV_DTYPE array")
            cap = len(out)
        else:
            cap = max(n, 1) * max_per_read if out_cap is None else out_cap
            out = np.zeros(max(cap, 1), abi.INTV_DTYPE)
        cnt = np.zeros(max(n, 1), np.int32)
        self._check(self.lib.bwagpu_collect_intv(self.ctx, C.byref(o), n, _ptr(seq_off), _ptr(seq), max_per_read,
                                                 _ptr(out), cap, _ptr(cnt)), "collect_intv")
        cnt = cnt[:n]
        return cnt, out[:int(cnt.sum())]

    def set_alt(self, is_alt):
        self._alt = None if is_alt is None else np.ascontiguousarray(is_alt, np.uint8)
        self._check(self.lib.bwagpu_set_alt(self.ctx, None if self._alt is None else _ptr(self._alt)), "set_alt")

    @staticmethod
    def _seed_chain_opts(seedopt, split_factor, chainopt):
        so = np.asarray(seedopt, np.int32)
        co = abi.default_chainopt() if chainopt is None else chainopt
        return (abi.SeedOpt(int(so[0]), int(so[1]), int(so[2]), float(split_factor)),
                abi.ChainOpt(int(co["max_occ"]), int(co["max_chain_gap"]), int(co["min_chain_weight"]),
                             int(co["max_chain_extend"]), float(co["mask_level"]), float(co["drop_ratio"])))

    def seqs2chains(self, seq_off, seq, seedopt=(19, 10, 20), split_factor: float = 1.5, chainopt: dict | None = None,
                    raw: bool = False, copy: bool = True):
        seq_off = np.ascontiguousarray(seq_off, np.int64)
        seq = np.ascontiguousarray(seq, np.uint8)
        n = len(seq_off) - 1
        so, co = self._seed_chain_opts(seedopt, split_factor, chainopt)
        out = abi.ChainsC()
        self._check(self.lib.bwagpu_seqs2chains(self.ctx, C.byref(so), C.byref(co), n, _ptr(seq_off), _ptr(seq),
                                                int(raw), C.byref(out)), "seqs2chains")
        nc, ns = out.n_chains, out.n_seeds

        def view(p, dt, k):
            if k == 0:
                return np.zeros(0, dt)
            v = np.frombuffer((C.c_char * (k * np.dtype(dt).itemsize)).from_address(p), dt)
            return v.copy() if copy else v
        return (view(out.read_chain_off, np.int32, n + 1), view(out.chains, abi.CHAIN_DTYPE, nc),
                view(out.chain_seed_off, np.int32, nc + 1), view(out.seeds, abi.SEED_DTYPE, ns))

    def seqs2regions(self, seq_off, seq, seedopt=(19, 10, 20), split_factor: float = 1.5,
                     chainopt: dict | None = None, copy: bool = True):
        seq_off = np.ascontiguousarray(seq_off, np.int64)
        seq = np.ascontiguousarray(seq, np.uint8)
        n = len(seq_off) - 1
        so, co = self._seed_chain_opts(seedopt, split_factor, chainopt)
        cnt = np.zeros(max(n, 1), np.int32)
        regs, nreg = C.c_void_p(), C.c_int64()
        self._check(self.lib.bwagpu_seqs2regions(self.ctx, C.byref(so), C.byref(co), n, _ptr(seq_off), _ptr(seq),
                                                 _ptr(cnt), C.byref(regs), C.byref(nreg)), "seqs2regions")
        k = nreg.value
        out = np.zeros(0, abi.ALNREG_DTYPE) if k == 0 else np.frombuffer(
            (C.c_char * (k * abi.ALNREG_DTYPE.itemsize)).from_address(regs.value), abi.ALNREG_DTYPE)
        return cnt[:n], (out.copy() if copy else out)

    def regs_post(self, seq_off, seq, reg_off, regs, n, flags: int, id0: int = 0, popt: abi.PostOpt | None = None):
        seq_off = np.ascontiguousarray(seq_off, np.int64)
        seq = np.ascontiguousarray(seq, np.uint8)
        reg_off = np.ascontiguousarray(reg_off, np.int64)
        regs = np.array(regs, abi.ALNREG_DTYPE, order="C")
        n = np.array(n, np.int32, order="C")
        nr = len(seq_off) - 1
        if len(reg_off) < nr or len(n) < nr:
            raise ValueError("regs_post: reg_off / n shorter than the batch")
        po = abi.default_postopt() if popt is None else popt
        self._check(self.lib.bwagpu_regs_post(self.ctx, C.byref(po), int(flags), int(id0), nr, _ptr(seq_off),
                                              _ptr(seq), _ptr(reg_off), _ptr(regs), _ptr(n)), "regs_post")
        return regs, n

    def regs_post_device(self, dev_batch: abi.BatchC, dev_reg_off: int | None, dev_regs: int, dev_n: int,
                         flags: int, id0: int = 0, popt: abi.PostOpt | None = None, stream: int | None = None):
        po = abi.default_postopt() if popt is None else popt
        self._check(self.lib.bwagpu_regs_post_device(self.ctx, C.byref(po), int(flags), int(id0), C.byref(dev_batch),
                                                     C.c_void_p(dev_reg_off) if dev_reg_off else None,
                                                     C.c_void_p(dev_regs), C.c_void_p(dev_n),
                                                     C.c_void_p(stream) if stream else None), "regs_post_device")

    def set_regs_post(self, flags: int, id0: int = 0, popt: abi.PostOpt | None = None):
        po = abi.default_postopt() if popt is None else popt
        self._check(self.lib.bwagpu_set_regs_post(self.ctx, C.byref(po), int(flags), int(id0)), "set_regs_post")

    def pestat(self, reg_off, regs, n, popt: abi.PairOpt | None = None) -> np.ndarray:
        reg_off = np.ascontiguousarray(reg_off, np.int64)
        regs = np.ascontiguousarray(regs, abi.ALNREG_DTYPE)
        n = np.ascontiguousarray(n, np.int32)
        if len(reg_off) != len(n):
            raise ValueError("pestat: reg_off and n differ in length")
        po = abi.default_pairopt() if popt is None else popt
        pes = np.zeros(4, abi.PESTAT_DTYPE)
        self._check(self.lib.bwagpu_pestat(self.ctx, C.byref(po), len(n), _ptr(reg_off), _ptr(regs), _ptr(n),
                                           _ptr(pes)), "pestat")
        return pes

    def pestat_device(self, n_reads: int, dev_reg_off: int, dev_regs: int, dev_n: int, dev_pes: int,
                      popt: abi.PairOpt | None = None, stream: int | None = None):
        po = abi.default_pairopt() if popt is None else popt
        self._check(self.lib.bwagpu_pestat_device(self.ctx, C.byref(po), int(n_reads), C.c_void_p(dev_reg_off),
                                                  C.c_void_p(dev_regs), C.c_void_p(dev_n), C.c_void_p(dev_pes),
                                                  C.c_void_p(stream) if stream else None), "pestat_device")

    def mate_rescue(self, pes, seq_off, seq, reg_off, regs, n, out_off, popt: abi.PairOpt | None = None):
        pes = np.ascontiguousarray(pes, abi.PESTAT_DTYPE)
        seq_off = np.ascontiguousarray(seq_off, np.int64)
        seq = np.ascontiguousarray(seq, np.uint8)
        reg_off = np.ascontiguousarray(reg_off, np.int64)
        regs = np.ascontiguousarray(regs, abi.ALNREG_DTYPE)
        n = np.ascontiguousarray(n, np.int32)
        out_off = np.ascontiguousarray(out_off, np.int64)
        nr = len(seq_off) - 1
        if len(pes) != 4 or len(reg_off) < nr or len(n) < nr or len(out_off) != nr + 1:
            raise ValueError("mate_rescue: pes / reg_off / n / out_off do not fit the batch")
        po = abi.default_pairopt() if popt is None else popt
        out = np.zeros(max(int(out_off[-1]), 1), abi.ALNREG_DTYPE)
        out_n = np.zeros(max(nr, 1), np.int32)
        status = np.zeros(max(nr // 2, 1), np.int32)
        n_sw = np.zeros(max(nr // 2, 1), np.int32)
        self._check(self.lib.bwagpu_mate_rescue(self.ctx, C.byref(po), _ptr(pes), nr, _ptr(seq_off), _ptr(seq),
                                                _ptr(reg_off), _ptr(regs), _ptr(n), _ptr(out_off), _ptr(out),
                                                _ptr(out_n), _ptr(status), _ptr(n_sw)), "mate_rescue")
        return out, out_n[:nr], status[:nr // 2], n_sw[:nr // 2]

    def mate_rescue_device(self, dev_pes: int, dev_batch: abi.BatchC, dev_reg_off: int, dev_regs: int, dev_n: int,
                           dev_out_off: int, dev_out_regs: int, dev_out_n: int, dev_status: int, dev_n_sw: int,
                           popt: abi.PairOpt | None = None, stream: int | None = None):
        po = abi.default_pairopt() if popt is None else popt
        self._check(self.lib.bwagpu_mate_rescue_device(
            self.ctx, C.byref(po), C.c_void_p(dev_pes), C.byref(dev_batch), C.c_void_p(dev_reg_off),
            C.c_void_p(dev_regs), C.c_void_p(dev_n), C.c_void_p(dev_out_off), C.c_void_p(dev_out_regs),
            C.c_void_p(dev_out_n), C.c_void_p(dev_status), C.c_void_p(dev_n_sw),
            C.c_void_p(stream) if stream else None), "mate_rescue_device")
# ... 84 lines not shown
```

### include/bwagpu_debug.h

```cpp
#ifndef BWAGPU_DEBUG_H
#define BWAGPU_DEBUG_H
#include "bwagpu.h"

#ifdef __cplusplus
extern "C" {
#endif

int bwagpu_debug_seed_budget(bwagpu_ctx_t *ctx, int32_t budget);

int bwagpu_debug_sup_shift(bwagpu_ctx_t *ctx, int32_t shift);

int bwagpu_debug_set_trace(bwagpu_ctx_t *ctx, void *dev_ptr);
int bwagpu_debug_fail_wait(bwagpu_ctx_t *ctx, int after_n_waits, int code);

int bwagpu_prof_start(bwagpu_ctx_t *ctx, int max_launches);
int bwagpu_debug_spec_counters(bwagpu_ctx_t *ctx, void *stream, int64_t *out);
int bwagpu_debug_occupancy(bwagpu_ctx_t *ctx, void *stream, int64_t *out);
int bwagpu_debug_spec_ext(bwagpu_ctx_t *ctx, void *stream, void *host_out, int32_t n);
int bwagpu_prof_read(bwagpu_ctx_t *ctx, double *total_ms, int32_t *launches);
int bwagpu_debug_ext_form(int form);
int bwagpu_ctx_ext_form(bwagpu_ctx_t *ctx, int form);
int bwagpu_ctx_ext_short(bwagpu_ctx_t *ctx, int q);
int bwagpu_ctx_ext_short_fill(bwagpu_ctx_t *ctx, int percent);
int bwagpu_ctx_light_pack(bwagpu_ctx_t *ctx, int on);
int bwagpu_debug_spec_short(bwagpu_ctx_t *ctx, void *stream, int64_t *out);
int bwagpu_ctx_row_bound(bwagpu_ctx_t *ctx, int on);
int bwagpu_debug_ext_kernel(bwagpu_ctx_t *ctx, int32_t lq_max);
int bwagpu_streams_concurrent(void *a, void *b);
int bwagpu_debug_rescue_drop(bwagpu_ctx_t *ctx, int32_t k);
int bwagpu_debug_rescue_times(bwagpu_ctx_t *ctx, double *out);
int bwagpu_debug_reg2aln_times(bwagpu_ctx_t *ctx, double *out);
int bwagpu_prof_intervals(bwagpu_ctx_t *ctx, double *start_ms, double *end_ms, int32_t max, int32_t *n);

#ifdef __cplusplus
}
#endif
#endif
```

Measured before the change: 64.52.

## Bin light reads by seed width into quad/oct/wide work units

```diff
diff --git a/bwa-flow_amd/csrc/capi.hip b/bwa-flow_amd/csrc/capi.hip
--- a/bwa-flow_amd/csrc/capi.hip
+++ b/bwa-flow_amd/csrc/capi.hip
@@ -241,6 +241,7 @@
   ctx->ext_short = ext_short_default();
   ctx->ext_short_fill = ext_short_fill_default();
   ctx->light_pack = light_pack_default();
+  ctx->light_class = light_class_default();
   *made = ctx;
   HIPC(hipSetDevice(device), "hipSetDevice");
   HIPC(hipMalloc(&ctx->d_ann_off, sizeof(int64_t) * bns->n_seqs), "hipMalloc(ann_offset)");
@@ -578,6 +579,9 @@
   HIPC(s.d_redo.ensure(sizeof(int32_t) * nr), "hipMalloc(redo)");
   HIPC(s.d_rbits.ensure(sizeof(uint32_t) * (nr / 32 + 1)), "hipMalloc(rbits)");
   HIPC(s.d_desc.ensure(sizeof(ReadDesc) * nr), "hipMalloc(desc)");
+  HIPC(s.d_ldesc.ensure(sizeof(ReadDesc) * nr), "hipMalloc(ldesc)");
+  HIPC(s.d_ltile.ensure(sizeof(int32_t) * 4 * ((nr + kLightTile - 1) / kLightTile)), "hipMalloc(ltile)");
+  HIPC(s.d_lunit.ensure(sizeof(int2) * nr), "hipMalloc(lunit)");
   HIPC(s.d_schain.ensure(sizeof(int32_t) * ns), "hipMalloc(seedchain)");
   HIPC(s.d_hinfo.ensure(sizeof(int4) * nr), "hipMalloc(hinfo)");
   HIPC(s.d_cov.ensure(sizeof(int32_t) * ns), "hipMalloc(cov)");
@@ -604,6 +608,9 @@
   a.redo = s.d_redo.as<int32_t>();
   a.rbits = s.d_rbits.as<uint32_t>();
   a.rdesc = s.d_desc.as<ReadDesc>();
+  a.ldesc = s.d_ldesc.as<ReadDesc>();
+  a.ltile = s.d_ltile.as<int32_t>();
+  a.lunit = s.d_lunit.as<int2>();
   a.seedchain = s.d_schain.as<int32_t>();
   a.hinfo = s.d_hinfo.as<int4>();
   a.mat = s.d_mat.as<uint64_t>();
@@ -633,6 +640,7 @@
   }();
   a.emu_strict = emu_strict;
   a.light_pack = ctx->light_pack;
+  a.light_class = ctx->light_class && ctx->light_pack && !risky_first;
   a.out = d_out;
   a.out_n = d_n;
   a.stats = d_stats;
@@ -1126,6 +1134,13 @@
   if (!ctx) return BWAGPU_E_INVAL;
   const int prev = ctx->light_pack;
   if (on >= 0) ctx->light_pack = on != 0;
+  return prev;
+}
+
+int bwagpu_ctx_light_class(bwagpu_ctx_t* ctx, int on) {
+  if (!ctx) return BWAGPU_E_INVAL;
+  const int prev = ctx->light_class;
+  if (on >= 0) ctx->light_class = on != 0;
   return prev;
 }
 
diff --git a/bwa-flow_amd/csrc/ctx.h b/bwa-flow_amd/csrc/ctx.h
--- a/bwa-flow_amd/csrc/ctx.h
+++ b/bwa-flow_amd/csrc/ctx.h
@@ -49,6 +49,7 @@
   hipEvent_t ev0 = nullptr, ev1 = nullptr, ev2 = nullptr, ev3 = nullptr;
   DevBuf d_in, d_win, d_srt, d_prog, d_desc, d_out, d_n, d_stats, d_lists, d_counts;
   DevBuf d_cread, d_ext, d_tasks, d_ctr, d_regpos, d_skipf, d_heavy, d_redo, d_rbits;
+  DevBuf d_ldesc, d_ltile, d_lunit;
   DevBuf d_schain, d_hinfo, d_mat, d_cov, d_hflag, d_colent, d_qh, d_longc, d_sorth, d_stasks, d_ftask, d_ftaskR;
   SpecStreams spec;
   bool side_chosen = false;
@@ -57,6 +58,7 @@
     d_cread.release(); d_ext.release(); d_tasks.release(); d_ctr.release(); d_regpos.release(); d_skipf.release();
     d_heavy.release(); d_redo.release(); d_rbits.release(); d_schain.release(); d_hinfo.release(); d_mat.release(); d_cov.release(); d_hflag.release(); d_colent.release(); d_longc.release();
     d_qh.release();
+    d_ldesc.release(); d_ltile.release(); d_lunit.release();
     d_sorth.release();
     d_stasks.release();
     d_ftask.release();
@@ -121,6 +123,7 @@
   int ext_form = 0;
   int ext_short = 0;
   int light_pack = 0;
+  int light_class = 0;
   int ext_short_fill = 0;
   Slot slot[BWAGPU_NUM_SLOTS];
   hipStream_t dev_stream[BWAGPU_NUM_SLOTS] = {};
diff --git a/bwa-flow_amd/csrc/engine.h b/bwa-flow_amd/csrc/engine.h
--- a/bwa-flow_amd/csrc/engine.h
+++ b/bwa-flow_amd/csrc/engine.h
@@ -4,6 +4,7 @@
 
 #include "bwagpu.h"
 #include "bwagpu_debug.h"
+#include "light_class.h"
 #include "pure.h"
 #include "spec_plan.h"
 
@@ -89,6 +90,7 @@
 constexpr int kSpecRounds = 3;
 constexpr int kOrderLane = 8;
 constexpr int kSelLight = 64;
+static_assert(kSelLight == kLcLight, "light_class.h's widest light read");
 constexpr int kSelRegLds = 256;
 constexpr int kSelMatMaxSeeds = 4096;
 enum {
@@ -107,6 +109,8 @@
   SPC_LLONG = 84,
   SPC_RLONG = 93,
   SPC_SHORT_N = 102,
+  SPC_LTILES = 104,
+  SPC_LUNITS = 105,
   SPC_WORDS = 128
 };
 constexpr int kQHStride = 32;
@@ -142,6 +146,9 @@
   int32_t* redo;
   uint32_t* rbits;
   ReadDesc* rdesc;
+  ReadDesc* ldesc;
+  int32_t* ltile;
+  int2* lunit;
   int32_t* seedchain;
   int4* hinfo;
   int32_t* colent;
@@ -158,6 +165,7 @@
   int risky_first;
   int emu_strict;
   int light_pack;
+  int light_class;
   int ext_prefetch;
   bwagpu_alnreg_t* out;
   int32_t* out_n;
@@ -177,6 +185,7 @@
 int ext_short_default();
 int ext_short_fill_default();
 int light_pack_default();
+int light_class_default();
 int ext_kernel_for(const DevOpt& o, int form, int tb_bytes);
 hipError_t launch_spec_clear(const SpecArgs& a, int n_reads, int n_seeds, hipStream_t st);
 hipError_t launch_spec_chain2aln(const DevOpt& o, const DevRef& ref, const DevBatch& b, const SpecArgs& a,
diff --git a/bwa-flow_amd/csrc/light_class.h b/bwa-flow_amd/csrc/light_class.h
--- /dev/null
+++ b/bwa-flow_amd/csrc/light_class.h
@@ -0,0 +1,54 @@
+#pragma once
+#include <cstdint>
+
+#if defined(__HIPCC__) || defined(__CUDACC__)
+#define LC_HD __host__ __device__
+#else
+#define LC_HD
+#endif
+
+namespace bwagpu {
+
+constexpr int kLightTile = 1024;
+constexpr int kLcLight = 64;
+enum { LC_QUAD = 0, LC_OCT = 1, LC_WIDE = 2, LC_NONE = 3, kLightClasses = 3 };
+
+LC_HD inline int light_class_of(int ns, int nch, bool skipped) {
+  const int w = ns > nch ? ns : nch;
+  return skipped || w > kLcLight ? LC_NONE : w <= 4 ? LC_QUAD : w <= 8 ? LC_OCT : LC_WIDE;
+}
+LC_HD inline int light_unit_reads(int cls) { return cls == LC_QUAD ? 16 : cls == LC_OCT ? 8 : 1; }
+LC_HD inline int light_unit_lanes(int cls) { return cls == LC_QUAD ? 4 : cls == LC_OCT ? 8 : 64; }
+LC_HD inline int light_class_units(int cls, int n) { return (n + light_unit_reads(cls) - 1) / light_unit_reads(cls); }
+LC_HD inline int light_tile_units(const int32_t* n) {
+  return light_class_units(LC_QUAD, n[LC_QUAD]) + light_class_units(LC_OCT, n[LC_OCT]) +
+         light_class_units(LC_WIDE, n[LC_WIDE]);
+}
+
+LC_HD inline int light_tile_pos(const int32_t (*wc)[kLightClasses], int n_waves, int wave, int cls, int rank) {
+  int pos = rank;
+  for (int w = 0; w < n_waves; ++w)
+    for (int c = 0; c <= cls; ++c)
+      if (c < cls || w < wave) pos += wc[w][c];
+  return pos;
+}
+
+struct LightUnit {
+  int32_t cls, pos, cnt;
+};
+LC_HD inline LightUnit light_tile_unit(const int32_t* n, int lu) {
+  int first = 0;
+  for (int c = 0; c < kLightClasses; ++c) {
+    const int nu = light_class_units(c, n[c]), per = light_unit_reads(c);
+    if (lu < nu) {
+      const int left = n[c] - lu * per;
+      return LightUnit{c, first + lu * per, left < per ? left : per};
+    }
+    lu -= nu;
+    first += n[c];
+  }
+  return LightUnit{LC_NONE, first, 0};
+}
+LC_HD inline int32_t light_unit_word(const LightUnit& u) { return u.cls | u.cnt << 8; }
+
+}
diff --git a/bwa-flow_amd/csrc/spec.hip b/bwa-flow_amd/csrc/spec.hip
--- a/bwa-flow_amd/csrc/spec.hip
+++ b/bwa-flow_amd/csrc/spec.hip
@@ -65,15 +65,20 @@
   if (p >= 0) a.longc[p] = c;
 }
 
-__global__ void __launch_bounds__(256) spec_reads_kernel(DevBatch b, SpecArgs a) {
+__global__ void __launch_bounds__(kLightTile) spec_reads_kernel(DevBatch b, SpecArgs a) {
   sel_prio();
+  constexpr int kWaves = kLightTile / 64;
+  __shared__ int32_t WC[kWaves][kLightClasses];
+  __shared__ int32_t WS[kWaves];
+  __shared__ int32_t TU[kLightTile];
+  __shared__ int32_t s_last, s_carry;
   const int rd = blockIdx.x * blockDim.x + threadIdx.x;
   bool heavy = false;
-  int ns = 0;
+  int ns = 0, cls = LC_NONE;
+  ReadDesc d{};
   if (rd < b.n_reads) {
     const int lq = (int)(b.seq_off[rd + 1] - b.seq_off[rd]);
     if (lq > a.lq_bound) atomicOr((unsigned long long*)&a.stats[ST_ERR], (unsigned long long)ERR_LEN);
-    ReadDesc d;
     d.qoff = b.seq_off[rd];
     d.rd = rd;
     d.lq = lq;
@@ -85,6 +90,7 @@
     for (int c = d.c0; c < d.c0 + d.nch; ++c) a.chain_read[c] = rd;
     heavy = d.ns > kSelLight || d.nch > kSelLight;
     ns = d.ns;
+    cls = light_class_of(d.ns, d.nch, lq > a.lq_bound);
   }
   const int p = wave_append(&a.ctr[SPC_HEAVY_N], heavy);
   if (p >= 0) {
@@ -102,6 +108,65 @@
     }
     a.hinfo[p] = make_int4(rd, woff, col, ns);
   }
+  if (!a.light_class) return;
+  const int r = (int)(threadIdx.x & 63), wv = (int)(threadIdx.x >> 6);
+  const uint64_t lt_mask = r ? (~0ull >> (64 - r)) : 0ull;
+  uint64_t own = 0;
+#pragma unroll
+  for (int c = 0; c < kLightClasses; ++c) {
+    const uint64_t m = __builtin_amdgcn_ballot_w64(cls == c);
+    own = cls == c ? m : own;
+    if (r == 0) WC[wv][c] = (int)__popcll(m);
+  }
+  __syncthreads();
+  if (cls != LC_NONE)
+    a.ldesc[(size_t)blockIdx.x * kLightTile + light_tile_pos(WC, kWaves, wv, cls, (int)__popcll(own & lt_mask))] = d;
+  if (threadIdx.x == 0) {
+    for (int c = 0; c < kLightClasses; ++c) {
+      int n = 0;
+      for (int w = 0; w < kWaves; ++w) n += WC[w][c];
+      __hip_atomic_store(&a.ltile[4 * blockIdx.x + c], n, __ATOMIC_RELAXED, __HIP_MEMORY_SCOPE_AGENT);
+    }
+    s_last = __hip_atomic_fetch_add(&a.ctr[SPC_LTILES], 1, __ATOMIC_ACQ_REL, __HIP_MEMORY_SCOPE_AGENT) ==
+             (int)gridDim.x - 1;
+    s_carry = 0;
+  }
+  __syncthreads();
+  if (!s_last) return;
+  __threadfence();
+  const int n_tiles = (int)gridDim.x;
+  for (int t0 = 0; t0 < n_tiles; t0 += kLightTile) {
+    const int t = t0 + (int)threadIdx.x;
+    int32_t cn[kLightClasses] = {0, 0, 0};
+    if (t < n_tiles)
+      for (int c = 0; c < kLightClasses; ++c)
+        cn[c] = __hip_atomic_load(&a.ltile[4 * t + c], __ATOMIC_RELAXED, __HIP_MEMORY_SCOPE_AGENT);
+    const int nu = light_tile_units(cn);
+    int inc = nu;
+    for (int m = 1; m < 64; m <<= 1) {
+      const int v = __shfl_up(inc, m, 64);
+      inc += r >= m ? v : 0;
+    }
+    if (r == 63) WS[wv] = inc;
+    __syncthreads();
+    int first = s_carry + inc - nu;
+    for (int w = 0; w < wv; ++w) first += WS[w];
+    TU[threadIdx.x] = first;
+    __syncthreads();
+    if (threadIdx.x == kLightTile - 1) s_carry = first + nu;
+    for (int tt = t0 + wv; tt < min(t0 + kLightTile, n_tiles); tt += kWaves) {
+      int32_t tn[kLightClasses];
+      for (int c = 0; c < kLightClasses; ++c)
+        tn[c] = __hip_atomic_load(&a.ltile[4 * tt + c], __ATOMIC_RELAXED, __HIP_MEMORY_SCOPE_AGENT);
+      const int tnu = light_tile_units(tn), tfirst = TU[tt - t0];
+      for (int lu = r; lu < tnu; lu += 64) {
+        const LightUnit u = light_tile_unit(tn, lu);
+        a.lunit[tfirst + lu] = make_int2(tt * kLightTile + u.pos, light_unit_word(u));
+      }
+    }
+    __syncthreads();
+  }
+  if (threadIdx.x == 0) a.ctr[SPC_LUNITS] = s_carry;
 }
 
 constexpr int kOrderBlocks = 1024;
@@ -1293,19 +1358,22 @@
 }
 
 constexpr int kPackW = 8;
-template <int MODE>
+template <int MODE, int G>
 __device__ __forceinline__ uint64_t light_packed(const DevBatch& b, const SpecArgs& a, const int32_t* MG, int rd,
                                                  const ReadDesc& d, bool nar, Tally& tl) {
+  static_assert(G == 4 || G == kPackW, "a group is a quad or half a DPP row");
   constexpr bool WRITE = MODE != SEL_EMULATE;
+  using Sets = typename std::conditional<G == 4, uint32_t, uint64_t>::type;
+  constexpr uint32_t kGrp = (1u << G) - 1u;
   const uint64_t t_start = g_trace ? __builtin_amdgcn_s_memrealtime() : 0;
   int r = (int)(threadIdx.x & 63);
   asm volatile("" : "+v"(r));
-  const int i = r & 7, g0 = r & ~7;
+  const int i = r & (G - 1), g0 = r & ~(G - 1);
   const auto grp = [&](int v, int l) { return __builtin_amdgcn_ds_bpermute((g0 + l) << 2, v); };
   const auto grp64 = [&](int64_t v, int l) {
     return (int64_t)((uint64_t)(uint32_t)grp((int)(v >> 32), l) << 32 | (uint32_t)grp((int)v, l));
   };
-  const auto byte_of = [&](uint64_t m) { return (uint32_t)(m >> g0) & 0xFFu; };
+  const auto byte_of = [&](uint64_t m) { return (uint32_t)(m >> g0) & kGrp; };
   const bool has_c = nar && i < d.nch, has_s = nar && i < d.ns;
   int ce_l = 15, rid_l = 0;
   float fr_l = 0.f;
@@ -1326,10 +1394,10 @@
   uint32_t ends = (uint32_t)ce_l << (4 * i);
   ends |= (uint32_t)dpp<0xB1>(0, (int)ends);
   ends |= (uint32_t)dpp<0x4E>(0, (int)ends);
-  ends |= (uint32_t)dpp<0x141>(0, (int)ends);
+  if (G == 8) ends |= (uint32_t)dpp<0x141>(0, (int)ends);
   int cid = 0;
 #pragma unroll
-  for (int c = 0; c < kPackW - 1; ++c) cid += (int)((ends >> (4 * c)) & 15u) <= i;
+  for (int c = 0; c < G - 1; ++c) cid += (int)((ends >> (4 * c)) & 15u) <= i;
   const bool vchain = grp(ok_l ? 1 : 0, cid) != 0;
   const int rid = grp(rid_l, cid);
   const float frac = __int_as_float(grp(__float_as_int(fr_l), cid));
@@ -1347,10 +1415,10 @@
   pj.qe = x.qe;
   pj.w = x.w;
   pj.seedlen0 = sd.len;
-  uint64_t C = 0, O = 0;
+  Sets C = 0, O = 0;
   int cov = 0;
 #pragma unroll 1
-  for (int k = 0; k < kPackW && __builtin_amdgcn_ballot_w64(nar && k < d.ns) != 0; ++k) {
+  for (int k = 0; k < G && __builtin_amdgcn_ballot_w64(nar && k < d.ns) != 0; ++k) {
     bwagpu_seed_t sk;
     sk.rbeg = grp64(sd.rbeg, k);
     sk.qbeg = grp(sd.qbeg, k);
@@ -1368,8 +1436,8 @@
     const bool b1 = sd.qbeg <= sk.qbeg && sd.qbeg + sd.len - sk.qbeg >= sk.len >> 2 &&
                     (int64_t)(sk.qbeg - sd.qbeg) != sk.rbeg - sd.rbeg;
     const uint64_t om = __builtin_amdgcn_ballot_w64(valid && i < k && cid == k_cid && !j_pad && sd.len >= len95 && (a1 || b1));
-    C |= (uint64_t)byte_of(cm) << (8 * k);
-    O |= (uint64_t)byte_of(om) << (8 * k);
+    C |= (Sets)byte_of(cm) << (G * k);
+    O |= (Sets)byte_of(om) << (G * k);
     if (WRITE) {
       const int64_t krb = grp64(x.rb, k), kre = grp64(x.re, k);
       const int kqb = grp(x.qb, k), kqe = grp(x.qe, k);
@@ -1377,16 +1445,16 @@
                       sd.rbeg + sd.len <= kre ? sd.len : 0;
       v += dpp<0xB1>(0, v);
       v += dpp<0x4E>(0, v);
-      v += dpp<0x141>(0, v);
+      if (G == 8) v += dpp<0x141>(0, v);
       cov = i == k ? v : cov;
     }
   }
   uint32_t ext = 0, skip = pad_m, pend = 0, spend = 0, unc = 0;
   bool missed = false;
 #pragma unroll
-  for (int k = 0; k < kPackW; ++k) {
+  for (int k = 0; k < G; ++k) {
     const uint32_t bit = 1u << k;
-    const uint32_t cm = (uint32_t)(C >> (8 * k)) & 0xFFu, om = (uint32_t)(O >> (8 * k)) & 0xFFu;
+    const uint32_t cm = (uint32_t)(C >> (G * k)) & kGrp, om = (uint32_t)(O >> (G * k)) & kGrp;
     const bool act = (present_m & bit) != 0 && !missed;
     const bool done = (computed_m & bit) != 0;
     const bool skp = act && (cm & ext) != 0 && !(om & ~skip);
@@ -1436,21 +1504,23 @@
   }
   if (uint32_t* const tr = g_trace) {
     const uint64_t t_end = __builtin_amdgcn_s_memrealtime();
-    uint32_t v = 1u;
-    v = i == 0 ? (uint32_t)t_start : v;
-    v = i == 1 ? (uint32_t)(t_start >> 32) : v;
-    v = i == 2 ? (uint32_t)t_end : v;
-    v = i == 3 ? (uint32_t)(t_end >> 32) : v;
-    v = i == 4 ? (uint32_t)d.ns : v;
-    v = i == 5 ? (uint32_t)__popc(ext) : v;
-    v = i == 6 ? __builtin_amdgcn_s_getreg((31 << 11) | 20) : v;
-    if (nar && !missed) tr[((size_t)MODE * b.n_reads + rd) * 8 + i] = v;
+    for (int q = i; q < 8; q += G) {
+      uint32_t v = 1u;
+      v = q == 0 ? (uint32_t)t_start : v;
+      v = q == 1 ? (uint32_t)(t_start >> 32) : v;
+      v = q == 2 ? (uint32_t)t_end : v;
+      v = q == 3 ? (uint32_t)(t_end >> 32) : v;
+      v = q == 4 ? (uint32_t)d.ns : v;
+      v = q == 5 ? (uint32_t)__popc(ext) : v;
+      v = q == 6 ? __builtin_amdgcn_s_getreg((31 << 11) | 20) : v;
+      if (nar && !missed) tr[((size_t)MODE * b.n_reads + rd) * 8 + q] = v;
+    }
   }
   return __builtin_amdgcn_ballot_w64(nar && missed);
 }
 
 template <int MODE>
-__global__ void __launch_bounds__(kBlock) spec_select_light(DevOpt o, DevRef ref, DevBatch b, SpecArgs a,
+__global__ void __launch_bounds__(kBlock, MODE == SEL_EMULATE ? 8 : 1) spec_select_light(DevOpt o, DevRef ref, DevBatch b, SpecArgs a,
                                                             int tb_bytes) {
   sel_prio();
   constexpr bool WRITE = MODE != SEL_EMULATE;
@@ -1501,27 +1571,49 @@
   };
   const bool dyn = MODE == SEL_FINAL && a.risky_first;
   const bool pack = a.light_pack && !dyn;
-  const int n_units = pack ? (b.n_reads + kPackW - 1) / kPackW : b.n_reads;
-  const int unit_reads = pack ? kPackW : dyn ? 1 : 64;
-  const uint64_t first_lanes = pack ? 0x0101010101010101ull : dyn ? 1ull : ~0ull;
+  const bool cm = pack && a.light_class;
+  const int n_units = cm ? uni(a.ctr[SPC_LUNITS]) : pack ? (b.n_reads + kPackW - 1) / kPackW : b.n_reads;
+  const int unit_reads = cm ? 16 : pack ? kPackW : dyn ? 1 : 64;
   const auto lane_read = [&](int u) { return pack ? kPackW * u + (r >> 3) : dyn ? u : u + r * NW; };
+  const auto fetch = [&](int u, int2 rec) -> ReadDesc {
+    ReadDesc x{};
+    x.rd = b.n_reads;
+    if (cm) {
+      const int cls = rec.y & 255, cnt = rec.y >> 8;
+      const int slot = cls == LC_QUAD ? r >> 2 : cls == LC_OCT ? r >> 3 : 0;
+      if (slot < cnt) x = a.ldesc[rec.x + slot];
+    } else if (lane_read(u) < b.n_reads) {
+      x = a.rdesc[lane_read(u)];
+    }
+    return x;
+  };
   const uint64_t lt_mask = r ? (~0ull >> (64 - r)) : 0ull;
   int un = dyn ? next_read() : w0;
+  int2 rec = make_int2(0, 0), recn = make_int2(0, 0);
+  if (cm && un < n_units) rec = a.lunit[un];
+  if (cm && un + NW < n_units) recn = a.lunit[un + NW];
   while (un < n_units) {
     int nw = 0;
-    ReadDesc dn{};
-    if (lane_read(un) < b.n_reads) dn = a.rdesc[lane_read(un)];
+    ReadDesc dn = fetch(un, rec);
     while (un < n_units && nw + unit_reads <= kLightList) {
       const ReadDesc d = dn;
-      const int rd = lane_read(un);
+      const int rd = d.rd;
+      const int ucls = cm ? uni(rec.y & 255) : LC_OCT;
       un = dyn ? next_read() : pack ? un + NW : un + 64 * NW;
-      if (un < n_units && lane_read(un) < b.n_reads) dn = a.rdesc[lane_read(un)];
+      if (cm) {
+        rec = recn;
+        if (un + NW < n_units) recn = a.lunit[un + NW];
+      }
+      if (un < n_units) dn = fetch(un, rec);
       const bool mine = rd < b.n_reads && !(d.ns > kSelLight || d.nch > kSelLight) && !(d.lq > a.lq_bound);
-      const bool nar = pack && mine && d.ns <= kPackW && d.nch <= kPackW;
+      const int gw = ucls == LC_QUAD ? 4 : kPackW;
+      const bool nar = pack && ucls != LC_WIDE && mine && d.ns <= gw && d.nch <= gw;
       if (WRITE && mine && !nar && d.ns == 0) a.out_n[rd] = 0;
       uint64_t wide = __builtin_amdgcn_ballot_w64(mine && !nar && d.ns != 0);
-      if (pack) wide |= light_packed<MODE>(b, a, MG, rd, d, nar, tl);
-      wide &= first_lanes;
+      if (pack && ucls == LC_OCT) wide |= light_packed<MODE, kPackW>(b, a, MG, rd, d, nar, tl);
+      if (pack && ucls == LC_QUAD) wide |= light_packed<MODE, 4>(b, a, MG, rd, d, nar, tl);
+      wide &= !pack ? (dyn ? 1ull : ~0ull)
+              : ucls == LC_QUAD ? 0x1111111111111111ull : ucls == LC_OCT ? 0x0101010101010101ull : 1ull;
       if ((wide >> r) & 1) wl[nw + (int)__popcll(wide & lt_mask)] = rd;
       nw += (int)__popcll(wide);
     }
@@ -1931,15 +2023,28 @@
   }();
   return v;
 }
+#ifndef BWAGPU_LIGHT_CLASS_DEFAULT
+#define BWAGPU_LIGHT_CLASS_DEFAULT 1
+#endif
+int light_class_default() {
+  static const int v = [] {
+    const char* e = getenv("BWAGPU_LIGHT_CLASS");
+    return e && e[0] ? (atoi(e) != 0 ? 1 : 0) : BWAGPU_LIGHT_CLASS_DEFAULT;
+  }();
+  return v;
+}
 #ifndef BWAGPU_LIGHT_PACK_WGS_DEFAULT
 #define BWAGPU_LIGHT_PACK_WGS_DEFAULT 2
 #endif
-static int light_pack_wgs() {
+#ifndef BWAGPU_LIGHT_CLASS_WGS_DEFAULT
+#define BWAGPU_LIGHT_CLASS_WGS_DEFAULT 1
+#endif
+static int light_pack_wgs(bool by_class) {
   static const int v = [] {
     const char* e = getenv("BWAGPU_LIGHT_PACK_WGS");
-    return std::min(std::max(e && e[0] ? atoi(e) : BWAGPU_LIGHT_PACK_WGS_DEFAULT, 1), 64);
+    return e && e[0] ? std::min(std::max(atoi(e), 1), 64) : 0;
   }();
-  return v;
+  return v ? v : by_class ? BWAGPU_LIGHT_CLASS_WGS_DEFAULT : BWAGPU_LIGHT_PACK_WGS_DEFAULT;
 }
 static int device_cus() {
   int dev = 0, ncu = 0;
@@ -1963,7 +2068,7 @@
     int nb = resident_blocks(spec_select_light<MODE>, lds);
     if (a.light_pack && !(MODE == SEL_FINAL && a.risky_first)) {
       const int octets = (b.n_reads + kPackW - 1) / kPackW, per_wg = kBlock / 64;
-      nb = std::min(nb, std::max(1, std::min((octets + per_wg - 1) / per_wg, light_pack_wgs() * device_cus())));
+      nb = std::min(nb, std::max(1, std::min((octets + per_wg - 1) / per_wg, light_pack_wgs(a.light_class != 0) * device_cus())));
     }
     hipLaunchKernelGGL((spec_select_light<MODE>), dim3(nb), dim3(kBlock), lds, st, o, ref, b, a, tb_bytes);
   }
@@ -2048,7 +2153,7 @@
 hipError_t launch_spec_chain2aln(const DevOpt& o, const DevRef& ref, const DevBatch& b, const SpecArgs& a,
                                  int tb_bytes, int lq_max, hipStream_t st, const SpecStreams& ss) {
   if (b.n_reads == 0) return hipSuccess;
-  hipLaunchKernelGGL(spec_reads_kernel, dim3((b.n_reads + 255) / 256), dim3(256), 0, st, b, a);
+  hipLaunchKernelGGL(spec_reads_kernel, dim3((b.n_reads + kLightTile - 1) / kLightTile), dim3(kLightTile), 0, st, b, a);
   if (b.n_chains) {
     hipLaunchKernelGGL(spec_chain_kernel, dim3((b.n_chains + 255) / 256), dim3(256), 0, st, o, ref, b, a);
     hipLaunchKernelGGL(spec_order_kernel, dim3(kOrderBlocks), dim3(256), 0, st, o, ref, b, a);
diff --git a/bwa-flow_amd/python/bwagpu/abi.py b/bwa-flow_amd/python/bwagpu/abi.py
--- a/bwa-flow_amd/python/bwagpu/abi.py
+++ b/bwa-flow_amd/python/bwagpu/abi.py
@@ -196,6 +196,7 @@
     "bwagpu_ctx_ext_short": (C.c_int, [_VP, C.c_int]),
     "bwagpu_ctx_ext_short_fill": (C.c_int, [_VP, C.c_int]),
     "bwagpu_ctx_light_pack": (C.c_int, [_VP, C.c_int]),
+    "bwagpu_ctx_light_class": (C.c_int, [_VP, C.c_int]),
     "bwagpu_debug_spec_short": (C.c_int, [_VP, _VP, _VP]),
     "bwagpu_ctx_row_bound": (C.c_int, [_VP, C.c_int]),
     "bwagpu_debug_ext_kernel": (C.c_int, [_VP, C.c_int32]),
@@ -252,7 +253,8 @@
         raise RuntimeError(f"bwagpu: HIP engine library missing at {p}; run __graft_entry__.build()")
     lib = C.CDLL(p)
     for name, (res, args) in PROTOS.items():
-        if (name.startswith("bwagpu_debug_") or name == "bwagpu_ctx_light_pack") and not hasattr(lib, name):
+        ab = name.startswith("bwagpu_debug_") or name in ("bwagpu_ctx_light_pack", "bwagpu_ctx_light_class")
+        if ab and not hasattr(lib, name):
             continue
         fn = getattr(lib, name)
         fn.restype = res
diff --git a/bwa-flow_amd/python/bwagpu/engine.py b/bwa-flow_amd/python/bwagpu/engine.py
--- a/bwa-flow_amd/python/bwagpu/engine.py
+++ b/bwa-flow_amd/python/bwagpu/engine.py
@@ -306,6 +306,9 @@
     def light_pack(self, on: int = -1) -> int:
         return self.lib.bwagpu_ctx_light_pack(self.ctx, int(on))
 
+    def light_class(self, on: int = -1) -> int:
+        return self.lib.bwagpu_ctx_light_class(self.ctx, int(on))
+
     def row_bound(self, on: int = -1) -> int:
         return self.lib.bwagpu_ctx_row_bound(self.ctx, int(on))
 
diff --git a/include/bwagpu_debug.h b/include/bwagpu_debug.h
--- a/include/bwagpu_debug.h
+++ b/include/bwagpu_debug.h
@@ -23,6 +23,7 @@
 int bwagpu_ctx_ext_short(bwagpu_ctx_t *ctx, int q);
 int bwagpu_ctx_ext_short_fill(bwagpu_ctx_t *ctx, int percent);
 int bwagpu_ctx_light_pack(bwagpu_ctx_t *ctx, int on);
+int bwagpu_ctx_light_class(bwagpu_ctx_t *ctx, int on);
 int bwagpu_debug_spec_short(bwagpu_ctx_t *ctx, void *stream, int64_t *out);
 int bwagpu_ctx_row_bound(bwagpu_ctx_t *ctx, int on);
 int bwagpu_debug_ext_kernel(bwagpu_ctx_t *ctx, int32_t lq_max);
```

Measured after the change: 65.20, median of 6. 1.01x the previous value.
